# danini/multi-h

Hardware: AMD Instinct MI355X
Metric: scored homography hypotheses/sec (50k pts x 100k models) (higher is better)
Workload: dtype f64

## Files before the change

### multi-h_amd/csrc/capi.hip

```cpp

#include "capi_engine.hpp"

thread_local std::string g_err;

namespace mhe {

void resolve_timers(mh_engine* e)
{
    for (int k = 0; k < MH_K_COUNT_; ++k) {
        KernelTimer& t = e->timers[k];
        for (auto& pr : t.pending) {
            float ms = 0.f;
            if (hipEventSynchronize(pr.second) == hipSuccess &&
                hipEventElapsedTime(&ms, pr.first, pr.second) == hipSuccess) {
                t.total_ms += ms;
                t.launches += 1;
            }
        }
        t.pending.clear();
    }
}

int enter(mh_engine* e)
{
    if (!e) return fail(MH_ERR_INVALID, "null engine");
    HIPCHK(hipSetDevice(e->device));
    return MH_OK;
}

int require_points(mh_engine* e)
{
    int rc = enter(e);
    if (rc) return rc;
    if (e->n <= 0) return fail(MH_ERR_NOT_SET, "correspondences are not set");
    return MH_OK;
}

int require_models(mh_engine* e)
{
    int rc = require_points(e);
    if (rc) return rc;
    if (e->m <= 0) return fail(MH_ERR_NOT_SET, "model set is empty");
    return MH_OK;
}

int require_models_or_empty_shard(mh_engine* e, bool* empty)
{
    *empty = false;
    int rc = require_points(e);
    if (rc) return rc;
    if (e->m <= 0 && (e->t_stream_fn || e->t_host_fn)) { *empty = true; e->counts_fresh = true; return MH_OK; }
    if (e->m <= 0) return fail(MH_ERR_NOT_SET, "model set is empty");
    return MH_OK;
}

hipError_t reserve_counts(mh_engine* e, size_t n)
{
    if (n <= e->counts.cap) return hipSuccess;
    e->counts_zeroed = false;
    return e->counts.reserve(n);
}

int quiesce(mh_engine* e)
{
    HIPCHK(hipStreamSynchronize(e->stream));
    if (e->side_stream) HIPCHK(hipStreamSynchronize(e->side_stream));
    if (e->xchg_stream) HIPCHK(hipStreamSynchronize(e->xchg_stream));
    e->xchg_pending = false;
    return MH_OK;
}

int join_xchg(mh_engine* e)
{
    if (e->xchg_pending && e->xchg_calls > 0)
        HIPCHK(hipStreamWaitEvent(e->stream, e->ev_x[(e->xchg_calls - 1) % 3], 0));
    return MH_OK;
}

}

namespace {

template <typename Fn>
static void host_parallel_for(int n, Fn fn)
{
    unsigned t = std::thread::hardware_concurrency();
    if (t == 0) t = 1;
    if (t > 16) t = 16;
    if (n < 20000) t = 1;
    if (t == 1) { fn(0, n); return; }
    std::vector<std::thread> pool;
    const int chunk = (n + (int)t - 1) / (int)t;
    for (unsigned k = 0; k < t; ++k) {
        const int b = (int)k * chunk, en = std::min(n, b + chunk);
        if (b < en) pool.emplace_back(fn, b, en);
    }
    for (auto& th : pool) th.join();
}

int build_sym_graph(mh_engine* e, const int* rowptr, const int* col, int n)
{
    for (int i = 0; i < n; ++i)
        if (rowptr[i + 1] < rowptr[i]) return fail(MH_ERR_INVALID, "rowptr must be non-decreasing");
    std::unique_ptr<std::atomic<int>[]> cnt(new std::atomic<int>[(size_t)n + 1]);
    for (int i = 0; i <= n; ++i) cnt[i].store(0, std::memory_order_relaxed);
    std::atomic<int> bad(0);
    host_parallel_for(n, [&](int b, int en) {
        for (int i = b; i < en; ++i)
            for (int k = rowptr[i]; k < rowptr[i + 1]; ++k) {
                const int j = col[k];
                if (j < 0 || j >= n) { bad.store(1, std::memory_order_relaxed); continue; }
                if (j == i) continue;
                cnt[i].fetch_add(1, std::memory_order_relaxed);
                cnt[j].fetch_add(1, std::memory_order_relaxed);
            }
    });
    if (bad.load()) return fail(MH_ERR_INVALID, "neighbour index out of range");
    std::vector<long long> start(n + 1, 0);
    for (int i = 0; i < n; ++i) start[i + 1] = start[i] + cnt[i].load(std::memory_order_relaxed);
    if (start[n] > 0x7fffffffll) return fail(MH_ERR_OVERFLOW, "too many neighbour entries");
    std::vector<int> raw((size_t)start[n]);
    for (int i = 0; i < n; ++i) cnt[i].store(0, std::memory_order_relaxed);
    host_parallel_for(n, [&](int b, int en) {
        for (int i = b; i < en; ++i)
            for (int k = rowptr[i]; k < rowptr[i + 1]; ++k) {
                const int j = col[k];
                if (j == i) continue;
                raw[(size_t)(start[i] + cnt[i].fetch_add(1, std::memory_order_relaxed))] = j;
                raw[(size_t)(start[j] + cnt[j].fetch_add(1, std::memory_order_relaxed))] = i;
            }
    });
    std::vector<int> mult((size_t)start[n]);
    e->g_rowptr.assign(n + 1, 0);
    host_parallel_for(n, [&](int b, int en) {
        for (int i = b; i < en; ++i) {
            int* rb = raw.data() + start[i];
            int* re = raw.data() + start[i + 1];
            int* mb = mult.data() + start[i];
            std::sort(rb, re);
            int u = 0;
            for (int* p = rb; p < re;) {
                int* q = p;
                while (q < re && *q == *p) ++q;
                rb[u] = *p;
                mb[u] = (int)(q - p);
                ++u;
                p = q;
            }
            e->g_rowptr[i + 1] = u;
        }
    });
    for (int i = 0; i < n; ++i) e->g_rowptr[i + 1] += e->g_rowptr[i];
    const int nnz = e->g_rowptr[n];
    e->g_col.resize(nnz);
    e->g_w.resize(nnz);
    e->g_rev.assign(nnz, -1);
    host_parallel_for(n, [&](int b, int en) {
        for (int i = b; i < en; ++i) {
            const int len = e->g_rowptr[i + 1] - e->g_rowptr[i];
            std::copy(raw.data() + start[i], raw.data() + start[i] + len, e->g_col.data() + e->g_rowptr[i]);
            std::copy(mult.data() + start[i], mult.data() + start[i] + len, e->g_w.data() + e->g_rowptr[i]);
        }
    });
    host_parallel_for(n, [&](int b, int en) {
        for (int i = b; i < en; ++i)
            for (int k = e->g_rowptr[i]; k < e->g_rowptr[i + 1]; ++k) {
                const int j = e->g_col[k];
                const int* rb = e->g_col.data() + e->g_rowptr[j];
                const int* re = e->g_col.data() + e->g_rowptr[j + 1];
                e->g_rev[k] = (int)(std::lower_bound(rb, re, i) - e->g_col.data());
            }
    });
    return MH_OK;
}

static int upload_order(mh_engine* e)
{
    const int n = e->n;
    if (e->order_n == n) return MH_OK;
    std::vector<int> order(n);
    for (int i = 0; i < n; ++i) order[i] = i;
    unsigned long long z = 0x6d682d6f72646572ull;
    for (int i = n - 1; i > 0; --i) {
        z += 0x9E3779B97F4A7C15ull;
        unsigned long long x = z;
        x = (x ^ (x >> 30)) * 0xBF58476D1CE4E5B9ull;
        x = (x ^ (x >> 27)) * 0x94D049BB133111EBull;
        x ^= x >> 31;
        const int j = (int)(((x >> 32) * (unsigned long long)(i + 1)) >> 32);
        std::swap(order[i], order[j]);
    }
    HIPCHK(e->d_order.reserve(n));
    HIPCHK(hipMemcpyAsync(e->d_order.p, order.data(), sizeof(int) * n, hipMemcpyHostToDevice, e->stream));
    HIPCHK(hipStreamSynchronize(e->stream));
    e->order_n = n;
    return MH_OK;
}

static int upload_wsum(mh_engine* e)
{
    HIPCHK(e->d_wsum.reserve(e->n));
    HIPCHK(launch_row_weight_sums(e->n, e->d_rowptr.p, e->d_w.p, e->d_wsum.p, e->stream));
    return MH_OK;
}

int upload_graph(mh_engine* e)
{
    const int n = e->n, nnz = (int)e->g_col.size();
    HIPCHK(e->d_rowptr.reserve(n + 1));
    HIPCHK(e->d_col.reserve(nnz));
    HIPCHK(e->d_w.reserve(nnz));
    HIPCHK(e->d_rev.reserve(nnz));
    HIPCHK(hipMemcpyAsync(e->d_rowptr.p, e->g_rowptr.data(), sizeof(int) * (n + 1), hipMemcpyHostToDevice, e->stream));
    if (nnz) {
        HIPCHK(hipMemcpyAsync(e->d_col.p, e->g_col.data(), sizeof(int) * nnz, hipMemcpyHostToDevice, e->stream));
        HIPCHK(hipMemcpyAsync(e->d_w.p, e->g_w.data(), sizeof(int) * nnz, hipMemcpyHostToDevice, e->stream));
        HIPCHK(hipMemcpyAsync(e->d_rev.p, e->g_rev.data(), sizeof(int) * nnz, hipMemcpyHostToDevice, e->stream));
    }
    HIPCHK(hipStreamSynchronize(e->stream));
    int rc = upload_order(e);
    if (rc) return rc;
    rc = upload_wsum(e);
    if (rc) return rc;
    HIPCHK(hipStreamSynchronize(e->stream));
    e->g_nnz = nnz;
    e->g_host_valid = true;
    e->have_graph = true;
    return MH_OK;
}

static hipError_t fetch_ints(mh_engine* e, int* dst, const int* src_dev, size_t count)
{
    hipError_t he = hipMemcpyAsync(dst, src_dev, sizeof(int) * count, hipMemcpyDeviceToHost, e->stream);
    return he != hipSuccess ? he : hipStreamSynchronize(e->stream);
}

static int device_sym_graph(mh_engine* e, const int* rowptr_dev, int stride, const int* col_dev)
{
    const int n = e->n;
    HIPCHK(e->gb_deg.reserve(n));
    HIPCHK(e->gb_start.reserve((size_t)n + 1));
    HIPCHK(launch_sym_count(n, rowptr_dev, stride, col_dev, e->gb_deg.p, e->gb_start.p, e->gb_info.p, e->stream));
    int info[8] = {}, total = 0;
    HIPCHK(hipMemcpyAsync(info, e->gb_info.p, sizeof(int) * 4, hipMemcpyDeviceToHost, e->stream));
    HIPCHK(hipMemcpyAsync(&total, e->gb_start.p + n, sizeof(int), hipMemcpyDeviceToHost, e->stream));
    HIPCHK(hipStreamSynchronize(e->stream));
    if (info[2] == 2) return fail(MH_ERR_INVALID, "rowptr must be non-decreasing");
    if (info[2]) return fail(MH_ERR_INVALID, "neighbour index out of range (non-finite coordinates, or fewer than k neighbours at finite float32 distance?)");
    if (info[0]) return fail(MH_ERR_OVERFLOW, "too many neighbour entries");
    if (info[1] > SYM_MAX_ROW) {
        std::vector<int> rp(n + 1), col;
        if (rowptr_dev) {
            HIPCHK(fetch_ints(e, rp.data(), rowptr_dev, (size_t)n + 1));
            col.resize((size_t)rp[n]);
            if (rp[n] > 0) HIPCHK(fetch_ints(e, col.data(), col_dev, col.size()));
        } else {
            std::vector<int> dense((size_t)n * stride);
            HIPCHK(fetch_ints(e, dense.data(), col_dev, dense.size()));
            for (int i = 0; i < n; ++i) {
                rp[i] = (int)col.size();
                for (int j = 0; j < stride; ++j) if (dense[(size_t)i * stride + j] >= 0) col.push_back(dense[(size_t)i * stride + j]);
            }
            rp[n] = (int)col.size();
        }
        int rc = build_sym_graph(e, rp.data(), col.data(), n);
        if (rc) return rc;
        return upload_graph(e);
    }
    HIPCHK(e->gb_cursor.reserve(n));
    HIPCHK(e->gb_uniq.reserve(n));
    HIPCHK(e->gb_raw.reserve((size_t)std::max(total, 1)));
    HIPCHK(e->gb_mult.reserve((size_t)std::max(total, 1)));
    HIPCHK(e->d_rowptr.reserve((size_t)n + 1));
    HIPCHK(launch_sym_build(n, rowptr_dev, stride, col_dev, e->gb_start.p, e->gb_cursor.p, e->gb_raw.p, e->gb_mult.p,
                            e->gb_uniq.p, e->d_rowptr.p, e->gb_info.p, e->stream));
    int nnz = 0;
    HIPCHK(hipMemcpyAsync(&nnz, e->d_rowptr.p + n, sizeof(int), hipMemcpyDeviceToHost, e->stream));
    HIPCHK(hipStreamSynchronize(e->stream));
    HIPCHK(e->d_col.reserve((size_t)std::max(nnz, 1)));
    HIPCHK(e->d_w.reserve((size_t)std::max(nnz, 1)));
    HIPCHK(e->d_rev.reserve((size_t)std::max(nnz, 1)));
    HIPCHK(launch_sym_finish(n, e->gb_start.p, e->gb_raw.p, e->gb_mult.p, e->d_rowptr.p, e->d_col.p, e->d_w.p, e->d_rev.p, e->stream));
    int rc = upload_order(e);
    if (rc) return rc;
    rc = upload_wsum(e);
    if (rc) return rc;
    HIPCHK(hipStreamSynchronize(e->stream));
    e->g_nnz = nnz;
    e->g_host_valid = false;
    e->have_graph = true;
    return MH_OK;
}

__global__ void k_split_soa(int n, const double* src, const double* dst, const double* aff,
                            double* x1, double* y1, double* x2, double* y2, double* a11,
                            double* a12, double* a21, double* a22)
{
    const int i = blockIdx.x * 256 + threadIdx.x;
    if (i >= n) return;
    x1[i] = src[2 * i]; y1[i] = src[2 * i + 1];
    x2[i] = dst[2 * i]; y2[i] = dst[2 * i + 1];
    if (aff) { a11[i] = aff[4 * i]; a12[i] = aff[4 * i + 1]; a21[i] = aff[4 * i + 2]; a22[i] = aff[4 * i + 3]; }
}

}

extern "C" {

int mh_abi_version(void) { return MH_ABI_VERSION; }

const char* mh_last_error(void) { return g_err.c_str(); }

int mh_device_count(void)
{
    int c = 0;
    if (hipGetDeviceCount(&c) != hipSuccess) return 0;
    return c;
}

int mh_create(mh_engine** out, int device)
{
    return guarded([&]() -> int {
    if (!out) return fail(MH_ERR_INVALID, "out is null");
    *out = nullptr;
    int c = 0;
    if (hipGetDeviceCount(&c) != hipSuccess || c <= 0)
        return fail(MH_ERR_NO_DEVICE, "no HIP device visible; the Multi-H engine has no CPU fallback");
    if (device < 0 || device >= c) return fail(MH_ERR_INVALID, "device index out of range");
    HIPCHK(hipSetDevice(device));
    hipDeviceProp_t prop;
    HIPCHK(hipGetDeviceProperties(&prop, device));
    if (std::strncmp(prop.gcnArchName, "gfx950", 6) != 0)
        return fail(MH_ERR_NO_DEVICE, std::string("device arch is ") + prop.gcnArchName +
                                           "; this library carries gfx950 code objects only");
    mh_engine* e = new (std::nothrow) mh_engine();
    if (!e) return fail(MH_ERR_INVALID, "out of host memory");
    e->device = device;
    e->cu_count = prop.multiProcessorCount > 0 ? prop.multiProcessorCount : 256;
    hipError_t he = e->own_stream.ensure();
    if (he != hipSuccess) { delete e; return fail(MH_ERR_HIP, hipGetErrorString(he)); }
    e->stream = e->own_stream;
    *out = e;
    return MH_OK;
    });
}

void mh_destroy(mh_engine* e)
{
    if (!e) return;
    (void)hipSetDevice(e->device);
    (void)quiesce(e);
    resolve_timers(e);
    delete e;
}

int mh_set_params(mh_engine* e, double thr_F, double thr_H, double locality, double lambda, int min_inliers)
{
    return guarded([&]() -> int {
    if (!e) return fail(MH_ERR_INVALID, "null engine");
    if (!(thr_H > 0.0) || !(lambda > 0.0)) return fail(MH_ERR_INVALID, "thr_hom and lambda must be positive");
    e->thr_F = thr_F; e->thr_H = thr_H; e->locality = locality; e->lambda = lambda;
    e->min_inliers = min_inliers;
    e->cost_L = 0;
    return MH_OK;
    });
}

int mh_set_stream(mh_engine* e, void* hip_stream, int external)
{
    return guarded([&]() -> int {
    int rc0 = enter(e);
    if (rc0) return rc0;
    int rcq = quiesce(e);
    if (rcq) return rcq;
    resolve_timers(e);
    e->stream = external ? (hipStream_t)hip_stream : e->own_stream.s;
    return MH_OK;
    });
}

int mh_synchronize(mh_engine* e)
{
    return guarded([&]() -> int {
    int rc0 = enter(e);
    if (rc0) return rc0;
    rc0 = quiesce(e);
    if (rc0) return rc0;
    resolve_timers(e);
    return MH_OK;
    });
}

int mh_set_correspondences(mh_engine* e, const double* src_xy, const double* dst_xy,
                           const double* affines, int n)
{
    return guarded([&]() -> int {
    int rc0 = enter(e);
    if (rc0) return rc0;
    if (!src_xy || !dst_xy || n <= 0) return fail(MH_ERR_INVALID, "src/dst must be non-null and n > 0");
    rc0 = quiesce(e);
    if (rc0) return rc0;
    e->pf_count = 0;
    e->pf_head = 0;
    e->smp_k = 0;
    e->weights_models_seq = -1;
    const size_t cap = (size_t)n + 2;
    HIPCHK(e->x1.reserve(cap)); HIPCHK(e->y1.reserve(cap));
    HIPCHK(e->x2.reserve(cap)); HIPCHK(e->y2.reserve(cap));
    HIPCHK(e->a11.reserve(cap)); HIPCHK(e->a12.reserve(cap));
    HIPCHK(e->a21.reserve(cap)); HIPCHK(e->a22.reserve(cap));
    DevBuf<double> s, d, a;
    HIPCHK(s.reserve((size_t)n * 2));
    HIPCHK(d.reserve((size_t)n * 2));
    HIPCHK(hipMemcpyAsync(s.p, src_xy, sizeof(double) * 2 * n, hipMemcpyHostToDevice, e->stream));
    HIPCHK(hipMemcpyAsync(d.p, dst_xy, sizeof(double) * 2 * n, hipMemcpyHostToDevice, e->stream));
    if (affines) {
        HIPCHK(a.reserve((size_t)n * 4));
        HIPCHK(hipMemcpyAsync(a.p, affines, sizeof(double) * 4 * n, hipMemcpyHostToDevice, e->stream));
    }
    hipLaunchKernelGGL(k_split_soa, dim3((n + 255) / 256), dim3(256), 0, e->stream, n, s.p, d.p,
                       affines ? a.p : nullptr, e->x1.p, e->y1.p, e->x2.p, e->y2.p, e->a11.p,
                       e->a12.p, e->a21.p, e->a22.p);
    HIPCHK(hipGetLastError());
    HIPCHK(hipStreamSynchronize(e->stream));
    if (n != e->n) {
        drop_models(e);
        e->ldr = 0; e->fm = 0; e->f7_m = 0;
    }
    {
        double xmin = src_xy[0], xmax = src_xy[0], ymin = src_xy[1], ymax = src_xy[1], dmax = 0.0;
        bool finite = true, dfinite = true;
        for (int i = 0; i < n; ++i) {
            const double x = src_xy[2 * i], y = src_xy[2 * i + 1];
            finite = finite && std::isfinite(x) && std::isfinite(y);
            xmin = x < xmin ? x : xmin; xmax = x > xmax ? x : xmax;
            ymin = y < ymin ? y : ymin; ymax = y > ymax ? y : ymax;
            const double a = std::fabs(dst_xy[2 * i]), b = std::fabs(dst_xy[2 * i + 1]);
            dfinite = dfinite && std::isfinite(a) && std::isfinite(b);
            dmax = a > dmax ? a : dmax; dmax = b > dmax ? b : dmax;
        }
        if (!finite) xmin = xmax = ymin = ymax = NAN;
        e->bbox[0] = xmin; e->bbox[1] = xmax; e->bbox[2] = ymin; e->bbox[3] = ymax;
        e->absmax_x = std::max(std::fabs(xmin), std::fabs(xmax));
        e->absmax_y = std::max(std::fabs(ymin), std::fabs(ymax));
        e->absmax_dst = dmax;
        e->coords32_ok = finite && dfinite && e->absmax_x < 0x1p20 && e->absmax_y < 0x1p20 && dmax < 0x1p20;
    }
    e->n = n;
    e->have_aff = affines != nullptr;
    e->have_graph = false;
    e->g_rowptr.clear(); e->g_col.clear(); e->g_w.clear(); e->g_rev.clear();
    e->g_host_valid = false; e->g_nnz = 0;
    e->cost_L = 0;
    return MH_OK;
    });
}

int mh_set_epipolar(mh_engine* e, const double F[9], const double e2[2])
{
    return guarded([&]() -> int {
    if (!e || !F || !e2) return fail(MH_ERR_INVALID, "null argument");
    for (int i = 0; i < 9; ++i) e->epi.F[i] = F[i];
    e->epi.ex = e2[0];
    e->epi.ey = e2[1];
    e->have_epi = true;
    return MH_OK;
    });
}

int mh_set_neighbors_csr(mh_engine* e, const int* rowptr, const int* col, int n)
{
    return guarded([&]() -> int {
    int rc = require_points(e);
    if (rc) return rc;
    if (!rowptr || n != e->n) return fail(MH_ERR_INVALID, "rowptr null or n != number of correspondences");
    if (rowptr[n] > 0 && !col) return fail(MH_ERR_INVALID, "col is null");
    if (rowptr[0] < 0) return fail(MH_ERR_INVALID, "rowptr must be non-decreasing");
    for (int i = 0; i < n; ++i)
        if (rowptr[i + 1] < rowptr[i]) return fail(MH_ERR_INVALID, "rowptr must be non-decreasing");
    HIPCHK(e->gb_info.reserve(8));
    HIPCHK(hipMemsetAsync(e->gb_info.p, 0, sizeof(int) * 8, e->stream));
    HIPCHK(e->gb_hits_rp.reserve((size_t)n + 1));
    HIPCHK(e->gb_hits_col.reserve((size_t)std::max(rowptr[n], 1)));
    HIPCHK(hipMemcpyAsync(e->gb_hits_rp.p, rowptr, sizeof(int) * ((size_t)n + 1), hipMemcpyHostToDevice, e->stream));
    if (rowptr[n] > 0)
        HIPCHK(hipMemcpyAsync(e->gb_hits_col.p, col, sizeof(int) * (size_t)rowptr[n], hipMemcpyHostToDevice, e->stream));
    HIPCHK(hipStreamSynchronize(e->stream));
    return device_sym_graph(e, e->gb_hits_rp.p, 0, e->gb_hits_col.p);
    });
}

static int knn_table(mh_engine* e, int k, double radius, int* tbl)
{
    const int n = e->n;
    HIPCHK(e->gb_info.reserve(8));
    HIPCHK(hipMemsetAsync(e->gb_info.p, 0, sizeof(int) * 8, e->stream));
    const Points pp = e->pts();
    if (e->tune_knn_grid && std::isfinite(pp.xmin) && std::isfinite(pp.xmax) && std::isfinite(pp.ymin) && std::isfinite(pp.ymax)) {
        const int G = knn_grid_cells(n);
        HIPCHK(e->knn_cell.reserve((size_t)n));
        HIPCHK(e->knn_count.reserve((size_t)G * G));
        HIPCHK(e->knn_start.reserve((size_t)G * G + 1));
        HIPCHK(e->knn_P.reserve((size_t)4 * n));
        HIPCHK(e->knn_orig.reserve((size_t)n));
        const hipError_t hg = launch_knn_grid(pp, k, tbl, e->knn_cell.p, e->knn_count.p, e->knn_start.p, e->knn_P.p, e->knn_orig.p, e->stream);
        if (hg == hipSuccess) {
            const float r2g = radius > 0.0 ? (float)radius * (float)radius : INFINITY;
            HIPCHK(launch_hits_filter(pp, k, r2g, tbl, e->gb_info.p + 2, e->stream));
            return MH_OK;
        }
        if (hg != hipErrorInvalidValue) HIPCHK(hg);
    }
    const int blocks = (n + 255) / 256;
    int splits = (4 * e->cu_count + blocks - 1) / blocks;
    splits = std::max(1, std::min(splits, std::min(KNN_MAX_SPLITS, (n + 1023) / 1024)));
    const int kk = k <= 8 ? 8 : k <= 16 ? 16 : 32;
    if (splits > 1) {
        HIPCHK(e->knn_part_d.reserve((size_t)splits * n * kk));
        HIPCHK(e->knn_part_i.reserve((size_t)splits * n * kk));
    }
    HIPCHK(launch_knn(e->pts(), k, tbl, splits, e->knn_part_d.p, e->knn_part_i.p, e->stream));
    const float r2 = radius > 0.0 ? (float)radius * (float)radius : INFINITY;
    HIPCHK(launch_hits_filter(e->pts(), k, r2, tbl, e->gb_info.p + 2, e->stream));
    return MH_OK;
}

static int build_knn_graph(mh_engine* e, int k, double radius)
{
    int rc = require_points(e);
    if (rc) return rc;
    if (k < 1 || k > 32 || k >= e->n) return fail(MH_ERR_INVALID, "k must be in [1, 32] and < n");
    HIPCHK(e->knn_tmp.reserve((size_t)e->n * k));
    rc = knn_table(e, k, radius, e->knn_tmp.p);
    if (rc) return rc;
    return device_sym_graph(e, nullptr, k, e->knn_tmp.p);
}

int mh_build_neighbors_knn(mh_engine* e, int k)
{
    return guarded([&]() -> int { return build_knn_graph(e, k, 0.0); });
}

int mh_build_neighbors_knn_radius(mh_engine* e, int k, double radius)
{
    return guarded([&]() -> int { return build_knn_graph(e, k, radius); });
}

int mh_build_sample_neighbours(mh_engine* e, int k)
{
    return guarded([&]() -> int {
    int rc = require_points(e);
    if (rc) return rc;
    if (k < 3 || k > 32 || k >= e->n) return fail(MH_ERR_INVALID, "k must be in [3, 32] and < n");
    rc = quiesce(e);
    if (rc) return rc;
    e->smp_k = 0;
    HIPCHK(e->smp_nbr.reserve((size_t)e->n * k));
    rc = knn_table(e, k, 0.0, e->smp_nbr.p);
    if (rc) return rc;
    int err = 0;
    HIPCHK(fetch_ints(e, &err, e->gb_info.p + 2, 1));
    if (err) return fail(MH_ERR_INVALID, "neighbour index out of range (non-finite coordinates, or fewer than k neighbours at finite float32 distance?)");
    e->smp_k = k;
    return MH_OK;
    });
}

int mh_get_sample_neighbours(mh_engine* e, int* nbr, int* k_out)
{
    return guarded([&]() -> int {
    if (!e) return fail(MH_ERR_INVALID, "null engine");
    if (e->smp_k <= 0) return fail(MH_ERR_NOT_SET, "no sampling table; call mh_build_sample_neighbours");
    HIPCHK(hipSetDevice(e->device));
    if (nbr) HIPCHK(fetch_ints(e, nbr, e->smp_nbr.p, (size_t)e->n * e->smp_k));
    if (k_out) *k_out = e->smp_k;
    return MH_OK;
    });
}

int mh_build_neighbors_radius(mh_engine* e, double radius, long long max_hits, long long* hits_out)
{
    return guarded([&]() -> int {
    int rc = require_points(e);
    if (rc) return rc;
    if (!(radius > 0.0)) return fail(MH_ERR_INVALID, "radius must be positive");
    const int n = e->n;
    const float r2 = (float)radius * (float)radius;
    HIPCHK(e->knn_tmp.reserve((size_t)n + 1));
    HIPCHK(launch_radius_count(e->pts(), r2, e->knn_tmp.p, e->stream));
    std::vector<int> cnt(n), rowptr(n + 1, 0);
    HIPCHK(hipMemcpyAsync(cnt.data(), e->knn_tmp.p, sizeof(int) * n, hipMemcpyDeviceToHost, e->stream));
    HIPCHK(hipStreamSynchronize(e->stream));
    long long total = 0;
    for (int i = 0; i < n; ++i) total += cnt[i];
    if (hits_out) *hits_out = total;
    const long long limit = max_hits > 0 ? max_hits : 0x7fffffffll;
    if (total > limit || total > 0x7fffffffll) {
        char msg[160];
        snprintf(msg, sizeof msg, "radius search yields %lld hits (limit %lld): use a smaller radius or k-NN", total, limit);
        return fail(MH_ERR_OVERFLOW, msg);
    }
    for (int i = 0; i < n; ++i) rowptr[i + 1] = rowptr[i] + cnt[i];
    DevBuf<int> d_rp, d_col;
    HIPCHK(d_rp.reserve((size_t)n + 1));
    HIPCHK(d_col.reserve((size_t)std::max<long long>(total, 1)));
    HIPCHK(hipMemcpyAsync(d_rp.p, rowptr.data(), sizeof(int) * (n + 1), hipMemcpyHostToDevice, e->stream));
    HIPCHK(launch_radius_fill(e->pts(), r2, d_rp.p, d_col.p, e->stream));
    HIPCHK(e->gb_info.reserve(8));
    HIPCHK(hipMemsetAsync(e->gb_info.p, 0, sizeof(int) * 8, e->stream));
    return device_sym_graph(e, d_rp.p, 0, d_col.p);
    });
}

int mh_get_sym_graph(mh_engine* e, int* rowptr, int* col, int* w, int* nnz)
{
    return guarded([&]() -> int {
    if (!e) return fail(MH_ERR_INVALID, "null engine");
    if (!e->have_graph) return fail(MH_ERR_NOT_SET, "neighbour graph is not set");
    if (!e->g_host_valid) {
        HIPCHK(hipSetDevice(e->device));
        e->g_rowptr.resize((size_t)e->n + 1); e->g_col.resize(e->g_nnz); e->g_w.resize(e->g_nnz); e->g_rev.resize(e->g_nnz);
        HIPCHK(fetch_ints(e, e->g_rowptr.data(), e->d_rowptr.p, (size_t)e->n + 1));
        if (e->g_nnz) {
            HIPCHK(fetch_ints(e, e->g_col.data(), e->d_col.p, (size_t)e->g_nnz));
            HIPCHK(fetch_ints(e, e->g_w.data(), e->d_w.p, (size_t)e->g_nnz));
            HIPCHK(fetch_ints(e, e->g_rev.data(), e->d_rev.p, (size_t)e->g_nnz));
        }
        e->g_host_valid = true;
    }
    if (nnz) *nnz = e->g_nnz;
    if (rowptr) std::copy(e->g_rowptr.begin(), e->g_rowptr.end(), rowptr);
    if (col) std::copy(e->g_col.begin(), e->g_col.end(), col);
    if (w) std::copy(e->g_w.begin(), e->g_w.end(), w);
    return MH_OK;
    });
}

int mh_device_buffer(mh_engine* e, int which, void** ptr_dev, unsigned long long* bytes)
{
    return guarded([&]() -> int {
    if (!e || !ptr_dev || !bytes) return fail(MH_ERR_INVALID, "null argument");
    switch (which) {
    case MH_BUF_COUNTS: *ptr_dev = e->counts.p; *bytes = sizeof(int) * (size_t)e->m; break;
    case MH_BUF_MODELS: *ptr_dev = e->H.p; *bytes = sizeof(double) * 9 * (size_t)e->m; break;
    case MH_BUF_RESIDUALS: *ptr_dev = (e->ldr > 0 && e->m > 0) ? e->R.p : nullptr; *bytes = sizeof(double) * (size_t)e->m * (size_t)e->ldr; break;
    case MH_BUF_LABELS: *ptr_dev = e->ew_label.p; *bytes = sizeof(int) * (size_t)e->n; break;
    case MH_BUF_COST: *ptr_dev = e->cost.p; *bytes = sizeof(int) * (size_t)e->n * e->cost_L; break;
    case MH_BUF_GATHERED_SCORES: *ptr_dev = e->sel_gathered.p; *bytes = sizeof(int) * e->sel_gathered.cap; break;
    case MH_BUF_LABEL_COUNTS: *ptr_dev = e->label_counts.p; *bytes = sizeof(int) * std::min<size_t>(e->label_counts.cap, (size_t)e->m); break;
    case MH_BUF_WEIGHTS: *ptr_dev = e->weights_models_seq == e->models_seq ? e->weights.p : nullptr; *bytes = sizeof(int) * (size_t)e->m; break;
    default: return fail(MH_ERR_INVALID, "unknown buffer id");
    }
    if (!*ptr_dev) return fail(MH_ERR_NOT_SET, "buffer has not been produced yet");
    return MH_OK;
    });
}

int mh_profile_enable(mh_engine* e, int on)
{
    return guarded([&]() -> int {
    if (!e) return fail(MH_ERR_INVALID, "null engine");
    e->profiling = on != 0;
    return MH_OK;
    });
}

int mh_profile_reset(mh_engine* e)
{
    return guarded([&]() -> int {
    int rc0 = enter(e);
    if (rc0) return rc0;
    HIPCHK(hipStreamSynchronize(e->stream));
    resolve_timers(e);
    for (int k = 0; k < MH_K_COUNT_; ++k) { e->timers[k].launches = 0; e->timers[k].total_ms = 0.0; }
    return MH_OK;
    });
}

int mh_profile_get(mh_engine* e, int kernel, int* launches, double* total_ms)
{
    return guarded([&]() -> int {
    if (!e || kernel < 0 || kernel >= MH_K_COUNT_) return fail(MH_ERR_INVALID, "bad kernel id");
    HIPCHK(hipSetDevice(e->device));
    HIPCHK(hipStreamSynchronize(e->stream));
    if (e->xchg_stream) HIPCHK(hipStreamSynchronize(e->xchg_stream));
    resolve_timers(e);
    if (launches) *launches = e->timers[kernel].launches;
    if (total_ms) *total_ms = e->timers[kernel].total_ms;
    return MH_OK;
    });
}

int mh_set_tuning(mh_engine* e, int key, int value)
{
    return guarded([&]() -> int {
    if (!e) return fail(MH_ERR_INVALID, "null engine");
#ifdef MH_TUNING
    if (key == 0) { e->tune_residual_variant = value; return MH_OK; }
    if (key == 1) { e->tune_score_variant = value; return MH_OK; }
    if (key == 13 && value >= 0) { e->tune_ld = value; return MH_OK; }
#else
    if (key == 0 || key == 1) {
        if (value == 0) return MH_OK;
        return fail(MH_ERR_INVALID, "residual / score kernel variants exist only in a library built with -DMH_TUNING");
    }
#endif
    if (key >= 2 && key <= 5 && value >= 1) { e->tune_expand[key - 2] = value; return MH_OK; }
    if (key == 6 && value >= 0) { e->tune_reduce = value; return MH_OK; }
    if (key == 7 && value >= 1 && value <= 64) { e->tune_ms_batch = value; return MH_OK; }
    if (key == 29 && value >= 0 && value <= 64) { e->tune_ms_persist = value; return MH_OK; }
    if (key == 32 && (value == 0 || value == 1)) { e->tune_ms_indexed = value; return MH_OK; }
    if (key == 37 && value >= 1 && value <= EXPAND_MAX_CTX) { e->tune_expand_ctx = value; return MH_OK; }
    if (key == 38 && value >= 0 && value <= (1 << 20)) { e->tune_batch_min_labels = value; return MH_OK; }
    if (key == 39 && (value == 0 || value == 16 || value == 32 || value == 64)) { e->tune_batch_spw = value; return MH_OK; }
    if (key == 36 && (value == 0 || value == 1)) { e->tune_select_decrement = value; return MH_OK; }
    if (key == 33 && value >= 0 && value <= (1 << 20)) { e->tune_ms_dense = value; return MH_OK; }
    if (key == 30 && (value == 0 || value == 1)) { e->tune_select_refine = value; return MH_OK; }
    if (key == 31 && (value == 0 || value == 1)) { e->tune_knn_grid = value; return MH_OK; }
    if (key == 8 && value >= 0 && value <= (1 << 20)) { e->trace_moves = value; return MH_OK; }
    if (key == 9 && value >= -1) { e->detail_move = value; return MH_OK; }
    if (key == 10 && value >= 1 && value <= 64) { e->tune_push_mult = value; return MH_OK; }
    if (key == 11 && (value == 0 || value == 1)) { e->tune_recycle = value; return MH_OK; }
    if (key == 12 && (value == 1 || value == 2)) { e->tune_reduce_launches = value; return MH_OK; }
    if (key == 14 && value >= 0 && value <= 8) { e->inject_barrier_timeouts = value; return MH_OK; }
    if (key == 40 && (value == 0 || (value >> 4) >= 1)) { e->inject_solve_failure = value; return MH_OK; }
    if (key == 15 && (value == 0 || value == 1)) { e->tune_score32 = value; return MH_OK; }
#ifdef MH_TUNING
    if (key == 16 && value >= 0 && value <= 16) { e->tune_score32_tiling = value; return MH_OK; }
#else
    if (key == 16 && value == 0) return MH_OK;
#endif
    if (key == 17 && value >= 0 && value <= 1000) { e->tune_cascade_iters = value; return MH_OK; }
    if (key == 18 && value >= 0 && value <= 1000) { e->inject_select_failure = value; return MH_OK; }
    if (key == 19 && value >= -1 && value <= 1024) { e->tune_sweep_headroom = value; return MH_OK; }
    if (key == 20 && (value == 0 || value == 1)) { e->tune_dlt_first = value; return MH_OK; }
    if (key == 21 && value >= 0 && value <= (1 << 16)) { e->comp_moves = value; return MH_OK; }
    if (key == 22 && value >= 0 && value <= 16 && !e->side_stream) { e->tune_stream_shift = value; return MH_OK; }
    if (key == 23 && value >= -1 && value <= 64) { e->tune_cost32_resident = value; return MH_OK; }
    if (key == 24 && value >= -1 && value <= 64) { e->tune_score32_resident = value; return MH_OK; }
    if (key == 25 && value >= 0 && value <= 2) { e->tune_dlt_variant = value; return MH_OK; }
#ifdef MH_TUNING
    if (key == 26 && value >= 0 && value <= 4096) { e->tune_sweep_slices = value; return MH_OK; }
    if (key == 27 && (value == 0 || value == 1)) { e->tune_cost32_slice_major = value; return MH_OK; }
    if (key == 28 && (value == 0 || value == 1)) { e->tune_cost32_batched = value; return MH_OK; }
    if (key == 34 && value >= 0 && value <= 2) { e->tune_3pt_form = value; return MH_OK; }
#else
    if ((key == 26 || key == 27 || key == 28 || key == 34) && value == 0) return MH_OK;
    if (key == 16 || key == 26 || key == 27 || key == 28 || key == 34)
        return fail(MH_ERR_INVALID, "this schedule variant exists only in a library built with -DMH_TUNING");
#endif
    return fail(MH_ERR_INVALID, "unknown tuning key");
    });
}

}
```

### multi-h_amd/csrc/capi_engine.hpp

```cpp
#pragma once
#include "../../include/multih_hip.h"
#include "mh_kernels.hpp"

#include <algorithm>
#include <chrono>
#include <cstdlib>
#include <cmath>
#include <cstdio>
#include <cstring>
#include <string>
#include <utility>
#include <atomic>
#include <memory>
#include <thread>
#include <vector>

using namespace mh;

extern thread_local std::string g_err;

inline int fail(int code, const std::string& msg)
{
    g_err = msg;
    return code;
}

#define HIPCHK(expr)                                                                      \
    do {                                                                                  \
        hipError_t e_ = (expr);                                                           \
        if (e_ != hipSuccess)                                                             \
            return fail(MH_ERR_HIP, std::string(#expr) + ": " + hipGetErrorString(e_));   \
    } while (0)

struct NoCopy {
    NoCopy() = default;
    NoCopy(const NoCopy&) = delete;
    NoCopy& operator=(const NoCopy&) = delete;
};

template <class T>
struct DevBuf : NoCopy {
    T* p = nullptr;
    size_t cap = 0;
    DevBuf() = default;
    DevBuf(DevBuf&& o) noexcept { *this = std::move(o); }
    DevBuf& operator=(DevBuf&& o) noexcept { std::swap(p, o.p); std::swap(cap, o.cap); return *this; }
    ~DevBuf() { if (p) (void)hipFree(p); }
    hipError_t reserve(size_t n)
    {
        if (n <= cap) return hipSuccess;
        if (p) { hipError_t e = hipFree(p); p = nullptr; cap = 0; if (e != hipSuccess) return e; }
        hipError_t e = hipMalloc((void**)&p, std::max<size_t>(n, 1) * sizeof(T));
        if (e == hipSuccess) cap = n;
        return e;
    }
};

template <class T>
struct PinnedBuf : NoCopy {
    T* h = nullptr;
    T* d = nullptr;
    size_t cap = 0;
    ~PinnedBuf() { if (h) (void)hipHostFree(h); }
    hipError_t ensure(size_t n, bool mapped = true)
    {
        if (n <= cap) return hipSuccess;
        if (h) { (void)hipHostFree(h); h = d = nullptr; cap = 0; }
        hipError_t e = hipHostMalloc((void**)&h, n * sizeof(T), mapped ? hipHostMallocMapped : hipHostMallocDefault);
        if (e == hipSuccess && mapped) e = hipHostGetDevicePointer((void**)&d, h, 0);
        if (e != hipSuccess) { if (h) (void)hipHostFree(h); h = d = nullptr; return e; }
        std::memset(h, 0, n * sizeof(T));
        cap = n;
        return hipSuccess;
    }
};

struct Event : NoCopy {
    hipEvent_t ev = nullptr;
    Event() = default;
    Event(Event&& o) noexcept : ev(o.ev) { o.ev = nullptr; }
    Event& operator=(Event&& o) noexcept { std::swap(ev, o.ev); return *this; }
    ~Event() { if (ev) (void)hipEventDestroy(ev); }
    hipError_t ensure(unsigned flags = hipEventDisableTiming) { return ev ? hipSuccess : hipEventCreateWithFlags(&ev, flags); }
    operator hipEvent_t() const { return ev; }
};

struct Stream : NoCopy {
    hipStream_t s = nullptr;
    ~Stream() { if (s) { (void)hipStreamSynchronize(s); (void)hipStreamDestroy(s); } }
    hipError_t ensure(bool highest_priority = false)
    {
        if (s) return hipSuccess;
        if (!highest_priority) return hipStreamCreateWithFlags(&s, hipStreamNonBlocking);
        int lo = 0, hi = 0;
        hipError_t e = hipDeviceGetStreamPriorityRange(&lo, &hi);
        return e != hipSuccess ? e : hipStreamCreateWithPriority(&s, hipStreamNonBlocking, hi);
    }
    operator hipStream_t() const { return s; }
};

struct ExpandCtxBufs {
    DevBuf<int> arcs, sites, core, flags;
    DevBuf<long long> acc;
    DevBuf<unsigned char> took;
    static size_t pitch(int count) { return ((size_t)count + 2 + 63) & ~(size_t)63; }
    hipError_t reserve(int n, int nnz, bool with_took_list, hipStream_t stream)
    {
        auto grow = [&](auto& buf, size_t count) -> hipError_t {
            const size_t had = buf.cap;
            hipError_t e = buf.reserve(count);
            if (e == hipSuccess && buf.cap != had) e = hipMemsetAsync(buf.p, 0, sizeof(*buf.p) * buf.cap, stream);
            return e;
        };
        hipError_t e = grow(arcs, 2 * pitch(nnz));
        if (e == hipSuccess) e = grow(sites, (with_took_list ? 5 : 4) * pitch(n));
        if (e == hipSuccess) e = grow(core, (size_t)EXPAND_CORE_SHARDS * n);
        if (e == hipSuccess) e = grow(flags, EXPAND_FLAG_WORDS);
        if (e == hipSuccess) e = grow(acc, EXPAND_ACC_WORDS);
        if (e == hipSuccess) e = grow(took, (size_t)n + 2);
        return e;
    }
    ExpandWork::Ctx view(int n, int nnz) const
    {
        const size_t pa = pitch(nnz), ps = pitch(n);
        ExpandWork::Ctx x{};
        x.cap = arcs.p; x.sent = arcs.p + pa;
        x.excess = sites.p; x.sink_cap = sites.p + ps; x.height = sites.p + 2 * ps; x.decided = sites.p + 3 * ps;
        x.took_list = sites.cap >= 5 * ps ? sites.p + 4 * ps : nullptr;
        x.took = took.p; x.core = core.p; x.flags = flags.p; x.acc = acc.p;
        return x;
    }
};

struct KernelTimer {
    std::vector<std::pair<Event, Event>> pending;
    int launches = 0;
    double total_ms = 0.0;
};

enum class BatchOrigin { GIVEN, DLT4, HAF, P3 };
struct ResidentBatch {
    int m = 0;
    BatchOrigin origin = BatchOrigin::GIVEN;
    int haf_members = 0;
    bool have_samples = false;
};

struct CountsSlot {
    DevBuf<int> buf;
    bool zeroed = false;
    int wait = -1;
};

struct mh_engine : ResidentBatch {
    int device = 0;
    Stream own_stream;
    hipStream_t stream = nullptr;
    double thr_F = 3.0, thr_H = 2.5, locality = 0.002, lambda = 0.5;
    int min_inliers = 0;

    int n = 0;
    bool have_aff = false, have_epi = false, have_graph = false;
    DevBuf<double> x1, y1, x2, y2, a11, a12, a21, a22;
    Epipolar epi{};

    std::vector<int> g_rowptr, g_col, g_w, g_rev;
    bool g_host_valid = false;
    int g_nnz = 0;
    DevBuf<int> gb_deg, gb_start, gb_cursor, gb_raw, gb_mult, gb_uniq, gb_info, gb_hits_rp, gb_hits_col;
    int order_n = -1;
    DevBuf<int> d_rowptr, d_col, d_w, d_rev;

    DevBuf<double> H, H_one;
    DevBuf<int> samples, counts;
    DevBuf<unsigned> haf_used;
    DevBuf<double> R;
    long long ldr = 0;
    DevBuf<int> C;
    long long ldc = 0;
    DevBuf<unsigned char> mask;
    DevBuf<double> moments, min_eig;
    DevBuf<double> cp_pts, cp_H, cp_out;
    DevBuf<int> cp_begin, cp_tri;
    DevBuf<unsigned char> cp_ok;
    DevBuf<int> sel_orig[2], sel_counts, sel_carried[2], sel_left, sel_rec, sel_scores, sel_gathered;
    DevBuf<int> sel_weights, sel_carried_w[2], sel_left_w;
    DevBuf<double> sel_cand_H[2], sel_out_H;
    DevBuf<SelRecord> sel_records;
    DevBuf<long long> sel_counter;
    DevBuf<unsigned long long> sel_keys;
    int t_rank = 0, t_world = 1;
    mh_allgather_stream_fn t_stream_fn = nullptr;
    mh_allgather_dev_fn t_host_fn = nullptr;
    void* t_ctx = nullptr;
    Stream side_stream;
    Event ev_main, ev_side_pre;
    int tune_score32_resident = 12;
    int occ_score32 = -1, occ_cost32 = -1;
    int tune_cost32_batched = 0;
    int tune_cost32_slice_major = 0;
    int tune_sweep_slices = 0;
    int tune_dlt_variant = 0;
    int tune_cost32_resident = 8;
    int tune_stream_shift = 0;
    Stream dummy_streams[16];
    int tune_dlt_first = 1;
    static constexpr int PF_DEPTH = 2;
    DevBuf<double> pf_H[PF_DEPTH];
    DevBuf<int> pf_samples[PF_DEPTH];
    int pf_m[PF_DEPTH] = { 0, 0 };
    Event pf_ev[PF_DEPTH];
    int pf_head = 0, pf_count = 0;
    Stream xchg_stream;
    Event ev_sweep, ev_x[3];
    CountsSlot counts_waiting[2];
    long long xchg_calls = 0;
    long long models_seq = 0, best_models_seq = -1;
    bool counts_zeroed = false;
    bool counts_fresh = false;
    bool xchg_pending = false;
    PinnedBuf<int> h_best;
    int best_seq = 0;
    PinnedBuf<int> h_sel;
    long long copies_h2d = 0, copies_d2h = 0;

    int fm = 0;
    int fund_metric = 0;
    DevBuf<double> fund, fund_one;
    DevBuf<int> fund_samples, fund_counts, fund_inl;
    int fund_tuple = 8;
    int f7_m = 0;
    DevBuf<int> fund_nvalid, fund_stop;
    DevBuf<unsigned char> fund_mask, ref_keep, ref_in, ref_reason;
    int ref_reason_n = 0;
    DevBuf<double> ref_out;

    DevBuf<double> loc_H, loc_feat, ms_data, ms_mean;
    DevBuf<int> ms_votes, ms_out, ms_list, ms_pcnt, ms_heads, ms_tickets;
    DevBuf<double> ms_partial, ms_partial2;
    DevBuf<unsigned long long> ms_ticks;
    DevBuf<int> ms_ctl, ms_pcnt2;
    int ms_persist_per_cu = -1, ms_persist_per_cu6 = -1;
    int tune_select_refine = 0;
    int estimator = MH_ESTIMATOR_HAF;
    int data_term = MH_DATA_TERM_REFERENCE;
    DevBuf<int> r3_scratch;
    int tune_3pt_form = 0;
    DevBuf<double> sel_refit;
    DevBuf<int> sel_refit_ctr;
    DevBuf<double> ms_rs;
    DevBuf<int> ms_order, ms_cells, ms_cursor, ms_cellcount;
    int tune_ms_indexed = 1;
    int tune_ms_dense = 8;
    long long ms_indexed_launches = 0;
    int tune_ms_persist = 12;
    long long ms_persist_launches = 0, ms_persist_fallbacks = 0, ms_rounds = 0;

    int cost_L = 0;
    DevBuf<int> cost, labels_in, labels_pts, label_counts;
    DevBuf<int> ew_label, ew_cur, ew_trace, ew_saved, d_order, d_wsum;
    int comp_moves = 0;
    DevBuf<int> ew_comp, ew_comp_out;
    int trace_moves = 0;
    int detail_move = -1;
    ExpandCtxBufs ew_ctx[EXPAND_MAX_CTX];
    DevBuf<int> ew_bctl;
    PinnedBuf<int> h_batch;
    int tune_expand_ctx = 16;
    int tune_batch_min_labels = 16;
    int tune_batch_spw = 0;
    int cu_count = 256;
    DevBuf<int> sweep_ctl;
    int sweep_wg_per_cu = -1;
    int tune_sweep_headroom = 0;
    int solve_grid_max = 0;
    double longest_barrier_wait_ms = 0.0;
    int last_expand_retries = 0;
    long long expand_retries_total = 0;
    int last_solve_grid = 0;
    int inject_select_failure = 0;
    int inject_barrier_timeouts = 0;
    int inject_solve_failure = 0;
    PinnedBuf<int> h_flags;
    PinnedBuf<long long> h_acc;
    PinnedBuf<MeanShiftResultBlock> h_ms;
    PinnedBuf<int> h_ms_list;
    DevBuf<double> sel_pts[4];
    DevBuf<int> sel_pack_count;
    DevBuf<double> sel_gone[4];
    int tune_select_decrement = 1;
    int tune_knn_grid = 1;
    DevBuf<int> knn_cell, knn_count, knn_start, knn_orig;
    DevBuf<float> knn_P;
    DevBuf<int> knn_tmp, knn_part_i;
    DevBuf<float> knn_part_d;
    int sampler = MH_SAMPLER_UNIFORM, sampler_uniform_per_16 = 0;
    DevBuf<int> smp_nbr;
    int smp_k = 0;
    Dlt4Local dlt_local() const { return sampler == MH_SAMPLER_LOCAL ? Dlt4Local{ smp_nbr.p, smp_k, sampler_uniform_per_16 } : Dlt4Local{}; }

    bool profiling = false;
    KernelTimer timers[MH_K_COUNT_];
    int tune_residual_variant = 0;
    int tune_ld = 0;
    int tune_score_variant = 0;
    int residual_mode = MH_RESIDUAL_FORWARD;
    int tune_ms_batch = 6;
    int tune_reduce = 2;
    int tune_reduce_launches = 1;
    int tune_recycle = 1;
    int tune_expand[4] = { 128, 512, 1, 256 };
    int tune_cascade_iters = 2;
    int tune_push_mult = 6;
    ExpandStats last_expand{};

    double bbox[4] = { NAN, NAN, NAN, NAN };
    bool coords32_ok = false;
    double absmax_x = NAN, absmax_y = NAN, absmax_dst = NAN;
    int tune_score32_tiling = 0;
    int tune_score32 = 1;
    DevBuf<float> H32;
    DevBuf<unsigned long long> fb_pairs;
    long long score_pairs = 0;
    long long score_pairs_plain_fp64 = 0;
    DevBuf<int> weights, weights_counts;
    long long weights_models_seq = -1;
    PinnedBuf<int> h_best_w;
    Points pts() const { return Points{ x1.p, y1.p, x2.p, y2.p, n, bbox[0], bbox[1], bbox[2], bbox[3] }; }
};

namespace mhe {

template <typename Fn>
int guarded(Fn&& fn)
{
    try {
        return fn();
    } catch (const std::bad_alloc&) {
        return fail(MH_ERR_INVALID, "out of host memory");
    } catch (const std::exception& ex) {
        return fail(MH_ERR_INVALID, std::string("internal error: ") + ex.what());
    } catch (...) {
        return fail(MH_ERR_INVALID, "internal error");
    }
}

struct ScopedTimer {
    mh_engine* e;
    int k;
    hipStream_t st;
    Event a, b;
    bool on = false;
    ScopedTimer(mh_engine* e_, int k_, hipStream_t on_stream = nullptr) : e(e_), k(k_), st(on_stream ? on_stream : e_->stream)
    {
        if (!e->profiling || a.ensure(hipEventDefault) != hipSuccess || b.ensure(hipEventDefault) != hipSuccess) return;
        (void)hipEventRecord(a, st);
        on = true;
    }
    ~ScopedTimer()
    {
        if (!on) return;
        (void)hipEventRecord(b, st);
        e->timers[k].pending.emplace_back(std::move(a), std::move(b));
    }
};

inline void drop_models(mh_engine* e)
{
    static_cast<ResidentBatch&>(*e) = ResidentBatch{};
    e->cost_L = 0;
    e->counts_fresh = false;
    ++e->models_seq;
}

inline void install_models(mh_engine* e, int m, BatchOrigin origin, bool have_samples, int haf_members = 0)
{
    static_cast<ResidentBatch&>(*e) = ResidentBatch{ m, origin, haf_members, have_samples };
}

inline void counts_scored(mh_engine* e) { e->counts_fresh = true; e->counts_zeroed = false; }

inline int hand_counts_to_exchange(mh_engine* e, int par)
{
    CountsSlot* w = e->counts_waiting;
    const int wait = w[0].wait;
    std::swap(e->counts, w[0].buf);
    e->counts_zeroed = w[0].zeroed;
    w[0].zeroed = true;
    w[0].wait = par;
    std::swap(w[0], w[1]);
    return wait;
}

void resolve_timers(mh_engine* e);
int enter(mh_engine* e);
int require_points(mh_engine* e);
int require_models(mh_engine* e);
int require_models_or_empty_shard(mh_engine* e, bool* empty);
hipError_t reserve_counts(mh_engine* e, size_t n);
int quiesce(mh_engine* e);
int join_xchg(mh_engine* e);
int score_models(mh_engine* e, const Points& p, const double* Hs, int m, double thr2, const unsigned char* dmask, int* counts_dev);
int msac_models(mh_engine* e, const Points& p, const double* Hs, int m, double thr2, const unsigned char* dmask, int* counts_dev,
                int* weights_dev, bool plain_variant_only);
int launch_estimator(mh_engine* e, const int* labels_dev, int Nh, double* H_dev, int* counts_dev);
int ensure_xchg_stream(mh_engine* e);
int ensure_side_stream(mh_engine* e);

}

using namespace mhe;
```

### multi-h_amd/csrc/capi_score.hip

```cpp
#include "capi_engine.hpp"

namespace mhe {

static bool pretest_usable(const mh_engine* e, double thr2, bool plain_variant_only)
{
    if (plain_variant_only && e->tune_score_variant != 0) return false;
    return e->tune_score32 && e->coords32_ok && thr2 >= 0x1p-40 && thr2 <= 0x1p40;
}

static int ensure_sweep_ctl(mh_engine* e)
{
    if (!e->sweep_ctl.p) {
        HIPCHK(e->sweep_ctl.reserve(2));
        HIPCHK(hipMemsetAsync(e->sweep_ctl.p, 0, sizeof(int) * 2, e->stream));
    }
    return MH_OK;
}

int score_models(mh_engine* e, const Points& p, const double* Hs, int m, double thr2, const unsigned char* dmask, int* counts_dev)
{
    const bool fwd = e->residual_mode != MH_RESIDUAL_SYMMETRIC;
    if (fwd && m > 0 && pretest_usable(e, thr2, true)) {
        HIPCHK(e->H32.reserve((size_t)m * 16));
        HIPCHK(e->fb_pairs.reserve(1));
        if (e->score_pairs == 0) HIPCHK(hipMemsetAsync(e->fb_pairs.p, 0, sizeof(unsigned long long), e->stream));
        HIPCHK(launch_model32(Hs, m, e->absmax_x, e->absmax_y, e->absmax_dst, e->H32.p, e->stream));
        int* ctl = nullptr;
        if (e->tune_score32_resident != 0) {
            int rc = ensure_sweep_ctl(e);
            if (rc) return rc;
            ctl = e->sweep_ctl.p;
        }
        HIPCHK(launch_score32(p, Hs, e->H32.p, m, thr2, e->absmax_dst, dmask, counts_dev, e->fb_pairs.p, e->tune_score32_tiling, e->stream,
                              ctl, e->cu_count, e->tune_score32_resident, &e->occ_score32));
        e->score_pairs += (long long)m * p.n;
        return MH_OK;
    }
    HIPCHK(launch_score(p, Hs, m, thr2, dmask, counts_dev, fwd ? e->tune_score_variant : -1, e->stream));
    return MH_OK;
}

int msac_models(mh_engine* e, const Points& p, const double* Hs, int m, double thr2, const unsigned char* dmask, int* counts_dev,
                int* weights_dev, bool plain_variant_only)
{
    if (m <= 0 || p.n <= 0) return MH_OK;
    HIPCHK(e->fb_pairs.reserve(1));
    if (e->score_pairs == 0) HIPCHK(hipMemsetAsync(e->fb_pairs.p, 0, sizeof(unsigned long long), e->stream));
    if (pretest_usable(e, thr2, plain_variant_only)) {
        HIPCHK(e->H32.reserve((size_t)m * 16));
        HIPCHK(launch_model32(Hs, m, e->absmax_x, e->absmax_y, e->absmax_dst, e->H32.p, e->stream));
        HIPCHK(launch_msac32(p, Hs, e->H32.p, m, thr2, e->absmax_dst, dmask, counts_dev, weights_dev, e->fb_pairs.p, e->stream));
    } else {
        HIPCHK(launch_msac64(p, Hs, m, thr2, dmask, counts_dev, weights_dev, e->stream));
        e->score_pairs_plain_fp64 += (long long)m * p.n;
    }
    e->score_pairs += (long long)m * p.n;
    return MH_OK;
}

int ensure_side_stream(mh_engine* e)
{
    if (!e->side_stream)
        for (int k = 0; k < e->tune_stream_shift; ++k) HIPCHK(e->dummy_streams[k].ensure());
    HIPCHK(e->side_stream.ensure(true));
    for (int q = 0; q < mh_engine::PF_DEPTH; ++q) HIPCHK(e->pf_ev[q].ensure());
    HIPCHK(e->ev_main.ensure());
    HIPCHK(e->ev_side_pre.ensure());
    return MH_OK;
}

}

extern "C" {

int mh_propose_dlt4(mh_engine* e, unsigned long long seed, long long first, int m)
{
    return guarded([&]() -> int {
    int rc = require_points(e);
    if (rc) return rc;
    if (m <= 0) return fail(MH_ERR_INVALID, "m must be positive");
    if (e->n < 4) return fail(MH_ERR_INVALID, "need at least 4 correspondences");
    if (e->sampler == MH_SAMPLER_LOCAL && e->smp_k <= 0) return fail(MH_ERR_NOT_SET, "the local sampler has no table; call mh_build_sample_neighbours");
    drop_models(e);
    HIPCHK(e->H.reserve((size_t)m * 9));
    HIPCHK(e->samples.reserve((size_t)m * 4));
    HIPCHK(reserve_counts(e, (size_t)m + 1));
    {
        ScopedTimer t(e, MH_K_DLT4);
        HIPCHK(launch_dlt4(e->pts(), seed, first, m, e->samples.p, e->H.p, e->stream, e->tune_dlt_variant == 1 ? 1 : 0, e->dlt_local()));
    }
    install_models(e, m, BatchOrigin::DLT4, true);
    return MH_OK;
    });
}

int mh_set_sampler(mh_engine* e, int sampler, int uniform_per_16)
{
    return guarded([&]() -> int {
    if (!e) return fail(MH_ERR_INVALID, "null engine");
    if (sampler != MH_SAMPLER_UNIFORM && sampler != MH_SAMPLER_LOCAL) return fail(MH_ERR_INVALID, "unknown sampler");
    if (uniform_per_16 < 0 || uniform_per_16 > 16) return fail(MH_ERR_INVALID, "uniform_per_16 must be in [0, 16]");
    e->sampler = sampler;
    e->sampler_uniform_per_16 = uniform_per_16;
    return MH_OK;
    });
}

int mh_set_models(mh_engine* e, const double* H, int m)
{
    return guarded([&]() -> int {
    if (!e || m < 0 || (m > 0 && !H)) return fail(MH_ERR_INVALID, "null argument or m < 0");
    HIPCHK(hipSetDevice(e->device));
    drop_models(e);
    if (m == 0) return MH_OK;
    HIPCHK(e->H.reserve((size_t)m * 9));
    HIPCHK(reserve_counts(e, (size_t)m + 1));
    HIPCHK(hipMemcpyAsync(e->H.p, H, sizeof(double) * 9 * m, hipMemcpyHostToDevice, e->stream));
    HIPCHK(hipStreamSynchronize(e->stream));
    install_models(e, m, BatchOrigin::GIVEN, false);
    return MH_OK;
    });
}

int mh_get_models(mh_engine* e, double* H)
{
    return guarded([&]() -> int {
    if (!e || !H) return fail(MH_ERR_INVALID, "null argument");
    HIPCHK(hipSetDevice(e->device));
    if (e->m <= 0) return fail(MH_ERR_NOT_SET, "model set is empty");
    HIPCHK(hipMemcpyAsync(H, e->H.p, sizeof(double) * 9 * e->m, hipMemcpyDeviceToHost, e->stream));
    HIPCHK(hipStreamSynchronize(e->stream));
    return MH_OK;
    });
}

int mh_get_model(mh_engine* e, int idx, double H[9])
{
    return guarded([&]() -> int {
    if (!e || !H) return fail(MH_ERR_INVALID, "null argument");
    HIPCHK(hipSetDevice(e->device));
    if (e->m <= 0) return fail(MH_ERR_NOT_SET, "model set is empty");
    if (idx < 0 || idx >= e->m) return fail(MH_ERR_INVALID, "model index out of range");
    HIPCHK(hipMemcpyAsync(H, e->H.p + 9 * (size_t)idx, sizeof(double) * 9, hipMemcpyDeviceToHost, e->stream));
    HIPCHK(hipStreamSynchronize(e->stream));
    return MH_OK;
    });
}

int mh_get_model_count(mh_engine* e, int* m)
{
    return guarded([&]() -> int {
    if (!e || !m) return fail(MH_ERR_INVALID, "null argument");
    *m = e->m;
    return MH_OK;
    });
}

int mh_get_samples(mh_engine* e, int* idx)
{
    return guarded([&]() -> int {
    if (!e || !idx) return fail(MH_ERR_INVALID, "null argument");
    HIPCHK(hipSetDevice(e->device));
    if (!e->have_samples) return fail(MH_ERR_NOT_SET, "no sampled batch; call mh_propose_dlt4");
    HIPCHK(hipMemcpyAsync(idx, e->samples.p, sizeof(int) * 4 * e->m, hipMemcpyDeviceToHost, e->stream));
    HIPCHK(hipStreamSynchronize(e->stream));
    return MH_OK;
    });
}

int mh_set_residual_mode(mh_engine* e, int mode)
{
    return guarded([&]() -> int {
    if (!e) return fail(MH_ERR_INVALID, "null engine");
    if (mode != MH_RESIDUAL_FORWARD && mode != MH_RESIDUAL_SYMMETRIC) return fail(MH_ERR_INVALID, "unknown residual mode");
    e->residual_mode = mode;
    return MH_OK;
    });
}

int mh_score(mh_engine* e, double thr2, const unsigned char* point_mask, int* counts)
{
    return guarded([&]() -> int {
    bool empty_shard = false;
    int rc = require_models_or_empty_shard(e, &empty_shard);
    if (rc || empty_shard) return rc;
    HIPCHK(reserve_counts(e, (size_t)e->m + 1));
    const unsigned char* dmask = nullptr;
    if (point_mask) {
        HIPCHK(e->mask.reserve((size_t)e->n + 2));
        HIPCHK(hipMemcpyAsync(e->mask.p, point_mask, e->n, hipMemcpyHostToDevice, e->stream));
        dmask = e->mask.p;
    }
    {
        ScopedTimer t(e, MH_K_SCORE);
        rc = score_models(e, e->pts(), e->H.p, e->m, thr2, dmask, e->counts.p);
        if (rc) return rc;
    }
    counts_scored(e);
    if (counts) {
        HIPCHK(hipMemcpyAsync(counts, e->counts.p, sizeof(int) * e->m, hipMemcpyDeviceToHost, e->stream));
        HIPCHK(hipStreamSynchronize(e->stream));
    }
    return MH_OK;
    });
}

int mh_score_msac(mh_engine* e, double thr2, const unsigned char* point_mask, int* counts, int* weights)
{
    return guarded([&]() -> int {
    bool empty_shard = false;
    int rc = require_models_or_empty_shard(e, &empty_shard);
    if (rc || empty_shard) return rc;
    if (e->residual_mode == MH_RESIDUAL_SYMMETRIC) return fail(MH_ERR_INVALID, "mh_score_msac: forward residual only");
    if ((long long)e->n * MH_MSAC_SCALE > 2147483647ll) return fail(MH_ERR_OVERFLOW, "mh_score_msac: n * MH_MSAC_SCALE exceeds int32");
    HIPCHK(reserve_counts(e, (size_t)e->m + 1));
    HIPCHK(e->weights.reserve((size_t)e->m + 1));
    HIPCHK(e->weights_counts.reserve((size_t)e->m + 1));
    const unsigned char* dmask = nullptr;
    if (point_mask) {
        HIPCHK(e->mask.reserve((size_t)e->n + 2));
        HIPCHK(hipMemcpyAsync(e->mask.p, point_mask, e->n, hipMemcpyHostToDevice, e->stream));
        dmask = e->mask.p;
    }
    e->weights_models_seq = -1;
    {
        ScopedTimer t(e, MH_K_SCORE);
        rc = msac_models(e, e->pts(), e->H.p, e->m, thr2, dmask, e->counts.p, e->weights.p, false);
        if (rc) return rc;
    }
    HIPCHK(hipMemcpyAsync(e->weights_counts.p, e->counts.p, sizeof(int) * (size_t)e->m, hipMemcpyDeviceToDevice, e->stream));
    counts_scored(e);
    e->weights_models_seq = e->models_seq;
    if (counts) HIPCHK(hipMemcpyAsync(counts, e->counts.p, sizeof(int) * e->m, hipMemcpyDeviceToHost, e->stream));
    if (weights) HIPCHK(hipMemcpyAsync(weights, e->weights.p, sizeof(int) * e->m, hipMemcpyDeviceToHost, e->stream));
    if (counts || weights) HIPCHK(hipStreamSynchronize(e->stream));
    return MH_OK;
    });
}

int mh_residual_matrix(mh_engine* e, double thr2, double* R_host, int* counts)
{
    return guarded([&]() -> int {
    bool empty_shard = false;
    int rc = require_models_or_empty_shard(e, &empty_shard);
    if (rc || empty_shard) return rc;
    e->ldr = residual_ld(e->n);
    size_t r_elems = (size_t)e->m * (size_t)e->ldr;
#ifdef MH_TUNING
    if (e->tune_ld > 0) { e->ldr = std::max<long long>(e->tune_ld, e->ldr); r_elems = (size_t)e->m * (size_t)e->ldr; }
    r_elems = std::max(r_elems, (size_t)((e->m + 15) / 16 * 16) * (size_t)((e->n + 1023) / 1024 * 1024));
#endif
    HIPCHK(e->R.reserve(r_elems));
    HIPCHK(reserve_counts(e, (size_t)e->m + 1));
    int resident = 0;
    if (e->tune_sweep_headroom >= 0 && e->residual_mode != MH_RESIDUAL_SYMMETRIC && (e->tune_residual_variant == 0 || (e->tune_residual_variant >= 50 && e->tune_residual_variant <= 52))) {
        if (e->sweep_wg_per_cu < 0) e->sweep_wg_per_cu = residual_workgroups_per_cu();
        const int headroom = e->tune_sweep_headroom > 0 ? e->tune_sweep_headroom : (e->t_stream_fn && e->t_world > 1 ? 32 : 0);
        resident = e->sweep_wg_per_cu * e->cu_count - headroom;
        if (resident < e->cu_count) resident = 0;
        if (resident > 0) {
            rc = ensure_sweep_ctl(e);
            if (rc) return rc;
        }
    }
    if (e->pf_count == 1 && e->tune_dlt_first && e->ev_side_pre) HIPCHK(hipStreamWaitEvent(e->stream, e->ev_side_pre, 0));
    {
        ScopedTimer t(e, MH_K_RESIDUAL);
        SweepLaunch how;
        how.slices = e->tune_sweep_slices;
        how.slice_major = e->tune_sweep_slices > 0 ? 1 : 0;
        how.counts_zeroed = e->counts_zeroed;
        how.resident_grid = resident;
        how.resident_ctl = e->sweep_ctl.p;
        HIPCHK(launch_residual(e->pts(), e->H.p, e->m, thr2, e->R.p, e->ldr, e->counts.p,
                               e->residual_mode == MH_RESIDUAL_SYMMETRIC ? -1 : e->tune_residual_variant, e->stream, how));
    }
    counts_scored(e);
    if (R_host)
        HIPCHK(hipMemcpy2DAsync(R_host, sizeof(double) * e->n, e->R.p, sizeof(double) * e->ldr,
                                sizeof(double) * e->n, e->m, hipMemcpyDeviceToHost, e->stream));
    if (counts)
        HIPCHK(hipMemcpyAsync(counts, e->counts.p, sizeof(int) * e->m, hipMemcpyDeviceToHost, e->stream));
    if (R_host || counts) HIPCHK(hipStreamSynchronize(e->stream));
    return MH_OK;
    });
}

int mh_cost_matrix(mh_engine* e, int* C_host, int* counts)
{
    return guarded([&]() -> int {
    bool empty_shard = false;
    int rc = require_models_or_empty_shard(e, &empty_shard);
    if (rc || empty_shard) return rc;
    e->ldc = cost_ld(e->n);
    HIPCHK(e->C.reserve((size_t)e->m * (size_t)e->ldc));
    HIPCHK(reserve_counts(e, (size_t)e->m + 1));
    {
        ScopedTimer t(e, MH_K_COSTMATRIX);
        const double thr2 = e->thr_H * e->thr_H;
        if (pretest_usable(e, thr2, false)) {
            HIPCHK(e->H32.reserve((size_t)e->m * 16));
            HIPCHK(launch_model32(e->H.p, e->m, e->absmax_x, e->absmax_y, e->absmax_dst, e->H32.p, e->stream));
            int* ctl = nullptr;
            if (e->tune_cost32_resident != 0) {
                rc = ensure_sweep_ctl(e);
                if (rc) return rc;
                ctl = e->sweep_ctl.p;
            }
            HIPCHK(launch_cost32(e->pts(), e->H.p, e->H32.p, e->m, e->lambda, thr2, e->absmax_dst, e->C.p, e->ldc, e->counts.p, e->stream,
                                 ctl, e->cu_count, e->tune_cost32_resident > 0 ? e->tune_cost32_resident : 0, e->tune_cost32_slice_major, e->tune_cost32_batched, &e->occ_cost32,
                                 e->data_term == MH_DATA_TERM_RISING));
        } else
            HIPCHK(launch_cost_matrix(e->pts(), e->H.p, e->m, e->lambda, thr2, e->C.p, e->ldc, e->counts.p, e->stream,
                                      e->data_term == MH_DATA_TERM_RISING));
    }
    counts_scored(e);
    if (C_host)
        HIPCHK(hipMemcpy2DAsync(C_host, sizeof(int) * e->n, e->C.p, sizeof(int) * e->ldc, sizeof(int) * e->n, e->m,
                                hipMemcpyDeviceToHost, e->stream));
    if (counts) HIPCHK(hipMemcpyAsync(counts, e->counts.p, sizeof(int) * e->m, hipMemcpyDeviceToHost, e->stream));
    if (C_host || counts) HIPCHK(hipStreamSynchronize(e->stream));
    return MH_OK;
    });
}

int mh_get_residual_rows(mh_engine* e, int first, int count, double* rows_host)
{
    return guarded([&]() -> int {
    int rc = require_models(e);
    if (rc) return rc;
    if (!e->R.p || e->ldr <= 0) return fail(MH_ERR_NOT_SET, "residual matrix has not been computed");
    if (first < 0 || count <= 0 || first + count > e->m || !rows_host)
        return fail(MH_ERR_INVALID, "row range out of bounds or null output");
    HIPCHK(hipMemcpy2DAsync(rows_host, sizeof(double) * e->n, e->R.p + (size_t)first * e->ldr,
                            sizeof(double) * e->ldr, sizeof(double) * e->n, count,
                            hipMemcpyDeviceToHost, e->stream));
    HIPCHK(hipStreamSynchronize(e->stream));
    return MH_OK;
    });
}

int mh_prefetch_dlt4(mh_engine* e, unsigned long long seed, long long first, int m)
{
    return guarded([&]() -> int {
    int rc = require_points(e);
    if (rc) return rc;
    if (m <= 0) return fail(MH_ERR_INVALID, "m must be positive");
    if (e->n < 4) return fail(MH_ERR_INVALID, "need at least 4 correspondences");
    if (e->sampler == MH_SAMPLER_LOCAL && e->smp_k <= 0) return fail(MH_ERR_NOT_SET, "the local sampler has no table; call mh_build_sample_neighbours");
    rc = ensure_side_stream(e);
    if (rc) return rc;
    if (e->pf_count >= mh_engine::PF_DEPTH) return fail(MH_ERR_INVALID, "two batches are already prefetched: adopt one first (mh_adopt_prefetched)");
    const int slot = (e->pf_head + e->pf_count) % mh_engine::PF_DEPTH;
    if (e->pf_H[slot].cap < (size_t)m * 9 || e->pf_samples[slot].cap < (size_t)m * 4) {
        HIPCHK(hipStreamSynchronize(e->side_stream));
        HIPCHK(hipStreamSynchronize(e->stream));
        HIPCHK(e->pf_H[slot].reserve((size_t)m * 9));
        HIPCHK(e->pf_samples[slot].reserve((size_t)m * 4));
    }
    HIPCHK(hipEventRecord(e->ev_main, e->stream));
    HIPCHK(hipStreamWaitEvent(e->side_stream, e->ev_main, 0));
    HIPCHK(hipEventRecord(e->ev_side_pre, e->side_stream));
    {
        ScopedTimer t(e, MH_K_DLT4, e->side_stream);
        HIPCHK(launch_dlt4(e->pts(), seed, first, m, e->pf_samples[slot].p, e->pf_H[slot].p, e->side_stream, e->tune_dlt_variant == 2 ? 0 : 1, e->dlt_local()));
    }
    HIPCHK(hipEventRecord(e->pf_ev[slot], e->side_stream));
    e->pf_m[slot] = m;
    ++e->pf_count;
    return MH_OK;
    });
}

int mh_adopt_prefetched(mh_engine* e)
{
    return guarded([&]() -> int {
    int rc = require_points(e);
    if (rc) return rc;
    if (e->pf_count <= 0) return fail(MH_ERR_NOT_SET, "no prefetched batch (mh_prefetch_dlt4)");
    const int slot = e->pf_head;
    drop_models(e);
    HIPCHK(hipStreamWaitEvent(e->stream, e->pf_ev[slot], 0));
    HIPCHK(reserve_counts(e, (size_t)e->pf_m[slot] + 1));
    std::swap(e->H, e->pf_H[slot]);
    std::swap(e->samples, e->pf_samples[slot]);
    e->pf_head = (e->pf_head + 1) % mh_engine::PF_DEPTH;
    --e->pf_count;
    install_models(e, e->pf_m[slot], BatchOrigin::DLT4, true);
    return MH_OK;
    });
}

int mh_inliers_of_model(mh_engine* e, int idx, double thr2, int label_value, int* labels)
{
    return guarded([&]() -> int {
    int rc = require_models(e);
    if (rc) return rc;
    if (idx < 0 || idx >= e->m || !labels) return fail(MH_ERR_INVALID, "bad model index or null labels");
    HIPCHK(e->labels_pts.reserve(e->n));
    HIPCHK(hipMemcpyAsync(e->labels_pts.p, labels, sizeof(int) * e->n, hipMemcpyHostToDevice, e->stream));
    HIPCHK(launch_inliers_of_model(e->pts(), e->H.p, idx, thr2, label_value, e->labels_pts.p, e->stream));
    HIPCHK(hipMemcpyAsync(labels, e->labels_pts.p, sizeof(int) * e->n, hipMemcpyDeviceToHost, e->stream));
    HIPCHK(hipStreamSynchronize(e->stream));
    return MH_OK;
    });
}

int mh_inliers_of_homography(mh_engine* e, const double* H, double thr2, int label_value, int* labels)
{
    return guarded([&]() -> int {
    int rc = require_points(e);
    if (rc) return rc;
    if (!H || !labels) return fail(MH_ERR_INVALID, "null homography or labels");
    HIPCHK(e->H_one.reserve(9));
    HIPCHK(e->labels_pts.reserve(e->n));
    HIPCHK(hipMemcpyAsync(e->H_one.p, H, sizeof(double) * 9, hipMemcpyHostToDevice, e->stream));
    HIPCHK(hipMemcpyAsync(e->labels_pts.p, labels, sizeof(int) * e->n, hipMemcpyHostToDevice, e->stream));
    HIPCHK(launch_inliers_of_model(e->pts(), e->H_one.p, 0, thr2, label_value, e->labels_pts.p, e->stream));
    HIPCHK(hipMemcpyAsync(labels, e->labels_pts.p, sizeof(int) * e->n, hipMemcpyDeviceToHost, e->stream));
    HIPCHK(hipStreamSynchronize(e->stream));
    return MH_OK;
    });
}

int mh_inlier_moments(mh_engine* e, double thr2, double* moments, double* min_eig)
{
    return guarded([&]() -> int {
    int rc = require_models(e);
    if (rc) return rc;
    HIPCHK(e->moments.reserve((size_t)e->m * 6));
    HIPCHK(e->min_eig.reserve(e->m));
    HIPCHK(launch_moments(e->pts(), e->H.p, e->m, thr2, e->moments.p, e->min_eig.p, e->stream));
    if (moments)
        HIPCHK(hipMemcpyAsync(moments, e->moments.p, sizeof(double) * 6 * e->m, hipMemcpyDeviceToHost, e->stream));
    if (min_eig)
        HIPCHK(hipMemcpyAsync(min_eig, e->min_eig.p, sizeof(double) * e->m, hipMemcpyDeviceToHost, e->stream));
    HIPCHK(hipStreamSynchronize(e->stream));
    return MH_OK;
    });
}

}
```

### multi-h_amd/csrc/capi_select.hip

```cpp
#include "capi_engine.hpp"

namespace mhe {

int ensure_xchg_stream(mh_engine* e)
{
    HIPCHK(e->xchg_stream.ensure(true));
    HIPCHK(e->ev_sweep.ensure());
    for (int b = 0; b < 3; ++b) HIPCHK(e->ev_x[b].ensure());
    return MH_OK;
}

}

namespace {

int exchange(mh_engine* e, const void* send_dev, void* recv_dev, size_t bytes_per_rank, hipStream_t on)
{
    if (e->t_stream_fn) {
        if (e->t_stream_fn(e->t_ctx, send_dev, recv_dev, (unsigned long long)bytes_per_rank, (void*)on) != 0)
            return fail(MH_ERR_INVALID, "all-gather failed (stream-ordered transport)");
        return MH_OK;
    }
    if (!e->t_host_fn) return fail(MH_ERR_NOT_SET, "no transport set (mh_set_transport)");
    HIPCHK(hipStreamSynchronize(on));
    if (e->t_host_fn(e->t_ctx, send_dev, recv_dev, (unsigned long long)bytes_per_rank) != 0)
        return fail(MH_ERR_INVALID, "all-gather failed (host-synchronised transport)");
    return MH_OK;
}

int selection_mode_word(const mh_engine* e, bool by_weight)
{
    int w = 0;
    if (e->residual_mode == MH_RESIDUAL_SYMMETRIC) w |= SEL_MODE_SYMMETRIC;
    if (e->tune_select_refine != 0) w |= SEL_MODE_REFIT | (e->estimator == MH_ESTIMATOR_3PT ? SEL_MODE_REFIT_3PT : 0);
    if (e->sampler == MH_SAMPLER_LOCAL)
        w |= SEL_MODE_SAMPLER_LOCAL | (e->smp_k << SEL_MODE_SAMPLER_K_SHIFT) | (e->sampler_uniform_per_16 << SEL_MODE_SAMPLER_UNIFORM_SHIFT);
    if (by_weight) w |= SEL_MODE_BY_WEIGHT;
    if (e->origin == BatchOrigin::HAF) w |= SEL_MODE_HAF | (e->haf_members << SEL_MODE_HAF_MEMBERS_SHIFT);
    if (e->origin == BatchOrigin::P3) w |= SEL_MODE_P3;
    return w;
}

int select_greedy(mh_engine* e, double thr2, int need, int max_models, unsigned char* point_mask, double* H_out,
                  long long* counters_out, int* counts_out, int* weights_out, int* selected_out, long long total_m, const bool by_weight)
{
    int rc = require_points(e);
    if (rc) return rc;
    if (!H_out || !selected_out || max_models <= 0 || need < 1) return fail(MH_ERR_INVALID, "bad argument");
    const int n = e->n;
    if (by_weight) {
        if (e->residual_mode == MH_RESIDUAL_SYMMETRIC) return fail(MH_ERR_INVALID, "mh_select_greedy_msac: forward residual only");
        if ((long long)n * MH_MSAC_SCALE > 2147483647ll) return fail(MH_ERR_OVERFLOW, "mh_select_greedy_msac: n * MH_MSAC_SCALE exceeds int32");
    }
    int M = e->m;
    const bool sharded = e->t_stream_fn || e->t_host_fn;
    const int world = sharded ? e->t_world : 1, rank = sharded ? e->t_rank : 0;
    if (total_m <= 0) total_m = M;
    if (total_m > 0xfffffffell) return fail(MH_ERR_INVALID, "more than 2^32 - 2 hypotheses in a batch");
    const int base = (int)(total_m / world), rem = (int)(total_m % world);
    const int longest = base + (rem ? 1 : 0);
    const int mine = base + (rank < rem ? 1 : 0);
    const unsigned int my_off = (unsigned int)((long long)rank * base + std::min(rank, rem));
    int local_rc = MH_OK;
    std::string local_msg;
    auto local_failure = [&](int code, const std::string& msg) { if (local_rc == MH_OK) { local_rc = code; local_msg = msg; } };
    const int symmetric = e->residual_mode == MH_RESIDUAL_SYMMETRIC ? 1 : 0;
    const bool refine = e->tune_select_refine != 0;
    const bool refit3 = e->estimator == MH_ESTIMATOR_3PT;
    const bool refine_usable = refine && e->have_epi && (refit3 || e->have_aff);
    const int mode_word = selection_mode_word(e, by_weight);
    if (refine && !refine_usable)
        local_failure(MH_ERR_NOT_SET, std::string(by_weight ? "mh_select_greedy_msac" : "mh_select_greedy") +
                                      (refit3 ? " with refitted winners (mh_set_tuning key 30) needs the epipolar geometry"
                                              : " with refitted winners (mh_set_tuning key 30) needs affinities and the epipolar geometry"));
    if (refine) {
        HIPCHK(e->labels_pts.reserve((size_t)n));
        HIPCHK(e->sel_refit.reserve(10));
        HIPCHK(e->sel_refit_ctr.reserve(2));
        if (refit3) HIPCHK(e->r3_scratch.reserve(reestimate_3pt_scratch_ints(n, 1)));
    }
    if (!sharded && M <= 0) local_failure(MH_ERR_NOT_SET, "model set is empty");
    else if (M != mine) local_failure(MH_ERR_INVALID, "the resident model set is not this rank's shard of total_m hypotheses");
    if (local_rc != MH_OK && !sharded) return fail(local_rc, local_msg);
    if (local_rc != MH_OK) M = 0;
    rc = join_xchg(e);
    if (rc) return rc;
    const size_t cap = (size_t)std::max(M, 1);
    for (int b = 0; b < 2; ++b) { HIPCHK(e->sel_orig[b].reserve(cap)); HIPCHK(e->sel_cand_H[b].reserve(cap * 9)); }
    HIPCHK(e->sel_counts.reserve(cap));
    if (by_weight) HIPCHK(e->sel_weights.reserve(cap));
    HIPCHK(e->sel_rec.reserve(8));
    HIPCHK(e->sel_keys.reserve(2));
    HIPCHK(e->sel_out_H.reserve((size_t)max_models * 9));
    HIPCHK(e->sel_counter.reserve(max_models));
    HIPCHK(e->sel_records.reserve((size_t)world + 1));
    HIPCHK(e->mask.reserve((size_t)n + 2));
    if (sharded) {
        HIPCHK(e->sel_scores.reserve((size_t)std::max(longest, 1)));
        HIPCHK(e->sel_gathered.reserve((size_t)world * std::max(longest, 1)));
    }
    HIPCHK(e->h_sel.ensure(8));
    const int* const h_sel = e->h_sel.h;
    hipStream_t s = e->stream;
    if (point_mask) { HIPCHK(hipMemcpyAsync(e->mask.p, point_mask, n, hipMemcpyHostToDevice, s)); ++e->copies_h2d; }
    else HIPCHK(hipMemsetAsync(e->mask.p, 1, n, s));
    HIPCHK(hipMemsetAsync(e->sel_rec.p, 0, sizeof(int) * 8, s));
    HIPCHK(hipMemsetAsync(e->sel_keys.p, 0, sizeof(unsigned long long) * 2, s));
    HIPCHK(hipMemsetAsync(e->sel_records.p, 0, sizeof(SelRecord) * ((size_t)world + 1), s));
    if (sharded && longest > 0) HIPCHK(hipMemsetAsync(e->sel_scores.p, 0xff, sizeof(int) * (size_t)longest, s));
    unsigned long long* key_local = e->sel_keys.p;
    unsigned long long* key_check = e->sel_keys.p + 1;
    SelRecord* my_record = e->sel_records.p;
    SelRecord* records = sharded ? e->sel_records.p + 1 : e->sel_records.p;

    int active = n;
    if (point_mask) { active = 0; for (int i = 0; i < n; ++i) active += point_mask[i] != 0 ? 1 : 0; }
    for (int c = 0; c < 4; ++c) HIPCHK(e->sel_pts[c].reserve((size_t)n + 2));
    HIPCHK(e->sel_pack_count.reserve(1));
    const bool decrement = e->tune_select_decrement != 0;
    if (decrement) {
        for (int c = 0; c < 4; ++c) HIPCHK(e->sel_gone[c].reserve((size_t)n + 2));
        for (int b = 0; b < 2; ++b) HIPCHK(e->sel_carried[b].reserve(cap));
        HIPCHK(e->sel_left.reserve(cap));
        if (by_weight) {
            for (int b = 0; b < 2; ++b) HIPCHK(e->sel_carried_w[b].reserve(cap));
            HIPCHK(e->sel_left_w.reserve(cap));
        }
    }
    int gone = 0;
    int* const weights = by_weight ? e->sel_weights.p : nullptr;

    int Mc = M, cur = 0, selected = 0, packed_as = -1;
    bool first = true;
    for (int round = 0; round < max_models; ++round) {
        const double* Hs = first ? e->H.p : e->sel_cand_H[cur].p;
        const int* orig = first ? nullptr : e->sel_orig[cur].p;
        auto score = [&](const Points& p, int* counts, int* wgts) -> int {
            return by_weight ? msac_models(e, p, Hs, Mc, thr2, nullptr, counts, wgts, true) : score_models(e, p, Hs, Mc, thr2, nullptr, counts);
        };
        auto score_round = [&]() -> int {
            if (e->inject_select_failure > 0 && --e->inject_select_failure == 0)
                return fail(MH_ERR_HIP, "greedy selection: injected rank-local failure (test hook, mh_set_tuning key 18)");
            if (Mc <= 0) return MH_OK;
            ScopedTimer t(e, MH_K_SCORE);
            if (decrement && !first && gone <= active) {
                if (gone == 0) {
                    HIPCHK(hipMemcpyAsync(e->sel_counts.p, e->sel_carried[cur].p, sizeof(int) * (size_t)Mc, hipMemcpyDeviceToDevice, s));
                    if (weights) HIPCHK(hipMemcpyAsync(weights, e->sel_carried_w[cur].p, sizeof(int) * (size_t)Mc, hipMemcpyDeviceToDevice, s));
                    return MH_OK;
                }
                Points left = e->pts();
                left.x1 = e->sel_gone[0].p; left.y1 = e->sel_gone[1].p; left.x2 = e->sel_gone[2].p; left.y2 = e->sel_gone[3].p;
                left.n = gone;
                const int rcs = score(left, e->sel_left.p, e->sel_left_w.p);
                if (rcs) return rcs;
                HIPCHK(launch_sel_subtract(e->sel_carried[cur].p, e->sel_left.p, e->sel_carried_w[cur].p, e->sel_left_w.p, Mc, e->sel_counts.p, weights, s));
                return MH_OK;
            }
            if (active == n) return score(e->pts(), e->sel_counts.p, weights);
            if (active > 0) {
                HIPCHK(launch_sel_pack_points(e->pts(), e->mask.p, e->sel_pts[0].p, e->sel_pts[1].p, e->sel_pts[2].p, e->sel_pts[3].p,
                                              e->sel_pack_count.p, s));
                packed_as = active;
                Points packed = e->pts();
                packed.x1 = e->sel_pts[0].p; packed.y1 = e->sel_pts[1].p; packed.x2 = e->sel_pts[2].p; packed.y2 = e->sel_pts[3].p;
                packed.n = active;
                return score(packed, e->sel_counts.p, weights);
            }
            HIPCHK(hipMemsetAsync(e->sel_counts.p, 0, sizeof(int) * (size_t)Mc, s));
            if (weights) HIPCHK(hipMemsetAsync(weights, 0, sizeof(int) * (size_t)Mc, s));
            return MH_OK;
        };
        if (local_rc == MH_OK) {
            const int src = score_round();
            if (src != MH_OK) {
                if (!sharded) return src;
                local_failure(src, g_err);
                Mc = 0;
            }
        }
        const int local_err = local_rc != MH_OK ? 1 : 0;
        const bool gather_scores = sharded && first && longest > 0;
        HIPCHK(launch_sel_argmax(e->sel_counts.p, weights, orig, Mc, need, my_off, key_local, gather_scores ? e->sel_scores.p : nullptr, s));
        HIPCHK(launch_sel_record(e->sel_counts.p, weights, orig, Hs, Mc, my_off, key_local, local_err, mode_word, my_record, s));
        if (sharded) {
            if (gather_scores) {
                rc = exchange(e, e->sel_scores.p, e->sel_gathered.p, sizeof(int) * (size_t)longest, s);
                if (rc) return rc;
                HIPCHK(launch_sel_argmax_gathered(e->sel_gathered.p, world, longest, base, rem, key_check, s));
            }
            rc = exchange(e, my_record, records, sizeof(SelRecord), s);
            if (rc) return rc;
        }
        HIPCHK(launch_sel_compact(e->sel_counts.p, weights, orig, Hs, Mc, need, records, world, my_off, e->sel_orig[cur ^ 1].p,
                                  e->sel_cand_H[cur ^ 1].p, e->sel_rec.p, decrement ? e->sel_carried[cur ^ 1].p : nullptr,
                                  e->sel_carried_w[cur ^ 1].p, s));
        const double* refit = nullptr;
        if (refine_usable) {
            Affines aff{ e->a11.p, e->a12.p, e->a21.p, e->a22.p };
            HIPCHK(launch_sel_refit(e->pts(), aff, e->epi, records, world, thr2, e->mask.p, e->labels_pts.p, e->sel_refit.p,
                                    e->sel_refit_ctr.p, e->sel_refit_ctr.p + 1, s, by_weight, symmetric, refit3 ? e->r3_scratch.p : nullptr));
            refit = e->sel_refit.p;
        }
        const unsigned long long* check = gather_scores && !local_err ? key_check : nullptr;
        double* gp[4] = { decrement ? e->sel_gone[0].p : nullptr, decrement ? e->sel_gone[1].p : nullptr,
                          decrement ? e->sel_gone[2].p : nullptr, decrement ? e->sel_gone[3].p : nullptr };
        HIPCHK(launch_sel_claim(e->pts(), records, world, check, thr2, e->mask.p, e->sel_rec.p, e->sel_out_H.p, e->sel_counter.p,
                                max_models, s, by_weight, symmetric, refit, gp[0], gp[1], gp[2], gp[3]));
        HIPCHK(launch_sel_publish(e->sel_rec.p, e->sel_keys.p, my_record, e->h_sel.d, s));
        HIPCHK(hipStreamSynchronize(s));
        if (local_rc != MH_OK) return fail(local_rc, local_msg);
        if (h_sel[4] != 0)
            return fail(h_sel[4] == 3 ? MH_ERR_INVALID : MH_ERR_HIP,
                        h_sel[4] == 2 ? "greedy selection: the gathered score vector and the ranks' records disagree about the winner"
                        : h_sel[4] == 3 ? "greedy selection: the ranks are not in the same residual mode (mh_set_residual_mode) or do not agree on refitted winners (mh_set_tuning key 30), the estimator (mh_set_estimator), the proposer's sampler (mh_set_sampler) or the selection's score (mh_select_greedy / mh_select_greedy_msac), or proposed their shards differently (mh_propose_haf and its members, mh_propose_3pt)"
                                           : "greedy selection: a rank reported an error");
        if (h_sel[0] < 0) break;
        if (counts_out) counts_out[selected] = h_sel[6];
        if (weights_out) weights_out[selected] = h_sel[0];
        ++selected;
        gone = h_sel[5];
        active -= gone;
        Mc = h_sel[2];
        cur ^= 1;
        first = false;
    }
    *selected_out = selected;
    if (selected > 0) {
        HIPCHK(hipMemcpyAsync(H_out, e->sel_out_H.p, sizeof(double) * 9 * (size_t)selected, hipMemcpyDeviceToHost, s));
        ++e->copies_d2h;
        if (counters_out) {
            HIPCHK(hipMemcpyAsync(counters_out, e->sel_counter.p, sizeof(long long) * (size_t)selected, hipMemcpyDeviceToHost, s));
            ++e->copies_d2h;
        }
    }
    if (point_mask) { HIPCHK(hipMemcpyAsync(point_mask, e->mask.p, n, hipMemcpyDeviceToHost, s)); ++e->copies_d2h; }
    int packed_n = packed_as;
    if (packed_as >= 0) { HIPCHK(hipMemcpyAsync(&packed_n, e->sel_pack_count.p, sizeof(int), hipMemcpyDeviceToHost, s)); ++e->copies_d2h; }
    HIPCHK(hipStreamSynchronize(s));
    if (packed_n != packed_as)
        return fail(MH_ERR_HIP, "greedy selection: the packed support set does not have the expected size");
    return MH_OK;
}

}

extern "C" {

int mh_set_transport(mh_engine* e, int rank, int world, mh_allgather_stream_fn stream_fn, mh_allgather_dev_fn host_fn, void* ctx)
{
    return guarded([&]() -> int {
    if (!e) return fail(MH_ERR_INVALID, "null engine");
    if (world < 1 || rank < 0 || rank >= world) return fail(MH_ERR_INVALID, "bad rank / world");
    if (stream_fn && host_fn) return fail(MH_ERR_INVALID, "give ONE transport: stream-ordered or host-synchronised");
    if (world > 1 && !stream_fn && !host_fn) return fail(MH_ERR_INVALID, "world > 1 needs a transport");
    if (e->xchg_pending) {
        HIPCHK(hipSetDevice(e->device));
        int rcq = quiesce(e);
        if (rcq) return rcq;
    }
    e->t_rank = rank; e->t_world = world; e->t_stream_fn = stream_fn; e->t_host_fn = host_fn; e->t_ctx = ctx;
    return MH_OK;
    });
}

int mh_select_greedy(mh_engine* e, double thr2, int need, int max_models, unsigned char* point_mask,
                     double* H_out, long long* counters_out, int* counts_out, int* selected_out, long long total_m)
{
    return guarded([&]() -> int {
    return select_greedy(e, thr2, need, max_models, point_mask, H_out, counters_out, counts_out, nullptr, selected_out, total_m, false);
    });
}

int mh_select_greedy_msac(mh_engine* e, double thr2, int need, int max_models, unsigned char* point_mask,
                          double* H_out, long long* counters_out, int* counts_out, int* weights_out, int* selected_out, long long total_m)
{
    return guarded([&]() -> int {
    return select_greedy(e, thr2, need, max_models, point_mask, H_out, counters_out, counts_out, weights_out, selected_out, total_m, true);
    });
}

int mh_select_best(mh_engine* e, long long total_m, long long* best_index, int* best_count)
{
    return guarded([&]() -> int {
    int rc = require_points(e);
    if (rc) return rc;
    const bool sharded = e->t_stream_fn || e->t_host_fn;
    const int world = sharded ? e->t_world : 1, rank = sharded ? e->t_rank : 0;
    if (e->m <= 0 && (!sharded || total_m <= 0)) return fail(MH_ERR_NOT_SET, "model set is empty");
    HIPCHK(reserve_counts(e, (size_t)e->m + 1));
    if (total_m <= 0) total_m = e->m;
    const int base = (int)(total_m / world), rem = (int)(total_m % world);
    const int longest = base + (rem ? 1 : 0);
    HIPCHK(e->h_best.ensure(4));
    const int* const h_best = e->h_best.h;
    hipStream_t s = e->stream;
    const bool fetch = best_index || best_count;
    auto result = [&]() -> int {
        if (h_best[2] != e->best_seq) return fail(MH_ERR_HIP, "best-model result is stale");
        if (h_best[3] != 0) return fail(MH_ERR_HIP, "mh_select_best: a rank reported an error");
        if (best_index) *best_index = h_best[1];
        if (best_count) *best_count = h_best[0];
        return MH_OK;
    };
    const bool same_generation = e->best_seq != 0 && e->best_models_seq == e->models_seq;
    if (same_generation && !e->counts_fresh) {
        if (!fetch) return MH_OK;
        rc = quiesce(e);
        if (rc) return rc;
        return result();
    }
    int local_rc = MH_OK;
    const char* local_msg = "";
    if (e->m != base + (rank < rem ? 1 : 0)) { local_rc = MH_ERR_INVALID; local_msg = "the resident model set is not this rank's shard of total_m hypotheses"; }
    else if (e->m > 0 && !e->counts_fresh) { local_rc = MH_ERR_NOT_SET; local_msg = "the batch has not been scored (mh_residual_matrix / mh_score / mh_cost_matrix)"; }
    if (local_rc != MH_OK && !sharded) return fail(local_rc, local_msg);
    if (local_rc != MH_OK) {
        HIPCHK(reserve_counts(e, (size_t)std::max(longest, e->m) + 1));
        if (longest > 0) HIPCHK(hipMemsetAsync(e->counts.p, 0xfe, sizeof(int) * (size_t)longest, s));
        e->counts_zeroed = false;
    }
    const int mine = local_rc != MH_OK ? longest : e->m;
    if (e->t_host_fn) {
        rc = join_xchg(e);
        if (rc) return rc;
        HIPCHK(e->sel_scores.reserve((size_t)std::max(longest, 1)));
        HIPCHK(e->sel_gathered.reserve((size_t)world * std::max(longest, 1)));
        HIPCHK(launch_pad_scores(e->counts.p, mine, longest, e->sel_scores.p, s));
        rc = exchange(e, e->sel_scores.p, e->sel_gathered.p, sizeof(int) * (size_t)longest, s);
        if (rc) return rc;
        HIPCHK(launch_best_fused(e->sel_gathered.p, world, longest, base, rem, e->h_best.d, nullptr, 0, s));
        ++e->best_seq;
        e->best_models_seq = e->models_seq;
        e->counts_fresh = false;
        if (fetch || local_rc != MH_OK) HIPCHK(hipStreamSynchronize(s));
    } else {
        rc = ensure_xchg_stream(e);
        if (rc) return rc;
        hipStream_t x = e->xchg_stream;
        if (sharded) {
            if (e->sel_gathered.cap < (size_t)world * longest) {
                rc = quiesce(e);
                if (rc) return rc;
                HIPCHK(e->sel_gathered.reserve((size_t)world * longest));
            }
            if (longest > mine)
                HIPCHK(hipMemsetAsync(e->counts.p + mine, 0xff, sizeof(int) * (size_t)(longest - mine), s));
        }
        HIPCHK(hipEventRecord(e->ev_sweep, s));
        HIPCHK(hipStreamWaitEvent(x, e->ev_sweep, 0));
        const bool rotate = !fetch && local_rc == MH_OK;
        int* clear = rotate ? e->counts.p : nullptr;
        const int clear_count = rotate ? (int)e->counts.cap : 0;
        {
            ScopedTimer t(e, MH_K_EXCHANGE, x);
            if (sharded) {
                rc = exchange(e, e->counts.p, e->sel_gathered.p, sizeof(int) * (size_t)longest, x);
                if (rc) return rc;
                HIPCHK(launch_best_fused(e->sel_gathered.p, world, longest, base, rem, e->h_best.d, clear, clear_count, x));
            } else {
                HIPCHK(launch_best_fused(e->counts.p, 1, e->m, 0, 0, e->h_best.d, clear, clear_count, x));
            }
        }
        const int par = (int)(e->xchg_calls % 3);
        HIPCHK(hipEventRecord(e->ev_x[par], x));
        ++e->xchg_calls;
        e->xchg_pending = true;
        ++e->best_seq;
        e->best_models_seq = e->models_seq;
        if (!rotate) {
            HIPCHK(hipStreamSynchronize(x));
            e->xchg_pending = false;
            e->counts_fresh = false;
        } else {
            const int wait = hand_counts_to_exchange(e, par);
            e->counts_fresh = false;
            HIPCHK(reserve_counts(e, (size_t)e->m + 1));
            if (wait >= 0) HIPCHK(hipStreamWaitEvent(s, e->ev_x[wait], 0));
        }
    }
    if (local_rc != MH_OK) return fail(local_rc, local_msg);
    if (fetch) return result();
    return MH_OK;
    });
}

int mh_select_best_msac(mh_engine* e, long long* best_index, int* best_weight, int* best_count)
{
    return guarded([&]() -> int {
    int rc = require_points(e);
    if (rc) return rc;
    if ((e->t_stream_fn || e->t_host_fn) && e->t_world > 1) return fail(MH_ERR_INVALID, "mh_select_best_msac: one rank only (the weights are not exchanged)");
    if (e->m <= 0) return fail(MH_ERR_NOT_SET, "model set is empty");
    if (e->weights_models_seq != e->models_seq || !e->weights.p) return fail(MH_ERR_NOT_SET, "the batch has no weights (mh_score_msac)");
    HIPCHK(e->h_best_w.ensure(4));
    const int* const h_best_w = e->h_best_w.h;
    const int seq = h_best_w[2];
    HIPCHK(launch_best_fused(e->weights.p, 1, e->m, 0, 0, e->h_best_w.d, nullptr, 0, e->stream));
    HIPCHK(hipStreamSynchronize(e->stream));
    if (h_best_w[2] != seq + 1 || h_best_w[3] != 0 || h_best_w[1] < 0 || h_best_w[1] >= e->m)
        return fail(MH_ERR_HIP, "mh_select_best_msac: no result from the arg-max");
    if (best_index) *best_index = h_best_w[1];
    if (best_weight) *best_weight = h_best_w[0];
    if (best_count) {
        HIPCHK(hipMemcpyAsync(best_count, e->weights_counts.p + h_best_w[1], sizeof(int), hipMemcpyDeviceToHost, e->stream));
        HIPCHK(hipStreamSynchronize(e->stream));
    }
    return MH_OK;
    });
}

int mh_get_score_stats(mh_engine* e, long long* pairs, long long* pairs_fp64, int reset)
{
    return guarded([&]() -> int {
    int rc = enter(e);
    if (rc) return rc;
    unsigned long long fb = 0;
    if (e->fb_pairs.p && e->score_pairs > 0) {
        HIPCHK(hipMemcpyAsync(&fb, e->fb_pairs.p, sizeof(fb), hipMemcpyDeviceToHost, e->stream));
        HIPCHK(hipStreamSynchronize(e->stream));
    }
    if (pairs) *pairs = e->score_pairs;
    if (pairs_fp64) *pairs_fp64 = (long long)fb + e->score_pairs_plain_fp64;
    if (reset) { e->score_pairs = 0; e->score_pairs_plain_fp64 = 0; }
    return MH_OK;
    });
}

int mh_get_copy_stats(mh_engine* e, long long* h2d, long long* d2h, int reset)
{
    return guarded([&]() -> int {
    if (!e) return fail(MH_ERR_INVALID, "null engine");
    if (h2d) *h2d = e->copies_h2d;
    if (d2h) *d2h = e->copies_d2h;
    if (reset) { e->copies_h2d = 0; e->copies_d2h = 0; }
    return MH_OK;
    });
}

}
```

### multi-h_amd/csrc/mh_kernels.hpp

```cpp
#pragma once
#include <hip/hip_runtime.h>
#include <cstdint>

namespace mh {

struct Points {
    const double* x1;
    const double* y1;
    const double* x2;
    const double* y2;
    int n;
    double xmin, xmax, ymin, ymax;
};

struct Affines {
    const double* a11;
    const double* a12;
    const double* a21;
    const double* a22;
};

struct Epipolar {
    double F[9];
    double ex, ey;
};

inline long long residual_ld(int n) { return ((long long)n + 15) & ~15ll; }

struct SweepLaunch {
    int slices = 0;
    bool contiguous = false;
    int swapxy = 0;
    bool counts_zeroed = false;
    int resident_grid = 0;
    int* resident_ctl = nullptr;
    int slice_major = 0;
};
hipError_t launch_residual(const Points& p, const double* H, int M, double thr2, double* R,
                           long long ldr, int* counts, int variant, hipStream_t s, const SweepLaunch& how);
int residual_workgroups_per_cu();
hipError_t launch_score(const Points& p, const double* H, int M, double thr2,
                        const unsigned char* mask, int* counts, int variant, hipStream_t s);
hipError_t launch_model32(const double* H, int M, double X, double Y, double Cmax, float* H32 , hipStream_t s);
hipError_t launch_score32(const Points& p, const double* H, const float* H32, int M, double thr2, double Cmax, const unsigned char* mask,
                          int* counts, unsigned long long* fallback_pairs, int tiling, hipStream_t s, int* resident_ctl = nullptr,
                          int cu_count = 256, int resident_slices = 0, int* occ_cache = nullptr);
hipError_t launch_cost32(const Points& p, const double* H, const float* H32, int M, double lambda, double thr2, double Cmax,
                         int* C, long long ldc, int* counts, hipStream_t s, int* resident_ctl = nullptr, int cu_count = 256,
                         int psplit_override = 0, int slice_major = 0, int batched = 0, int* occ_cache = nullptr, int rising = 0);
hipError_t launch_msac32(const Points& p, const double* H, const float* H32, int M, double thr2, double Cmax, const unsigned char* mask,
                         int* counts, int* weights, unsigned long long* fp64_pairs, hipStream_t s);
hipError_t launch_msac64(const Points& p, const double* H, int M, double thr2, const unsigned char* mask, int* counts, int* weights,
                         hipStream_t s);
hipError_t launch_inliers_of_model(const Points& p, const double* H, int idx, double thr2,
                                   int label_value, int* labels, hipStream_t s);
hipError_t launch_moments(const Points& p, const double* H, int M, double thr2, double* moments,
                          double* min_eig, hipStream_t s);

hipError_t launch_compat_select(const double* pts , const int* begin , int clusters,
                                const int* tri , const double* H ,
                                const unsigned char* ok, int trials, double* out , hipStream_t s);
hipError_t launch_compat_fit(const double* pts, const int* begin, int clusters, const int* tri, const double F[9], int trials,
                             double* H, unsigned char* ok, hipStream_t s);

struct Dlt4Local { const int* nbr = nullptr; int k = 0; int uniform_per_16 = 0; };
hipError_t launch_dlt4(const Points& p, unsigned long long seed, long long first, int M,
                       int* idx_out, double* H_out, hipStream_t s, int variant = 0 ,
                       Dlt4Local local = Dlt4Local{});

hipError_t launch_fund8(const Points& p, unsigned long long seed, long long first, int M,
                        int* idx_out , double* F_out, hipStream_t s);

hipError_t launch_fund7(const Points& p, unsigned long long seed, long long first, int M,
                        int* idx_out , double* F_out , int* nvalid_out , hipStream_t s);

hipError_t launch_ransac_stop(const int* counts , const int* nvalid , int S, int n, double confidence,
                              const double* F , double* F_win, int* out, hipStream_t s);
hipError_t launch_fund_mask(const Points& p, const double* F_in, double thr2, unsigned char* mask_out, int* count,
                            hipStream_t s, int metric);
hipError_t launch_sampson_score(const Points& p, const double* F, int M, double thr2, int* counts,
                                hipStream_t s, int metric);
hipError_t launch_fund_refit(const Points& p, const double* F_in, double thr2, double* F_out,
                             unsigned char* mask_out, int* count_out, hipStream_t s, int metric);

inline long long cost_ld(int n) { return ((long long)n + 31) & ~31ll; }
hipError_t launch_cost_matrix(const Points& p, const double* H, int M, double lambda, double thr2, int* C, long long ldc,
                              int* counts, hipStream_t s, int rising = 0);
hipError_t launch_data_cost(const Points& p, const double* H, int Nh, double lambda, double thr2,
                            int* cost, hipStream_t s, int rising = 0);

hipError_t launch_reestimate(const Points& p, const Affines& a, const int* labels, int Nh,
                             const Epipolar& ep, double* H, int* counts, hipStream_t s);

size_t reestimate_3pt_scratch_ints(int n, int Nh);
hipError_t launch_reestimate_3pt(const Points& p, const int* labels, int Nh, const Epipolar& ep, double* H, int* counts,
                                 int* scratch, hipStream_t s, int form = 0);

hipError_t launch_haf_point(const Points& p, const Affines& a, const Epipolar& ep, double locality,
                            double* H_out , double* feat_out ,
                            hipStream_t s);

hipError_t launch_haf_propose(const Points& p, const Affines& a, const Epipolar& ep, const int* nbr, int k, int members,
                              double thr2, long long first, int m, int stride, double* H_out, unsigned* used_out, hipStream_t s);

hipError_t launch_propose_3pt(const Points& p, const double F[9], unsigned long long seed, long long first, int M,
                              int* idx_out, double* H_out, hipStream_t s, Dlt4Local local = Dlt4Local{});

hipError_t launch_refine_points(const Points& p, const Affines& a, const double F[9], const double e1[2],
                                const double e2[2], const unsigned char* in_mask, unsigned char* keep,
                                double* out , unsigned char* reason , hipStream_t s,
                                int points_only = 0);

constexpr int MS_BATCH = 256;
struct MeanShiftWork {
    const double* data;
    int n, d;
    double* mean;
    int* votes;
    int* out;
    int* list;
    double* partial;
    int* partial_cnt;
};
struct MeanShiftResultBlock { int out[4]; double mean[16]; };
struct MeanShiftActive { unsigned char climb[MS_BATCH]; };
hipError_t launch_ms_climb(const MeanShiftWork& w, const MeanShiftActive& active, int n_active, const int* starts_dev, double band_sq,
                           double stop_thresh, int iterations, MeanShiftResultBlock* result_dev,
                           int* tickets , hipStream_t s);
hipError_t launch_ms_persist(const MeanShiftWork& w, const MeanShiftActive& active, int n_active, double band_sq, double stop_thresh,
                             int max_iters, int* ctl, double* partial2, int* partial_cnt2, MeanShiftResultBlock* result_dev,
                             hipStream_t s, unsigned long long* ticks = nullptr);
bool ms_persist_supported(int n, int d);
int ms_persist_occupancy(int d);
struct MeanShiftIndex {
    const double* rs;
    const int* order;
    const int* cell_start;
    int cells, coord;
    double lo, inv_w;
};
bool ms_indexed_supported(int n, int d);
int ms_index_max_cells();
hipError_t launch_ms_index_build(const double* data, int n, int d, const MeanShiftIndex& ix, int* count, int* cursor, int* cell_start,
                                 int* order, double* rs, hipStream_t s);
hipError_t launch_ms_indexed(const MeanShiftWork& w, const MeanShiftActive& active, int n_active, const int* starts_dev,
                             const MeanShiftIndex& ix, double band_sq, double stop_thresh, int max_iters, int dense_limit,
                             int keep, int* running, MeanShiftResultBlock* result_dev, hipStream_t s,
                             unsigned long long* ticks = nullptr);
hipError_t launch_ms_pack(const MeanShiftWork& w, int climbs, int longest, const int* offsets_dev, const int* lengths_dev, int* packed,
                          hipStream_t s);
hipError_t launch_ms_collect(const MeanShiftWork& w, int climbs, hipStream_t s);

struct Graph {
    const int* rowptr;
    const int* col;
    const int* w;
    const int* rev;
    int n, nnz;
    const int* order;
    const int* wsum;
};

constexpr int EXPAND_MAX_CTX = 16;
constexpr int EXPAND_FLAG_WORDS = 896;
constexpr int EXPAND_HOST_WORDS = 32;
constexpr int EXPAND_ACC_WORDS = 64 + 3 * 64 * 16;
constexpr int EXPAND_CORE_SHARDS = 8;

struct ExpandTuning {
    int relax_rounds = 0, push_cycles = 0, push_phases = 0, solve_grid = 0, push_mult = 0;
    int reduce_rounds = 0;
    int reduce_launches = 1;
    int cascade_iters = 0;
    long long barrier_timeout_ticks = 0;
    long long barrier_first_timeout_ticks = 0;
    int batch_min_labels = 0;
    int batch_spw = 0;
};

struct ExpandHooks { int inject_group = 0, inject_ctx = 0; };

struct ExpandWork {
    int* label = nullptr;
    int* cur_cost = nullptr;
    struct Ctx {
        int* cap;
        int* sent;
        int* excess;
        int* sink_cap;
        int* height;
        int* decided;
        unsigned char* took;
        int* core;
        int* flags;
        long long* acc;
        int* took_list;
    };
    int n_ctx = 1;
    Ctx ctx[EXPAND_MAX_CTX] = {};
    int* h_flags = nullptr;
    long long* h_acc = nullptr;
    int* h_flags_dev = nullptr;
    long long* h_acc_dev = nullptr;
    int* bctl = nullptr;
    int* h_batch = nullptr;
    int* h_batch_dev = nullptr;
    int* saved_flow = nullptr;
    int* saved_sink = nullptr;
    int* trace = nullptr;
    int trace_moves = 0;
    int detail_move = -1;
    int* comp_out = nullptr;
    int* comp_scratch = nullptr;
    int comp_moves = 0;
    ExpandTuning tune;
    ExpandHooks hooks;
};

struct ExpandStats {
    int cycles;
    long long energy;
    int moves, accepted;
    long long push_phases, relax_intervals;
    long long host_syncs;
    long long reduce_launches, flow_moves;
    long long launches;
    long long moves_run;
    long long moves_solved;
    long long core_sites, core_max;
    long long barriers, outer_iterations;
    double solve_ms;
    double barrier_ms, relax_ms, push_ms;
    double tail_ms;
    long long tail_rounds;
    double max_barrier_wait_ms;
    long long batches, batch_committed, batch_invalid, host_skipped, solo_moves;
    long long injected_discarded;
};

enum class ExpandStatus { ok, hip_error, overflow, barrier_timeout, no_convergence, too_many_sites };
struct ExpandResult { ExpandStatus status = ExpandStatus::ok; hipError_t hip = hipSuccess; };

hipError_t solver_blocks_per_cu(int* blocks);
ExpandResult run_expansion(const Graph& g, const int* cost , int L, int potts,
                           ExpandWork& w, int max_cycles, ExpandStats* st, hipStream_t s);
hipError_t launch_init_labeling(const int* cost, int L, int n, const int* init_or_null_dev,
                                int* label, int* cur_cost, hipStream_t s);
hipError_t launch_argmin_labels(const int* cost, int L, int n, int* label, long long* acc,
                                hipStream_t s);

hipError_t launch_sel_pack_points(const Points& p, const unsigned char* mask, double* cx1, double* cy1, double* cx2, double* cy2,
                                  int* count, hipStream_t s);
struct SelRecord { unsigned long long key; double H[9]; int err; int mode; };
constexpr int SEL_MODE_SYMMETRIC = 1 << 0;
constexpr int SEL_MODE_REFIT = 1 << 1;
constexpr int SEL_MODE_REFIT_3PT = 1 << 2;
constexpr int SEL_MODE_SAMPLER_LOCAL = 1 << 3;
constexpr int SEL_MODE_SAMPLER_K_SHIFT = 4;
constexpr int SEL_MODE_SAMPLER_UNIFORM_SHIFT = 10;
constexpr int SEL_MODE_BY_WEIGHT = 1 << 15;
constexpr int SEL_MODE_HAF = 1 << 16;
constexpr int SEL_MODE_HAF_MEMBERS_SHIFT = 17;
constexpr int SEL_MODE_P3 = 1 << 23;
static_assert(sizeof(SelRecord) == 88, "the exchanged record is 88 bytes");
hipError_t launch_sel_argmax(const int* counts, const int* weights, const int* orig, int Mc, int need, unsigned int my_off,
                             unsigned long long* key, int* scores_full, hipStream_t s);
hipError_t launch_sel_argmax_gathered(const int* gathered, int world, int longest, int base, int rem, unsigned long long* key,
                                      hipStream_t s);
hipError_t launch_sel_record(const int* counts, const int* weights, const int* orig, const double* Hs, int Mc, unsigned int my_off,
                             const unsigned long long* key_local, int err, int mode, SelRecord* record, hipStream_t s);
hipError_t launch_sel_compact(const int* counts, const int* weights, const int* orig, const double* Hs, int Mc, int need,
                              const SelRecord* records, int world, unsigned int my_off, int* next_orig, double* next_H, int* rec,
                              int* next_counts, int* next_weights, hipStream_t s);
hipError_t launch_sel_subtract(const int* carried_c, const int* left_c, const int* carried_w, const int* left_w, int Mc, int* counts,
                               int* weights, hipStream_t s);
hipError_t launch_sel_claim(const Points& p, const SelRecord* records, int world, const unsigned long long* key_check, double thr2,
                            unsigned char* mask, int* rec, double* sel_H, long long* sel_counter, int max_models, hipStream_t s,
                            bool by_weight, int symmetric, const double* refit, double* cx1, double* cy1, double* cx2, double* cy2);
hipError_t launch_sel_refit(const Points& p, const Affines& a, const Epipolar& ep, const SelRecord* records, int world, double thr2,
                            const unsigned char* mask, int* labels, double* refit, int* sum, int* label_count, hipStream_t s,
                            bool by_weight, int symmetric, int* scratch3);
hipError_t launch_sel_publish(int* rec, unsigned long long* keys, SelRecord* my_record, int* h_rec_dev, hipStream_t s);
hipError_t launch_best_fused(int* scores, int world, int longest, int base, int rem, int* h_best_dev, int* clear,
                             int clear_count, hipStream_t s);
hipError_t launch_pad_scores(const int* counts, int m, int longest, int* scores, hipStream_t s);

constexpr int KNN_MAX_SPLITS = 16;
hipError_t launch_knn(const Points& p, int k, int* nbr_out , int splits, float* part_d, int* part_i, hipStream_t s);
int knn_grid_cells(int n);
hipError_t launch_knn_grid(const Points& p, int k, int* nbr_out, int* cell_of, int* count, int* start, float* P4, int* orig, hipStream_t s);
hipError_t launch_radius_count(const Points& p, float r2, int* counts , hipStream_t s);
hipError_t launch_radius_fill(const Points& p, float r2, const int* rowptr , int* col , hipStream_t s);

constexpr int SYM_MAX_ROW = 1024;
hipError_t launch_hits_filter(const Points& p, int stride, float r2, int* col, int* err, hipStream_t s);
hipError_t launch_sym_count(int n, const int* rowptr, int stride, const int* col, int* deg, int* start , int* info, hipStream_t s);
hipError_t launch_sym_build(int n, const int* rowptr, int stride, const int* col, const int* start, int* cursor, int* raw,
                            int* mult, int* uniq, int* out_rowptr , int* info, hipStream_t s);
hipError_t launch_row_weight_sums(int n, const int* rowptr, const int* w, int* wsum, hipStream_t s);
hipError_t launch_sym_finish(int n, const int* start, const int* raw, const int* mult, const int* rowptr, int* col, int* w,
                             int* rev, hipStream_t s);

}
```

### multi-h_amd/csrc/msac32.hip

```cpp
#include "../../include/multih_hip.h"
#include "pretest32.hpp"

namespace mh {

template <int PPL, int MC, bool MASK>
__global__ void __launch_bounds__(256, 6)
k_msac32(const double* __restrict__ x1, const double* __restrict__ y1, const double* __restrict__ x2,
         const double* __restrict__ y2, int N, const double* __restrict__ H, const float* __restrict__ H32, int M,
         double thr2, float thr2_f, float c_thr, float k1, int* __restrict__ counts, int* __restrict__ weights,
         const unsigned char* __restrict__ mask, int psplit, unsigned long long* __restrict__ fp64_pairs)
{
    constexpr int WAVE_PTS = 64 * PPL, TILE = 4 * WAVE_PTS;
    const int lane = threadIdx.x & 63;
    const int wave = __builtin_amdgcn_readfirstlane(threadIdx.x >> 6);
    const int m0 = blockIdx.x * MC;
    __shared__ float4 s_m[MC * 4];
    stage_model32<MC, 256>(s_m, H32, m0, M);
    __syncthreads();
    const float vthr2 = vgpr_copy(thr2_f), vc_thr = vgpr_copy(c_thr), vk1 = vgpr_copy(k1);
    int cnt = 0, wgt = 0;
    unsigned long long fb = 0;
    for (int base = blockIdx.y * TILE; base < N; base += psplit * TILE) {
        const int n0 = base + wave * WAVE_PTS + lane * PPL;
        float fx[PPL], fy[PPL], gx[PPL], gy[PPL], cx[PPL];
        unsigned long long okm[PPL];
        load_tile32<PPL, MASK>(x1, y1, x2, y2, N, n0, mask, fx, fy, gx, gy, cx, okm);
#pragma unroll 1
        for (int mi = 0; mi < MC; ++mi) {
            const int m = m0 + mi;
            if (m >= M) break;
            const Model32 mod = model32_from_lds(s_m, mi);
            unsigned long long farq[PPL], all_far = ~0ull;
#pragma unroll
            for (int q = 0; q < PPL; ++q) {
                farq[q] = cheap_far(mod, fx[q], fy[q], gx[q], gy[q], vk1);
                all_far &= farq[q];
            }
            if (all_far == ~0ull) continue;
            int c_m = 0, w_lane = 0;
#pragma unroll
            for (int q = 0; q < PPL; ++q) {
                if (farq[q] == ~0ull) continue;
                asm volatile("; msac32: full bound");
                const Bound32 b = full_bound(mod, fx[q], fy[q], gx[q], gy[q], cx[q], vthr2, vc_thr);
                const unsigned long long above = __builtin_amdgcn_ballot_w64(b.t >= 0.0f);
                const unsigned long long out = (b.trust & b.clear & above) | farq[q];
                const unsigned long long cand = ~out & okm[q];
                if (cand == 0ull) continue;
                bool in64 = false;
                if ((cand >> lane) & 1ull) {
                    const double* h = H + 9 * (size_t)m;
                    const int n = n0 + q;
                    const double e2 = fwd_d2(h[0], h[1], h[2], h[3], h[4], h[5], h[6], h[7], h[8], x1[n], y1[n], x2[n], y2[n]);
                    in64 = e2 < thr2;
                    w_lane += data_term<false>(e2, thr2, (double)MH_MSAC_SCALE, 0);
                    ++fb;
                }
                c_m += __builtin_popcountll(__builtin_amdgcn_ballot_w64(in64));
            }
            if (c_m > 0) {
                cnt = lane_acc_add(cnt, mi, c_m);
                wgt = lane_acc_add(wgt, mi, __builtin_amdgcn_readfirstlane(wave_sum(w_lane)));
            }
        }
    }
    finish32<MC, 4, 2>({ cnt, wgt }, threadIdx.x >> 6, m0, M, psplit, { counts, weights });
    add_fp64_pairs(fp64_pairs, fb);
}

template <bool MASK>
__global__ void __launch_bounds__(256)
k_msac64(const double* __restrict__ x1, const double* __restrict__ y1, const double* __restrict__ x2,
         const double* __restrict__ y2, int N, const double* __restrict__ H, int M, double thr2, int* __restrict__ counts,
         int* __restrict__ weights, const unsigned char* __restrict__ mask, int psplit)
{
    constexpr int MC = 64, TILE = 256;
    const int lane = threadIdx.x & 63;
    const int wave = __builtin_amdgcn_readfirstlane(threadIdx.x >> 6);
    const int m0 = blockIdx.x * MC;
    __shared__ double s_h[MC * 9];
    stage_model64<MC, 256>(s_h, H, m0, M);
    __syncthreads();
    int cnt = 0, wgt = 0;
    for (int base = blockIdx.y * TILE; base < N; base += psplit * TILE) {
        const int n = base + wave * 64 + lane;
        bool ok = n < N;
        const double px = ok ? x1[n] : 1.0, py = ok ? y1[n] : 1.0, qx = ok ? x2[n] : 1.0, qy = ok ? y2[n] : 1.0;
        if (MASK && ok) ok = mask[n] != 0;
        if (__builtin_amdgcn_ballot_w64(ok) == 0ull) continue;
#pragma unroll 1
        for (int mi = 0; mi < MC; ++mi) {
            if (m0 + mi >= M) break;
            const double* h = s_h + 9 * mi;
            const double d2 = fwd_d2(h[0], h[1], h[2], h[3], h[4], h[5], h[6], h[7], h[8], px, py, qx, qy);
            const bool in = ok && d2 < thr2;
            const unsigned long long inl = __builtin_amdgcn_ballot_w64(in);
            if (inl == 0ull) continue;
            const int w = in ? data_term<false>(d2, thr2, (double)MH_MSAC_SCALE, 0) : 0;
            cnt = lane_acc_add(cnt, mi, __builtin_popcountll(inl));
            wgt = lane_acc_add(wgt, mi, __builtin_amdgcn_readfirstlane(wave_sum(w)));
        }
    }
    finish32<MC, 4, 2>({ cnt, wgt }, threadIdx.x >> 6, m0, M, psplit, { counts, weights });
}

hipError_t launch_msac32(const Points& p, const double* H, const float* H32, int M, double thr2, double Cmax, const unsigned char* mask,
                         int* counts, int* weights, unsigned long long* fp64_pairs, hipStream_t s)
{
    if (M <= 0 || p.n <= 0) return hipSuccess;
    constexpr int PPL = 4, MC = 64;
    const int gx = (M + MC - 1) / MC, ntiles = (p.n + 256 * PPL - 1) / (256 * PPL);
    int psplit = 0;
    hipError_t e = point_slices(gx, ntiles, 16, 4, 0, M, counts, weights, s, &psplit);
    if (e != hipSuccess) return e;
    const Pretest32Launch c(thr2, Cmax, 1.0);
    if (mask) hipLaunchKernelGGL((k_msac32<PPL, MC, true>), dim3(gx, psplit), dim3(256), 0, s, p.x1, p.y1, p.x2, p.y2, p.n, H, H32, M, thr2, c.thr2_f, c.c_thr, c.k1, counts, weights, mask, psplit, fp64_pairs);
    else hipLaunchKernelGGL((k_msac32<PPL, MC, false>), dim3(gx, psplit), dim3(256), 0, s, p.x1, p.y1, p.x2, p.y2, p.n, H, H32, M, thr2, c.thr2_f, c.c_thr, c.k1, counts, weights, mask, psplit, fp64_pairs);
    return hipGetLastError();
}

hipError_t launch_msac64(const Points& p, const double* H, int M, double thr2, const unsigned char* mask, int* counts, int* weights,
                         hipStream_t s)
{
    if (M <= 0 || p.n <= 0) return hipSuccess;
    const int gx = (M + 63) / 64, ntiles = (p.n + 255) / 256;
    int psplit = 0;
    hipError_t e = point_slices(gx, ntiles, 64, 4, 0, M, counts, weights, s, &psplit);
    if (e != hipSuccess) return e;
    if (mask) hipLaunchKernelGGL(k_msac64<true>, dim3(gx, psplit), dim3(256), 0, s, p.x1, p.y1, p.x2, p.y2, p.n, H, M, thr2, counts, weights, mask, psplit);
    else hipLaunchKernelGGL(k_msac64<false>, dim3(gx, psplit), dim3(256), 0, s, p.x1, p.y1, p.x2, p.y2, p.n, H, M, thr2, counts, weights, mask, psplit);
    return hipGetLastError();
}

}
```

### multi-h_amd/csrc/pretest32.hpp

```cpp
#pragma once
#include "mh_kernels.hpp"
#include "mh_device.hpp"

#include <cmath>

namespace mh {

constexpr float U32 = 5.9604644775390625e-08f;


__device__ __forceinline__ float vgpr_copy(float v)
{
    float r;
    asm volatile("v_mov_b32 %0, %1" : "=v"(r) : "s"(v));
    return r;
}

__device__ __forceinline__ int lane_acc_add(int acc, int mi, int add)
{
    const int v = __builtin_amdgcn_readlane(acc, mi) + add;
    asm("s_mov_b32 m0, %2\n\ts_nop 0\n\tv_writelane_b32 %0, %1, m0" : "+v"(acc) : "s"(v), "s"(mi) : "m0");
    return acc;
}

template <typename T>
__device__ __forceinline__ T wave_sum(T v)
{
#pragma unroll
    for (int o = 32; o >= 1; o >>= 1) v += __shfl_xor(v, o, 64);
    return v;
}

__device__ __forceinline__ void add_fp64_pairs(unsigned long long* __restrict__ counter, unsigned long long fb)
{
    if (counter) {
        fb = wave_sum(fb);
        if ((threadIdx.x & 63) == 0 && fb) atomicAdd(counter, fb);
    }
}

struct Model32 {
    float h0, h1, h2, h3, h4, h5, h6, h7, h8, es, en, tau, a25;
};

template <int MC, int THREADS>
__device__ __forceinline__ void stage_model32(float4* s_m, const float* __restrict__ H32, int m0, int M)
{
    for (int i = threadIdx.x; i < MC * 4; i += THREADS) {
        const size_t g = (size_t)m0 * 4 + i;
        s_m[i] = g < (size_t)M * 4 ? reinterpret_cast<const float4*>(H32)[g] : make_float4(0.f, 0.f, 0.f, NAN);
    }
}

template <int MC, int THREADS>
__device__ __forceinline__ void stage_model64(double* s_h, const double* __restrict__ H, int m0, int M)
{
    for (int i = threadIdx.x; i < MC * 9; i += THREADS) {
        const size_t g = (size_t)m0 * 9 + i;
        s_h[i] = g < (size_t)M * 9 ? H[g] : 0.0;
    }
}

__device__ __forceinline__ Model32 model32_from_lds(const float4* s_m, int mi)
{
    const float4 ma = s_m[4 * mi], mb = s_m[4 * mi + 1], mc = s_m[4 * mi + 2], md = s_m[4 * mi + 3];
    return { ma.x, ma.y, ma.z, ma.w, mb.x, mb.y, mb.z, mb.w, mc.x, mc.y, mc.z, mc.w, md.x };
}

template <int PPL, typename Each>
__device__ __forceinline__ void load_points32(const double* __restrict__ x1, const double* __restrict__ y1, const double* __restrict__ x2,
                                              const double* __restrict__ y2, int N, int n0, float (&fx)[PPL], float (&fy)[PPL],
                                              float (&gx)[PPL], float (&gy)[PPL], Each&& each)
{
#pragma unroll
    for (int q = 0; q < PPL; ++q) {
        const int n = n0 + q;
        const bool ok = n < N;
        const double px = ok ? x1[n] : 1.0, py = ok ? y1[n] : 1.0, qx = ok ? x2[n] : 1.0, qy = ok ? y2[n] : 1.0;
        each(q, ok, px, py, qx, qy);
        fx[q] = (float)px; fy[q] = (float)py; gx[q] = (float)qx; gy[q] = (float)qy;
    }
}

template <int PPL, bool MASK>
__device__ __forceinline__ void load_tile32(const double* __restrict__ x1, const double* __restrict__ y1, const double* __restrict__ x2,
                                            const double* __restrict__ y2, int N, int n0, const unsigned char* __restrict__ mask,
                                            float (&fx)[PPL], float (&fy)[PPL], float (&gx)[PPL], float (&gy)[PPL], float (&cx)[PPL],
                                            unsigned long long (&okm)[PPL])
{
    load_points32<PPL>(x1, y1, x2, y2, N, n0, fx, fy, gx, gy, [&](int q, bool ok, double, double, double, double) {
        if (MASK && ok) ok = mask[n0 + q] != 0;
        okm[q] = __builtin_amdgcn_ballot_w64(ok);
    });
#pragma unroll
    for (int q = 0; q < PPL; ++q) cx[q] = U32 * fmaxf(fabsf(gx[q]), fabsf(gy[q])) * 1.0000002f;
}

__device__ __forceinline__ unsigned long long cheap_far(const Model32& m, float fx, float fy, float gx, float gy, float vk1)
{
    const float s = __builtin_fmaf(m.h6, fx, __builtin_fmaf(m.h7, fy, m.h8));
    const float nx = __builtin_fmaf(m.h0, fx, __builtin_fmaf(m.h1, fy, m.h2));
    const float ny = __builtin_fmaf(m.h3, fx, __builtin_fmaf(m.h4, fy, m.h5));
    const float wx = __builtin_fmaf(gx, s, -nx), wy = __builtin_fmaf(gy, s, -ny);
    const float W = fmaxf(fabsf(wx), fabsf(wy));
    return __builtin_amdgcn_ballot_w64(fabsf(s) >= m.tau) & __builtin_amdgcn_ballot_w64(W >= fmaxf(vk1 * fabsf(s), m.a25));
}

struct Bound32 {
    unsigned long long trust, clear;
    float t;
};

__device__ __forceinline__ Bound32 full_bound(const Model32& m, float fx, float fy, float gx, float gy, float cx, float vthr2, float vc_thr)
{
    const float s = __builtin_fmaf(m.h6, fx, __builtin_fmaf(m.h7, fy, m.h8));
    const float nx = __builtin_fmaf(m.h0, fx, __builtin_fmaf(m.h1, fy, m.h2));
    const float ny = __builtin_fmaf(m.h3, fx, __builtin_fmaf(m.h4, fy, m.h5));
    const float r = __builtin_amdgcn_rcpf(s);
    const float uu = nx * r, vv = ny * r;
    const float dx = gx - uu, dy = gy - vv;
    const float w = fmaxf(fabsf(dx), fabsf(dy));
    const float d2 = __builtin_fmaf(dx, dx, dy * dy);
    const float mm = fmaxf(fabsf(uu), fabsf(vv));
    const float eq = __builtin_fmaf(__builtin_fmaf(mm, m.es, m.en), fabsf(r), (5.0f * U32) * mm);
    const float E = __builtin_fmaf(1.01f * U32, w, eq + cx);
    const float B0 = __builtin_fmaf(2.02f * E, __builtin_fmaf(2.0f, w, E), vc_thr);
    const float t = d2 - vthr2;
    return { __builtin_amdgcn_ballot_w64(fabsf(s) >= m.tau), __builtin_amdgcn_ballot_w64(fabsf(t) > B0), t };
}

template <int MC, int WAVES, int NS>
__device__ __forceinline__ void sums_to_global(int (&s_sum)[NS][WAVES][MC], int m0, int M, int psplit, int* const (&out)[NS])
{
    __syncthreads();
    if (threadIdx.x < MC && m0 + (int)threadIdx.x < M) {
        const int t = threadIdx.x;
#pragma unroll
        for (int k = 0; k < NS; ++k) {
            int c = 0;
#pragma unroll
            for (int w = 0; w < WAVES; ++w) c += s_sum[k][w][t];
            if (psplit == 1) out[k][m0 + t] = c;
            else atomicAdd(&out[k][m0 + t], c);
        }
    }
}

template <int MC, int WAVES, int NS>
__device__ __forceinline__ void finish32(const int (&acc)[NS], int wave, int m0, int M, int psplit, int* const (&out)[NS])
{
    static_assert(MC <= 64, "lane mi of a wave accumulates model m0 + mi");
    const int lane = threadIdx.x & 63;
    __shared__ int s_sum[NS][WAVES][MC];
    if (lane < MC) {
#pragma unroll
        for (int k = 0; k < NS; ++k) s_sum[k][wave][lane] = acc[k];
    }
    sums_to_global<MC, WAVES, NS>(s_sum, m0, M, psplit, out);
}

template <typename WG>
__device__ __forceinline__ void resident_items(int* __restrict__ ctl, int gx, int psplit, int nitems, int slice_major, WG&& wg)
{
    __shared__ int s_item;
#pragma unroll 1
    for (;;) {
        if (threadIdx.x == 0) s_item = atomicAdd(&ctl[0], 1);
        __syncthreads();
        const int item = s_item;
        if (item >= nitems) break;
        int bx, by;
        if (slice_major) { bx = item / psplit; by = item - bx * psplit; }
        else { by = item / gx; bx = item - by * gx; }
        wg(bx, by);
        __syncthreads();
    }
    if (threadIdx.x == 0 && atomicAdd(&ctl[1], 1) == (int)gridDim.x - 1) {
        ctl[1] = 0;
        __hip_atomic_store(&ctl[0], 0, __ATOMIC_RELEASE, __HIP_MEMORY_SCOPE_AGENT);
    }
}


struct Pretest32Launch {
    float thr2_f, c_thr, k1;
    Pretest32Launch(double thr2, double Cmax, double far_factor)
        : thr2_f((float)thr2),
          c_thr((float)(std::fabs((double)thr2_f - thr2) * 1.01 + 3.5 * (double)U32 * std::fabs(thr2) * 1.01) + 1e-45f),
          k1((float)(std::fmax(1.12 * far_factor * std::sqrt(std::fabs(thr2)), 25.4 * (double)U32 * Cmax) * (1.0 + 1e-6)) + 1e-30f)
    {
    }
};

inline int clamp_slices(int ps, int ntiles)
{
    if (ps > ntiles) ps = ntiles;
    return ps < 1 ? 1 : ps;
}

inline hipError_t point_slices(int gx, int ntiles, int many_tiles, int few, int chosen, int M, int* sums, int* sums2, hipStream_t s, int* psplit)
{
    *psplit = clamp_slices(chosen > 0 ? chosen : gx < 1024 ? (2048 + gx - 1) / gx : (ntiles >= many_tiles ? few : 1), ntiles);
    for (int* a : { sums, sums2 })
        if (a && *psplit > 1) {
            hipError_t e = hipMemsetAsync(a, 0, sizeof(int) * (size_t)M, s);
            if (e != hipSuccess) return e;
        }
    return hipSuccess;
}

inline int resident_grid(const void* kernel, int threads, int* occ_cache, int cu_count, int choice, int gx, int ntiles, int* slices)
{
    int per_cu = occ_cache ? *occ_cache : -1;
    if (per_cu < 0) {
        int q = 0;
        per_cu = hipOccupancyMaxActiveBlocksPerMultiprocessor(&q, kernel, threads, 0) == hipSuccess ? q : 0;
        if (per_cu > 0 && occ_cache) *occ_cache = per_cu;
    }
    *slices = clamp_slices(choice > 0 ? choice : (37500 + gx - 1) / gx, ntiles);
    const int grid = per_cu * cu_count;
    return grid > 0 && gx * *slices > grid ? grid : 0;
}

}
```

### multi-h_amd/csrc/score32.hip

```cpp
#include "pretest32.hpp"

namespace mh {

__global__ void __launch_bounds__(256)
k_model32(const double* __restrict__ H, int M, double X, double Y, double Cmax, float* __restrict__ out)
{
    const int m = blockIdx.x * 256 + threadIdx.x;
    if (m >= M) return;
    const double* h = H + 9 * (size_t)m;
    float* o = out + 16 * (size_t)m;
    bool ok = true;
    for (int q = 0; q < 9; ++q) {
        ok = ok && fabs(h[q]) < 0x1p100;
        o[q] = (float)h[q];
    }
    const double u = 0x1p-24;
    const double as = fabs(h[6]) * X + fabs(h[7]) * Y + fabs(h[8]);
    const double an = fmax(fabs(h[0]) * X + fabs(h[1]) * Y + fabs(h[2]), fabs(h[3]) * X + fabs(h[4]) * Y + fabs(h[5]));
    const double es = 5.0 * u * as, en = 5.0 * u * an;
    ok = ok && es >= 0x1p-80 && en >= 0x1p-80 && as < 0x1p100 && an < 0x1p100;
    const double up = 1.0 + 0x1p-22;
    o[9] = (float)(1.1 * es * up);
    o[10] = (float)(1.1 * en * up);
    o[11] = ok ? (float)(64.0 * es * up) : NAN;
    o[12] = (float)(25.2 * 1.01 * (Cmax * es + en) * up);
    o[13] = o[14] = o[15] = 0.f;
}

template <int PPL, int MC, bool MASK>
__device__ __forceinline__ void
score32_wg(const double* __restrict__ x1, const double* __restrict__ y1, const double* __restrict__ x2,
           const double* __restrict__ y2, int N, const double* __restrict__ H, const float* __restrict__ H32, int M,
           double thr2, float thr2_f, float c_thr, float k1, int* __restrict__ counts, const unsigned char* __restrict__ mask,
           int psplit, unsigned long long* __restrict__ fallback_pairs, const int bx, const int by)
{
    constexpr int WAVE_PTS = 64 * PPL, TILE = 4 * WAVE_PTS;
    const int lane = threadIdx.x & 63;
    const int wave = __builtin_amdgcn_readfirstlane(threadIdx.x >> 6);
    const int m0 = bx * MC;
    __shared__ float4 s_m[MC * 4];
    stage_model32<MC, 256>(s_m, H32, m0, M);
    __syncthreads();
    const float vthr2 = vgpr_copy(thr2_f), vc_thr = vgpr_copy(c_thr), vk1 = vgpr_copy(k1);
    int cnt = 0;
    unsigned long long fb = 0;
    for (int base = by * TILE; base < N; base += psplit * TILE) {
        const int n0 = base + wave * WAVE_PTS + lane * PPL;
        float fx[PPL], fy[PPL], gx[PPL], gy[PPL], cx[PPL];
        unsigned long long okm[PPL];
        load_tile32<PPL, MASK>(x1, y1, x2, y2, N, n0, mask, fx, fy, gx, gy, cx, okm);
#pragma unroll 1
        for (int mi = 0; mi < MC; ++mi) {
            const int m = m0 + mi;
            if (m >= M) break;
            const Model32 mod = model32_from_lds(s_m, mi);
            unsigned long long farq[PPL], all_far = ~0ull;
#pragma unroll
            for (int q = 0; q < PPL; ++q) {
                farq[q] = cheap_far(mod, fx[q], fy[q], gx[q], gy[q], vk1);
                all_far &= farq[q];
            }
            int c_m = 0;
            if (all_far != ~0ull) {
#pragma unroll
                for (int q = 0; q < PPL; ++q) {
                    if (farq[q] == ~0ull) continue;
                    asm volatile("; score32: full bound");
                    const Bound32 b = full_bound(mod, fx[q], fy[q], gx[q], gy[q], cx[q], vthr2, vc_thr);
                    const unsigned long long below = __builtin_amdgcn_ballot_w64(b.t < 0.0f);
                    const unsigned long long decided = (b.trust & b.clear) | farq[q];
                    unsigned long long inl = b.trust & b.clear & below;
                    if (decided != ~0ull) {
                        const bool need = ((decided >> lane) & 1ull) == 0ull;
                        bool in64 = false;
                        if (need) {
                            const double* h = H + 9 * (size_t)m;
                            const int n = n0 + q < N ? n0 + q : N - 1;
                            const double e2 = fwd_d2(h[0], h[1], h[2], h[3], h[4], h[5], h[6], h[7], h[8], x1[n], y1[n], x2[n], y2[n]);
                            in64 = e2 < thr2;
                            ++fb;
                        }
                        inl |= __builtin_amdgcn_ballot_w64(in64);
                    }
                    c_m += __builtin_popcountll(inl & okm[q]);
                }
            }
            cnt = lane_acc_add(cnt, mi, c_m);
        }
    }
    __shared__ int s_cnt[4][MC];
    if (lane < MC) s_cnt[wave][lane] = cnt;
    __syncthreads();
    if (threadIdx.x < MC && m0 + (int)threadIdx.x < M) {
        const int t = threadIdx.x;
        const int c = s_cnt[0][t] + s_cnt[1][t] + s_cnt[2][t] + s_cnt[3][t];
        if (psplit == 1) counts[m0 + t] = c;
        else atomicAdd(&counts[m0 + t], c);
    }
    add_fp64_pairs(fallback_pairs, fb);
}

template <int PPL, int MC, bool MASK, int MINW = 1>
__global__ void __launch_bounds__(256, MINW)
k_score32(const double* __restrict__ x1, const double* __restrict__ y1, const double* __restrict__ x2,
          const double* __restrict__ y2, int N, const double* __restrict__ H, const float* __restrict__ H32, int M,
          double thr2, float thr2_f, float c_thr, float k1, int* __restrict__ counts, const unsigned char* __restrict__ mask,
          int psplit, unsigned long long* __restrict__ fallback_pairs)
{
    score32_wg<PPL, MC, MASK>(x1, y1, x2, y2, N, H, H32, M, thr2, thr2_f, c_thr, k1, counts, mask, psplit, fallback_pairs, blockIdx.x, blockIdx.y);
}

template <int PPL, int MC, bool MASK, int MINW = 1>
__global__ void __launch_bounds__(256, MINW)
k_score32_resident(const double* __restrict__ x1, const double* __restrict__ y1, const double* __restrict__ x2,
                   const double* __restrict__ y2, int N, const double* __restrict__ H, const float* __restrict__ H32, int M,
                   double thr2, float thr2_f, float c_thr, float k1, int* __restrict__ counts, const unsigned char* __restrict__ mask,
                   int psplit, unsigned long long* __restrict__ fallback_pairs, int gx, int nitems, int* __restrict__ ctl)
{
    resident_items(ctl, gx, psplit, nitems, 0, [&](int bx, int by) {
        score32_wg<PPL, MC, MASK>(x1, y1, x2, y2, N, H, H32, M, thr2, thr2_f, c_thr, k1, counts, mask, psplit, fallback_pairs, bx, by);
    });
}

__device__ __forceinline__ void wave_lds_handover()
{
    asm volatile("" ::: "memory");
    __builtin_amdgcn_wave_barrier();
    asm volatile("" ::: "memory");
}

#define MH_COST32_ARGS                                                                                                          \
    const double* __restrict__ x1, const double* __restrict__ y1, const double* __restrict__ x2, const double* __restrict__ y2, \
    int N, const double* __restrict__ H, const float* __restrict__ H32, int M, double lam, double T, double thr2, float k1,     \
    int* __restrict__ C, long long ldc, int* __restrict__ counts, int psplit
#define MH_COST32_PASS x1, y1, x2, y2, N, H, H32, M, lam, T, thr2, k1, C, ldc, counts, psplit

template <int MC, int WAVES, bool RISING>
__device__ __forceinline__ void
cost32_wg(MH_COST32_ARGS, const int bx, const int by)
{
    constexpr int PPL = 4, WAVE_PTS = 64 * PPL, TILE = WAVES * WAVE_PTS, THREADS = 64 * WAVES;
    const int lane = threadIdx.x & 63;
    const int wave = __builtin_amdgcn_readfirstlane(threadIdx.x >> 6);
    const int m0 = bx * MC;
    __shared__ float4 s_m[MC * 4];
    __shared__ double s_h[MC * 9];
    __shared__ double s_p[WAVES * PPL * 4 * 64];
    stage_model32<MC, THREADS>(s_m, H32, m0, M);
    stage_model64<MC, THREADS>(s_h, H, m0, M);
    __syncthreads();
    double* wave_p = s_p + (size_t)wave * (PPL * 4 * 64);
    double* my_p = wave_p + lane;
    __shared__ unsigned char s_list[WAVES * 64 * PPL];
    __shared__ int s_c[WAVES * 64 * PPL];
    unsigned char* my_list = s_list + wave * (64 * PPL);
    int* my_c = s_c + wave * (64 * PPL);
    const float vk1 = vgpr_copy(k1);
    const int beyond = 2 * (int)round(lam * T);
    int cnt = 0;
    for (int base = by * TILE; base < N; base += psplit * TILE) {
        const int base_n = base + wave * WAVE_PTS;
        const int n0 = base_n + lane * PPL;
        float fx[PPL], fy[PPL], gx[PPL], gy[PPL];
        load_points32<PPL>(x1, y1, x2, y2, N, n0, fx, fy, gx, gy, [&](int q, bool, double px, double py, double qx, double qy) {
            my_p[(q * 4 + 0) * 64] = px; my_p[(q * 4 + 1) * 64] = py; my_p[(q * 4 + 2) * 64] = qx; my_p[(q * 4 + 3) * 64] = qy;
        });
        wave_lds_handover();
#pragma unroll 1
        for (int mi = 0; mi < MC; ++mi) {
            const int m = m0 + mi;
            if (m >= M) break;
            const Model32 mod = model32_from_lds(s_m, mi);
            int c[PPL];
            unsigned long long nearq[PPL], any_near = 0ull;
#pragma unroll
            for (int q = 0; q < PPL; ++q) {
                nearq[q] = ~cheap_far(mod, fx[q], fy[q], gx[q], gy[q], vk1);
                any_near |= nearq[q];
                c[q] = beyond;
            }
            int c_m = 0;
            if (any_near) {
                asm volatile("; cost32: FP64 pairs");
                int npairs = 0;
#pragma unroll
                for (int q = 0; q < PPL; ++q) {
                    if ((nearq[q] >> lane) & 1ull) {
                        const int pos = npairs + (int)__builtin_amdgcn_mbcnt_hi((unsigned)(nearq[q] >> 32), __builtin_amdgcn_mbcnt_lo((unsigned)nearq[q], 0u));
                        my_list[pos] = (unsigned char)(q * 64 + lane);
                    }
                    npairs += __builtin_popcountll(nearq[q]);
                }
                wave_lds_handover();
                const double* h = s_h + 9 * mi;
                const double h0d = h[0], h1d = h[1], h2d = h[2], h3d = h[3], h4d = h[4], h5d = h[5], h6d = h[6], h7d = h[7], h8d = h[8];
                for (int p0 = 0; p0 < npairs; p0 += 64) {
                    bool in64 = false;
                    if (p0 + lane < npairs) {
                        const int id = my_list[p0 + lane], q2 = id >> 6, l2 = id & 63;
                        const double* pp = wave_p + (q2 * 4) * 64 + l2;
                        const double d2 = fwd_d2(h0d, h1d, h2d, h3d, h4d, h5d, h6d, h7d, h8d, pp[0], pp[64], pp[128], pp[192]);
                        my_c[id] = data_term<RISING>(d2, T, lam, beyond);
                        in64 = (base_n + l2 * PPL + q2 < N) && d2 < thr2;
                    }
                    c_m += __builtin_popcountll(__builtin_amdgcn_ballot_w64(in64));
                }
                wave_lds_handover();
#pragma unroll
                for (int q = 0; q < PPL; ++q)
                    if ((nearq[q] >> lane) & 1ull) c[q] = my_c[q * 64 + lane];
                wave_lds_handover();
            }
            int* dst = C + (size_t)m * ldc + n0;
            if (n0 + 3 < N) {
                typedef int i4v __attribute__((ext_vector_type(4)));
                const i4v v = { c[0], c[1], c[2], c[3] };
                __builtin_nontemporal_store(v, reinterpret_cast<i4v*>(dst));
            }
            else
                for (int q = 0; q < PPL; ++q) if (n0 + q < N) dst[q] = c[q];
            if (any_near) cnt = lane_acc_add(cnt, mi, c_m);
        }
    }
    finish32<MC, WAVES, 1>({ cnt }, wave, m0, M, psplit, { counts });
}

template <int MC, int WAVES, bool RISING>
__device__ __forceinline__ void
cost32_wg_batched(MH_COST32_ARGS, const int bx, const int by)
{
    constexpr int PPL = 4, WAVE_PTS = 64 * PPL, TILE = WAVES * WAVE_PTS, THREADS = 64 * WAVES, LCAP = 64 + 64 * PPL;
    static_assert(MC <= 64, "a list entry carries the model in 6 bits");
    const int lane = threadIdx.x & 63;
    const int wave = __builtin_amdgcn_readfirstlane(threadIdx.x >> 6);
    const int m0 = bx * MC;
    __shared__ float4 s_m[MC * 4];
    __shared__ double s_h[MC * 9];
    __shared__ double s_p[WAVES * PPL * 4 * 64];
    __shared__ unsigned short s_list[WAVES * LCAP];
    __shared__ int s_cnt[1][WAVES][MC];
    stage_model32<MC, THREADS>(s_m, H32, m0, M);
    stage_model64<MC, THREADS>(s_h, H, m0, M);
    for (int i = threadIdx.x; i < WAVES * MC; i += THREADS) (&s_cnt[0][0][0])[i] = 0;
    __syncthreads();
    double* wave_p = s_p + (size_t)wave * (PPL * 4 * 64);
    double* my_p = wave_p + lane;
    unsigned short* my_list = s_list + wave * LCAP;
    const float vk1 = vgpr_copy(k1);
    const int beyond = 2 * (int)round(lam * T);
    typedef int i4v __attribute__((ext_vector_type(4)));
    const i4v vbeyond = { beyond, beyond, beyond, beyond };
    for (int base = by * TILE; base < N; base += psplit * TILE) {
        const int base_n = base + wave * WAVE_PTS;
        const int n0 = base_n + lane * PPL;
        float fx[PPL], fy[PPL], gx[PPL], gy[PPL];
        load_points32<PPL>(x1, y1, x2, y2, N, n0, fx, fy, gx, gy, [&](int q, bool, double px, double py, double qx, double qy) {
            my_p[(q * 4 + 0) * 64] = px; my_p[(q * 4 + 1) * 64] = py; my_p[(q * 4 + 2) * 64] = qx; my_p[(q * 4 + 3) * 64] = qy;
        });
        wave_lds_handover();
        auto evaluate = [&](int first, int count) {
            if (first + lane < count) {
                const int id = my_list[first + lane], mi2 = id >> 8, q2 = (id >> 6) & 3, l2 = id & 63;
                const double* h = s_h + 9 * mi2;
                const double* pp = wave_p + (q2 * 4) * 64 + l2;
                const double d2 = fwd_d2(h[0], h[1], h[2], h[3], h[4], h[5], h[6], h[7], h[8], pp[0], pp[64], pp[128], pp[192]);
                const int cost = data_term<RISING>(d2, T, lam, beyond);
                const int n = base_n + l2 * PPL + q2;
                if (n < N) {
                    C[(size_t)(m0 + mi2) * ldc + n] = cost;
                    if (d2 < thr2) atomicAdd(&s_cnt[0][wave][mi2], 1);
                }
            }
        };
        int nlist = 0;
#pragma unroll 1
        for (int mi = 0; mi < MC; ++mi) {
            const int m = m0 + mi;
            if (m >= M) break;
            const Model32 mod = model32_from_lds(s_m, mi);
            unsigned long long nearq[PPL], any_near = 0ull;
#pragma unroll
            for (int q = 0; q < PPL; ++q) {
                nearq[q] = ~cheap_far(mod, fx[q], fy[q], gx[q], gy[q], vk1);
                any_near |= nearq[q];
            }
            int* dst = C + (size_t)m * ldc + n0;
            if (n0 + 3 < N) *reinterpret_cast<i4v*>(dst) = vbeyond;
            else
                for (int q = 0; q < PPL; ++q) if (n0 + q < N) dst[q] = beyond;
            if (any_near) {
                asm volatile("; cost32: near pairs to the list");
#pragma unroll
                for (int q = 0; q < PPL; ++q) {
                    if ((nearq[q] >> lane) & 1ull) {
                        const int pos = nlist + (int)__builtin_amdgcn_mbcnt_hi((unsigned)(nearq[q] >> 32), __builtin_amdgcn_mbcnt_lo((unsigned)nearq[q], 0u));
                        my_list[pos] = (unsigned short)((mi << 8) | (q << 6) | lane);
                    }
                    nlist += __builtin_popcountll(nearq[q]);
                }
                if (nlist >= 64) {
                    wave_lds_handover();
                    asm volatile("s_waitcnt vmcnt(0)" ::: "memory");
                    do {
                        nlist -= 64;
                        evaluate(nlist, nlist + 64);
                    } while (nlist >= 64);
                    wave_lds_handover();
                }
            }
        }
        if (nlist > 0) {
            wave_lds_handover();
            asm volatile("s_waitcnt vmcnt(0)" ::: "memory");
            for (int p0 = 0; p0 < nlist; p0 += 64) evaluate(p0, nlist);
        }
        wave_lds_handover();
    }
    sums_to_global<MC, WAVES, 1>(s_cnt, m0, M, psplit, { counts });
}

template <int MC, int WAVES, bool BATCH, bool RISING>
__device__ __forceinline__ void
cost32_item(MH_COST32_ARGS, const int bx, const int by)
{
    if (BATCH) cost32_wg_batched<MC, WAVES, RISING>(MH_COST32_PASS, bx, by);
    else cost32_wg<MC, WAVES, RISING>(MH_COST32_PASS, bx, by);
}

template <int MC, int WAVES, bool BATCH>
__global__ void __launch_bounds__(64 * WAVES)
k_cost32(MH_COST32_ARGS)
{
    cost32_item<MC, WAVES, BATCH, false>(MH_COST32_PASS, blockIdx.x, blockIdx.y);
}

template <int MC, int WAVES, bool BATCH>
__global__ void __launch_bounds__(64 * WAVES)
k_cost32_resident(MH_COST32_ARGS, int gx, int nitems, int* __restrict__ ctl, int slice_major)
{
    resident_items(ctl, gx, psplit, nitems, slice_major, [&](int bx, int by) { cost32_item<MC, WAVES, BATCH, false>(MH_COST32_PASS, bx, by); });
}

template <int MC, int WAVES, bool BATCH>
__global__ void __launch_bounds__(64 * WAVES)
k_rising32(MH_COST32_ARGS)
{
    cost32_item<MC, WAVES, BATCH, true>(MH_COST32_PASS, blockIdx.x, blockIdx.y);
}

template <int MC, int WAVES, bool BATCH>
__global__ void __launch_bounds__(64 * WAVES)
k_rising32_resident(MH_COST32_ARGS, int gx, int nitems, int* __restrict__ ctl, int slice_major)
{
    resident_items(ctl, gx, psplit, nitems, slice_major, [&](int bx, int by) { cost32_item<MC, WAVES, BATCH, true>(MH_COST32_PASS, bx, by); });
}
#undef MH_COST32_ARGS
#undef MH_COST32_PASS

template <bool BATCH, bool RISING>
static hipError_t launch_cost32_t(const Points& p, const double* H, const float* H32, int M, double lambda, double thr2, double Cmax,
                                  int* C, long long ldc, int* counts, hipStream_t s, int* resident_ctl, int cu_count, int psplit_override, int slice_major,
                                  int* occ_cache)
{
    if (M <= 0 || p.n <= 0) return hipSuccess;
    constexpr int MC = 32;
    constexpr int WAVES = 8;
    const int gx = (M + MC - 1) / MC, ntiles = (p.n + 256 * WAVES - 1) / (256 * WAVES);
    const float k1 = Pretest32Launch(thr2, Cmax, 2.25).k1;
    const auto k_plain = RISING ? k_rising32<MC, WAVES, BATCH> : k_cost32<MC, WAVES, BATCH>;
    const auto k_resident = RISING ? k_rising32_resident<MC, WAVES, BATCH> : k_cost32_resident<MC, WAVES, BATCH>;
    int psplit = 0;
    const int grid = resident_ctl ? resident_grid((const void*)k_resident, 64 * WAVES, occ_cache, cu_count, psplit_override, gx, ntiles, &psplit) : 0;
    hipError_t e = point_slices(gx, ntiles, 8, 2, grid > 0 ? psplit : 0, M, counts, nullptr, s, &psplit);
    if (e != hipSuccess) return e;
    if (grid > 0)
        hipLaunchKernelGGL(k_resident, dim3(grid), dim3(64 * WAVES), 0, s, p.x1, p.y1, p.x2, p.y2, p.n, H, H32, M,
                           100.0 / lambda, thr2 * 81.0 / 16.0, thr2, k1, C, ldc, counts, psplit, gx, gx * psplit, resident_ctl, slice_major);
    else
        hipLaunchKernelGGL(k_plain, dim3(gx, psplit), dim3(64 * WAVES), 0, s, p.x1, p.y1, p.x2, p.y2, p.n, H, H32, M, 100.0 / lambda,
                           thr2 * 81.0 / 16.0, thr2, k1, C, ldc, counts, psplit);
    return hipGetLastError();
}

hipError_t launch_cost32(const Points& p, const double* H, const float* H32, int M, double lambda, double thr2, double Cmax,
                         int* C, long long ldc, int* counts, hipStream_t s, int* resident_ctl, int cu_count, int psplit_override, int slice_major,
                         int batched, int* occ_cache, int rising)
{
#ifdef MH_TUNING
    if (batched && rising) return launch_cost32_t<true, true>(p, H, H32, M, lambda, thr2, Cmax, C, ldc, counts, s, resident_ctl, cu_count, psplit_override, slice_major, nullptr);
    if (batched) return launch_cost32_t<true, false>(p, H, H32, M, lambda, thr2, Cmax, C, ldc, counts, s, resident_ctl, cu_count, psplit_override, slice_major, nullptr);
#else
    (void)batched;
    slice_major = 0;
#endif
    if (rising) return launch_cost32_t<false, true>(p, H, H32, M, lambda, thr2, Cmax, C, ldc, counts, s, resident_ctl, cu_count, psplit_override, slice_major, occ_cache);
    return launch_cost32_t<false, false>(p, H, H32, M, lambda, thr2, Cmax, C, ldc, counts, s, resident_ctl, cu_count, psplit_override, slice_major, occ_cache);
}

hipError_t launch_model32(const double* H, int M, double X, double Y, double Cmax, float* H32, hipStream_t s)
{
    if (M <= 0) return hipSuccess;
    hipLaunchKernelGGL(k_model32, dim3((M + 255) / 256), dim3(256), 0, s, H, M, X, Y, Cmax, H32);
    return hipGetLastError();
}

template <int PPL, int MC, int MINW = 1>
static hipError_t launch_score32_t(const Points& p, const double* H, const float* H32, int M, double thr2, double Cmax, const unsigned char* mask,
                                   int* counts, unsigned long long* fallback_pairs, hipStream_t s, int* resident_ctl = nullptr,
                                   int cu_count = 256, int resident_slices = 0, int* occ_cache = nullptr)
{
    const int gx = (M + MC - 1) / MC, ntiles = (p.n + 256 * PPL - 1) / (256 * PPL);
    int psplit = 0, resident = 0;
    if (resident_ctl && resident_slices != 0 && !mask)
        resident = resident_grid((const void*)k_score32_resident<PPL, MC, false, MINW>, 256, occ_cache, cu_count, resident_slices, gx, ntiles, &psplit);
    hipError_t e = point_slices(gx, ntiles, 16, 4, resident > 0 ? psplit : 0, M, counts, nullptr, s, &psplit);
    if (e != hipSuccess) return e;
    const Pretest32Launch c(thr2, Cmax, 1.0);
    if (resident > 0) {
        hipLaunchKernelGGL((k_score32_resident<PPL, MC, false, MINW>), dim3(resident), dim3(256), 0, s, p.x1, p.y1, p.x2, p.y2, p.n, H, H32, M, thr2, c.thr2_f,
                           c.c_thr, c.k1, counts, mask, psplit, fallback_pairs, gx, gx * psplit, resident_ctl);
        return hipGetLastError();
    }
    if (mask) hipLaunchKernelGGL((k_score32<PPL, MC, true, MINW>), dim3(gx, psplit), dim3(256), 0, s, p.x1, p.y1, p.x2, p.y2, p.n, H, H32, M, thr2, c.thr2_f, c.c_thr, c.k1, counts, mask, psplit, fallback_pairs);
    else hipLaunchKernelGGL((k_score32<PPL, MC, false, MINW>), dim3(gx, psplit), dim3(256), 0, s, p.x1, p.y1, p.x2, p.y2, p.n, H, H32, M, thr2, c.thr2_f, c.c_thr, c.k1, counts, mask, psplit, fallback_pairs);
    return hipGetLastError();
}

hipError_t launch_score32(const Points& p, const double* H, const float* H32, int M, double thr2, double Cmax, const unsigned char* mask,
                          int* counts, unsigned long long* fallback_pairs, int tiling, hipStream_t s, int* resident_ctl, int cu_count,
                          int resident_slices, int* occ_cache)
{
    if (M <= 0 || p.n <= 0) return hipSuccess;
    if (tiling == 0 && resident_ctl && resident_slices != 0)
        return launch_score32_t<4, 64, 6>(p, H, H32, M, thr2, Cmax, mask, counts, fallback_pairs, s, resident_ctl, cu_count, resident_slices, occ_cache);
#ifdef MH_TUNING
    switch (tiling) {
    case 1: return launch_score32_t<4, 16>(p, H, H32, M, thr2, Cmax, mask, counts, fallback_pairs, s);
    case 2: return launch_score32_t<8, 32>(p, H, H32, M, thr2, Cmax, mask, counts, fallback_pairs, s);
    case 3: return launch_score32_t<4, 32>(p, H, H32, M, thr2, Cmax, mask, counts, fallback_pairs, s);
    case 4: return launch_score32_t<8, 64>(p, H, H32, M, thr2, Cmax, mask, counts, fallback_pairs, s);
    case 5: return launch_score32_t<6, 32>(p, H, H32, M, thr2, Cmax, mask, counts, fallback_pairs, s);
    case 6: return launch_score32_t<8, 16>(p, H, H32, M, thr2, Cmax, mask, counts, fallback_pairs, s);
    case 7: return launch_score32_t<4, 64>(p, H, H32, M, thr2, Cmax, mask, counts, fallback_pairs, s);
    case 8: return launch_score32_t<4, 32, 5>(p, H, H32, M, thr2, Cmax, mask, counts, fallback_pairs, s);
    case 9: return launch_score32_t<4, 32, 6>(p, H, H32, M, thr2, Cmax, mask, counts, fallback_pairs, s);
    case 10: return launch_score32_t<4, 32, 8>(p, H, H32, M, thr2, Cmax, mask, counts, fallback_pairs, s);
    case 11: return launch_score32_t<2, 32, 8>(p, H, H32, M, thr2, Cmax, mask, counts, fallback_pairs, s);
    case 12: return launch_score32_t<4, 64, 6>(p, H, H32, M, thr2, Cmax, mask, counts, fallback_pairs, s);
    case 13: return launch_score32_t<4, 32>(p, H, H32, M, thr2, Cmax, mask, counts, fallback_pairs, s);
    case 14: return launch_score32_t<4, 64, 5>(p, H, H32, M, thr2, Cmax, mask, counts, fallback_pairs, s);
    case 15: return launch_score32_t<4, 64, 8>(p, H, H32, M, thr2, Cmax, mask, counts, fallback_pairs, s);
    case 16: return launch_score32_t<2, 64, 8>(p, H, H32, M, thr2, Cmax, mask, counts, fallback_pairs, s);
    default: break;
    }
#endif
    return launch_score32_t<4, 64, 6>(p, H, H32, M, thr2, Cmax, mask, counts, fallback_pairs, s);
}

}
```

### multi-h_amd/csrc/select.hip

```cpp
#include "../../include/multih_hip.h"
#include "mh_device.hpp"
#include "mh_kernels.hpp"

namespace mh {

__device__ __forceinline__ unsigned long long sel_key(int rank, unsigned int counter)
{
    return ((unsigned long long)(unsigned int)rank << 32) | (unsigned long long)(0xffffffffu - counter);
}

__device__ __forceinline__ unsigned long long wg_max_u64(unsigned long long k)
{
#pragma unroll
    for (int m = 32; m >= 1; m >>= 1) { const unsigned long long o = __shfl_xor(k, m, 64); k = o > k ? o : k; }
    __shared__ unsigned long long s[4];
    if ((threadIdx.x & 63) == 0) s[threadIdx.x >> 6] = k;
    __syncthreads();
    unsigned long long b = s[0];
    for (int w = 1; w < 4; ++w) b = s[w] > b ? s[w] : b;
    return b;
}

__device__ __forceinline__ int wave_append(bool on, int* __restrict__ count)
{
    const unsigned long long m = __ballot(on);
    const int lane = threadIdx.x & 63;
    int base = 0;
    if (lane == 0 && m) base = atomicAdd(count, (int)__popcll(m));
    base = __shfl(base, 0, 64);
    return base + (int)__popcll(m & ((1ull << lane) - 1ull));
}

__device__ __forceinline__ double sel_d2(const double* __restrict__ h, int symmetric, double x1, double y1, double x2, double y2)
{
    double d2 = fwd_d2(h[0], h[1], h[2], h[3], h[4], h[5], h[6], h[7], h[8], x1, y1, x2, y2);
    if (symmetric) {
        const double a0 = h[4] * h[8] - h[5] * h[7], a1 = h[2] * h[7] - h[1] * h[8], a2 = h[1] * h[5] - h[2] * h[4];
        const double a3 = h[5] * h[6] - h[3] * h[8], a4 = h[0] * h[8] - h[2] * h[6], a5 = h[2] * h[3] - h[0] * h[5];
        const double a6 = h[3] * h[7] - h[4] * h[6], a7 = h[1] * h[6] - h[0] * h[7], a8 = h[0] * h[4] - h[1] * h[3];
        d2 = d2 + fwd_d2(a0, a1, a2, a3, a4, a5, a6, a7, a8, x2, y2, x1, y1);
    }
    return d2;
}

template <bool BY_WEIGHT>
__global__ void __launch_bounds__(256)
k_sel_argmax(const int* __restrict__ counts, const int* __restrict__ weights, const int* __restrict__ orig, int Mc, int need,
             unsigned int my_off, unsigned long long* __restrict__ key, int* __restrict__ scores_full)
{
    const int c = blockIdx.x * 256 + threadIdx.x;
    unsigned long long k = 0;
    if (c < Mc) {
        const int o = orig ? orig[c] : c;
        const int cnt = counts[c];
        const int rank = BY_WEIGHT ? weights[c] : cnt;
        const bool eligible = cnt >= need;
        if (eligible) k = sel_key(rank, my_off + (unsigned int)o);
        if (scores_full) scores_full[o] = eligible ? rank : -1;
    }
    const unsigned long long b = wg_max_u64(k);
    if (threadIdx.x == 0 && b) atomicMax(key, b);
}

__global__ void __launch_bounds__(256)
k_sel_argmax_gathered(const int* __restrict__ gathered, int world, int longest, int base, int rem,
                      unsigned long long* __restrict__ key)
{
    const int c = blockIdx.x * 256 + threadIdx.x;
    unsigned long long k = 0;
    if (c < world * longest && gathered[c] >= 0) {
        const int r = c / longest, j = c - r * longest;
        k = sel_key(gathered[c], (unsigned int)(r * base + (r < rem ? r : rem) + j));
    }
    const unsigned long long b = wg_max_u64(k);
    if (threadIdx.x == 0 && b) atomicMax(key, b);
}

__global__ void __launch_bounds__(256)
k_sel_record(const int* __restrict__ rank, const int* __restrict__ orig, const double* __restrict__ Hs, int Mc,
             unsigned int my_off, const unsigned long long* __restrict__ key_local, int err, int mode, SelRecord* __restrict__ record)
{
    const int c = blockIdx.x * 256 + threadIdx.x;
    const unsigned long long kl = *key_local;
    if (c == 0) { record->err = err; record->mode = mode; }
    if (c >= Mc || !kl) return;
    const int o = orig ? orig[c] : c;
    if (sel_key(rank[c], my_off + (unsigned int)o) != kl) return;
    record->key = kl;
    const double* h = Hs + 9 * (size_t)c;
    for (int q = 0; q < 9; ++q) record->H[q] = h[q];
}

__device__ __forceinline__ unsigned long long sel_winner(const SelRecord* __restrict__ records, int world, int* rank_out)
{
    unsigned long long kg = 0;
    int wr = 0;
    for (int r = 0; r < world; ++r) { const unsigned long long k = records[r].key; if (k > kg) { kg = k; wr = r; } }
    if (rank_out) *rank_out = wr;
    return kg;
}

template <bool BY_WEIGHT>
__global__ void __launch_bounds__(256)
k_sel_compact(const int* __restrict__ counts, const int* __restrict__ weights, const int* __restrict__ orig,
              const double* __restrict__ Hs, int Mc, int need, const SelRecord* __restrict__ records, int world, unsigned int my_off,
              int* __restrict__ next_orig, double* __restrict__ next_H, int* __restrict__ rec, int* __restrict__ next_counts,
              int* __restrict__ next_weights)
{
    const int c = blockIdx.x * 256 + threadIdx.x;
    const unsigned long long kg = sel_winner(records, world, nullptr);
    bool keep = false;
    int o = 0, cnt_c = 0, rank_c = 0;
    if (c < Mc) {
        o = orig ? orig[c] : c;
        cnt_c = counts[c];
        rank_c = BY_WEIGHT ? weights[c] : cnt_c;
        const bool is_winner = kg && sel_key(rank_c, my_off + (unsigned int)o) == kg;
        keep = cnt_c >= need && !is_winner;
    }
    __shared__ int s_cnt, s_base;
    if (threadIdx.x == 0) s_cnt = 0;
    __syncthreads();
    int off = 0;
    if (keep) off = atomicAdd(&s_cnt, 1);
    __syncthreads();
    if (threadIdx.x == 0 && s_cnt > 0) s_base = atomicAdd(&rec[2], s_cnt);
    __syncthreads();
    if (keep) {
        const int pos = s_base + off;
        next_orig[pos] = o;
        if (next_counts) {
            next_counts[pos] = cnt_c;
            if (BY_WEIGHT) next_weights[pos] = rank_c;
        }
        const double* h = Hs + 9 * (size_t)c;
        for (int q = 0; q < 9; ++q) next_H[9 * (size_t)pos + q] = h[q];
    }
}

template <bool BY_WEIGHT>
__global__ void __launch_bounds__(256)
k_sel_claim(const double* __restrict__ x1, const double* __restrict__ y1, const double* __restrict__ x2,
            const double* __restrict__ y2, int N, const SelRecord* __restrict__ records, int world,
            const unsigned long long* __restrict__ key_check, double thr2, unsigned char* __restrict__ mask,
            int* __restrict__ rec, double* __restrict__ sel_H, long long* __restrict__ sel_counter, int max_models, int symmetric,
            const double* __restrict__ refit ,
            double* __restrict__ cx1, double* __restrict__ cy1, double* __restrict__ cx2, double* __restrict__ cy2 )
{
    int wr = 0;
    const unsigned long long kg = sel_winner(records, world, &wr);
    const int best = (int)(kg >> 32);
    const unsigned int pos = 0xffffffffu - (unsigned int)(kg & 0xffffffffull);
    const int n = blockIdx.x * 256 + threadIdx.x;
    if (n == 0) {
        rec[0] = kg ? best : -1;
        rec[1] = (int)pos;
        int err = 0;
        for (int r = 0; r < world; ++r) if (records[r].err) err = records[r].err;
        if (key_check && *key_check != kg) err = 2;
        for (int r = 1; r < world; ++r) if (records[r].mode != records[0].mode) err = 3;
        if (err) rec[4] = err;
    }
    if (!kg) return;
    const int sel = rec[3];
    if (sel >= max_models) return;
    const double* hyp = records[wr].H;
    const double* h = hyp;
    if (refit && refit[9] >= (double)best) {
        bool finite = true;
        for (int q = 0; q < 9; ++q) finite = finite && fabs(refit[q]) < 0x1p1000;
        if (finite) h = refit;
    }
    if (n == 0) {
        for (int q = 0; q < 9; ++q) sel_H[9 * (size_t)sel + q] = h[q];
        sel_counter[sel] = (long long)pos;
        if (!BY_WEIGHT) rec[6] = best;
    }
    bool leaves = false, own = false;
    if (n < N && mask[n]) {
        leaves = sel_d2(h, symmetric, x1[n], y1[n], x2[n], y2[n]) < thr2;
        if (BY_WEIGHT) own = h != hyp ? sel_d2(hyp, symmetric, x1[n], y1[n], x2[n], y2[n]) < thr2 : leaves;
        if (leaves) mask[n] = 0;
    }
    if (BY_WEIGHT) (void)wave_append(own, &rec[6]);
    const int at = wave_append(leaves, &rec[5]);
    if (leaves && cx1) { cx1[at] = x1[n]; cy1[at] = y1[n]; cx2[at] = x2[n]; cy2[at] = y2[n]; }
}

template <bool BY_WEIGHT>
__global__ void __launch_bounds__(256)
k_sel_subtract(const int* __restrict__ carried_c, const int* __restrict__ left_c, const int* __restrict__ carried_w,
               const int* __restrict__ left_w, int Mc, int* __restrict__ counts, int* __restrict__ weights)
{
    const int c = blockIdx.x * 256 + threadIdx.x;
    if (c >= Mc) return;
    counts[c] = carried_c[c] - left_c[c];
    if (BY_WEIGHT) weights[c] = carried_w[c] - left_w[c];
}

__global__ void __launch_bounds__(256)
k_sel_winner_labels(const double* __restrict__ x1, const double* __restrict__ y1, const double* __restrict__ x2,
                    const double* __restrict__ y2, int N, const SelRecord* __restrict__ records, int world, double thr2,
                    const unsigned char* __restrict__ mask, int* __restrict__ labels, double* __restrict__ refit, int symmetric)
{
    int wr = 0;
    const unsigned long long kg = sel_winner(records, world, &wr);
    const int n = blockIdx.x * 256 + threadIdx.x;
    const double* h = records[wr].H;
    if (n == 0) {
        for (int q = 0; q < 9; ++q) refit[q] = h[q];
        refit[9] = 0.0;
    }
    if (n >= N) return;
    int lab = -1;
    if (kg && mask[n] && sel_d2(h, symmetric, x1[n], y1[n], x2[n], y2[n]) < thr2) lab = 0;
    labels[n] = lab;
}

template <bool BY_WEIGHT>
__global__ void __launch_bounds__(256)
k_sel_measure(const double* __restrict__ x1, const double* __restrict__ y1, const double* __restrict__ x2,
              const double* __restrict__ y2, int N, double thr2, const unsigned char* __restrict__ mask,
              const double* __restrict__ refit, int* __restrict__ sum, int symmetric)
{
    const int n = blockIdx.x * 256 + threadIdx.x;
    bool in = false;
    int w = 0;
    if (n < N && mask[n]) {
        const double d2 = sel_d2(refit, symmetric, x1[n], y1[n], x2[n], y2[n]);
        in = d2 < thr2;
        if (BY_WEIGHT) w = data_term<false>(d2, thr2, (double)MH_MSAC_SCALE, 0);
    }
    const unsigned long long m = __ballot(in);
    if (!BY_WEIGHT) {
        if ((threadIdx.x & 63) == 0 && m) atomicAdd(sum, (int)__popcll(m));
        return;
    }
    if (m == 0ull) return;
#pragma unroll
    for (int o = 32; o >= 1; o >>= 1) w += __shfl_xor(w, o, 64);
    if ((threadIdx.x & 63) == 0) atomicAdd(sum, w);
}

__global__ void k_sel_measure_finish(const int* __restrict__ sum, double* __restrict__ refit)
{
    if (threadIdx.x == 0) refit[9] = (double)*sum;
}

__global__ void k_sel_publish(int* __restrict__ rec, unsigned long long* __restrict__ keys, SelRecord* __restrict__ my_record,
                              int* __restrict__ h_rec)
{
    if (threadIdx.x != 0) return;
    h_rec[0] = rec[0]; h_rec[1] = rec[1]; h_rec[2] = rec[2]; h_rec[4] = rec[4]; h_rec[5] = rec[5]; h_rec[6] = rec[6];
    if (rec[0] >= 0) rec[3] += 1;
    h_rec[3] = rec[3];
    rec[2] = 0;
    rec[5] = 0;
    rec[6] = 0;
    keys[0] = 0; keys[1] = 0;
    my_record->key = 0;
}

__global__ void __launch_bounds__(1024)
k_best_fused(int* scores, int world, int longest, int base, int rem, int* __restrict__ h_best, int* clear, int clear_count)
{
    const int total = world * longest;
    unsigned long long k = 0;
    int err = 0;
    for (int c = threadIdx.x; c < total; c += 1024) {
        const int v = scores[c];
        if (v < 0) { err |= v < -1 ? 1 : 0; continue; }
        const int r = world > 1 ? c / longest : 0, j = c - r * longest;
        const unsigned long long kk = sel_key(v, (unsigned int)(r * base + (r < rem ? r : rem) + j));
        k = kk > k ? kk : k;
    }
#pragma unroll
    for (int m = 32; m >= 1; m >>= 1) { const unsigned long long o = __shfl_xor(k, m, 64); k = o > k ? o : k; }
    err = __ballot(err != 0) != 0ull ? 1 : 0;
    __shared__ unsigned long long s_k[16];
    __shared__ int s_err[16];
    if ((threadIdx.x & 63) == 0) { s_k[threadIdx.x >> 6] = k; s_err[threadIdx.x >> 6] = err; }
    __syncthreads();
    if (threadIdx.x == 0) {
        unsigned long long b = 0;
        int any = 0;
        for (int w = 0; w < 16; ++w) { b = s_k[w] > b ? s_k[w] : b; any |= s_err[w]; }
        h_best[0] = b ? (int)(b >> 32) : -1;
        h_best[1] = (int)(0xffffffffu - (unsigned int)(b & 0xffffffffull));
        h_best[3] = any;
        h_best[2] += 1;
    }
    if (clear) for (int c = threadIdx.x; c < clear_count; c += 1024) clear[c] = 0;
}

__global__ void __launch_bounds__(256)
k_pad_scores(const int* __restrict__ counts, int m, int longest, int* __restrict__ scores)
{
    const int c = blockIdx.x * 256 + threadIdx.x;
    if (c < longest) scores[c] = c < m ? counts[c] : -1;
}

__global__ void __launch_bounds__(256)
k_sel_pack_points(Points p, const unsigned char* __restrict__ mask, double* __restrict__ cx1, double* __restrict__ cy1,
                  double* __restrict__ cx2, double* __restrict__ cy2, int* __restrict__ count)
{
    const int i = blockIdx.x * 256 + threadIdx.x;
    const bool on = i < p.n && mask[i] != 0;
    const int pos = wave_append(on, count);
    if (on) { cx1[pos] = p.x1[i]; cy1[pos] = p.y1[i]; cx2[pos] = p.x2[i]; cy2[pos] = p.y2[i]; }
}

hipError_t launch_sel_pack_points(const Points& p, const unsigned char* mask, double* cx1, double* cy1, double* cx2, double* cy2,
                                  int* count, hipStream_t s)
{
    hipError_t he = hipMemsetAsync(count, 0, sizeof(int), s);
    if (he != hipSuccess) return he;
    hipLaunchKernelGGL(k_sel_pack_points, dim3((p.n + 255) / 256), dim3(256), 0, s, p, mask, cx1, cy1, cx2, cy2, count);
    return hipGetLastError();
}

hipError_t launch_sel_argmax(const int* counts, const int* weights, const int* orig, int Mc, int need, unsigned int my_off,
                             unsigned long long* key, int* scores_full, hipStream_t s)
{
    if (Mc <= 0) return hipSuccess;
    const auto k = weights ? k_sel_argmax<true> : k_sel_argmax<false>;
    hipLaunchKernelGGL(k, dim3((Mc + 255) / 256), dim3(256), 0, s, counts, weights, orig, Mc, need, my_off, key, scores_full);
    return hipGetLastError();
}

hipError_t launch_sel_argmax_gathered(const int* gathered, int world, int longest, int base, int rem, unsigned long long* key,
                                      hipStream_t s)
{
    if (world * longest <= 0) return hipSuccess;
    hipLaunchKernelGGL(k_sel_argmax_gathered, dim3((world * longest + 255) / 256), dim3(256), 0, s, gathered, world, longest,
                       base, rem, key);
    return hipGetLastError();
}

hipError_t launch_sel_record(const int* counts, const int* weights, const int* orig, const double* Hs, int Mc, unsigned int my_off,
                             const unsigned long long* key_local, int err, int mode, SelRecord* record, hipStream_t s)
{
    hipLaunchKernelGGL(k_sel_record, dim3(Mc > 0 ? (Mc + 255) / 256 : 1), dim3(256), 0, s, weights ? weights : counts, orig, Hs, Mc,
                       my_off, key_local, err, mode, record);
    return hipGetLastError();
}

hipError_t launch_sel_compact(const int* counts, const int* weights, const int* orig, const double* Hs, int Mc, int need,
                              const SelRecord* records, int world, unsigned int my_off, int* next_orig, double* next_H, int* rec,
                              int* next_counts, int* next_weights, hipStream_t s)
{
    if (Mc <= 0) return hipSuccess;
    const auto k = weights ? k_sel_compact<true> : k_sel_compact<false>;
    hipLaunchKernelGGL(k, dim3((Mc + 255) / 256), dim3(256), 0, s, counts, weights, orig, Hs, Mc, need, records, world, my_off,
                       next_orig, next_H, rec, next_counts, next_weights);
    return hipGetLastError();
}

hipError_t launch_sel_subtract(const int* carried_c, const int* left_c, const int* carried_w, const int* left_w, int Mc, int* counts,
                               int* weights, hipStream_t s)
{
    if (Mc <= 0) return hipSuccess;
    const auto k = weights ? k_sel_subtract<true> : k_sel_subtract<false>;
    hipLaunchKernelGGL(k, dim3((Mc + 255) / 256), dim3(256), 0, s, carried_c, left_c, carried_w, left_w, Mc, counts, weights);
    return hipGetLastError();
}

hipError_t launch_sel_claim(const Points& p, const SelRecord* records, int world, const unsigned long long* key_check, double thr2,
                            unsigned char* mask, int* rec, double* sel_H, long long* sel_counter, int max_models, hipStream_t s,
                            bool by_weight, int symmetric, const double* refit, double* cx1, double* cy1, double* cx2, double* cy2)
{
    const auto k = by_weight ? k_sel_claim<true> : k_sel_claim<false>;
    hipLaunchKernelGGL(k, dim3((p.n + 255) / 256), dim3(256), 0, s, p.x1, p.y1, p.x2, p.y2, p.n, records, world, key_check, thr2,
                       mask, rec, sel_H, sel_counter, max_models, symmetric, refit, cx1, cy1, cx2, cy2);
    return hipGetLastError();
}

hipError_t launch_sel_refit(const Points& p, const Affines& a, const Epipolar& ep, const SelRecord* records, int world, double thr2,
                            const unsigned char* mask, int* labels, double* refit, int* sum, int* label_count, hipStream_t s,
                            bool by_weight, int symmetric, int* scratch3)
{
    const dim3 grid((p.n + 255) / 256);
    hipLaunchKernelGGL(k_sel_winner_labels, grid, dim3(256), 0, s, p.x1, p.y1, p.x2, p.y2, p.n, records, world, thr2, mask, labels,
                       refit, symmetric);
    hipError_t he = scratch3 ? launch_reestimate_3pt(p, labels, 1, ep, refit, label_count, scratch3, s)
                             : launch_reestimate(p, a, labels, 1, ep, refit, label_count, s);
    if (he != hipSuccess) return he;
    he = hipMemsetAsync(sum, 0, sizeof(int), s);
    if (he != hipSuccess) return he;
    const auto k = by_weight ? k_sel_measure<true> : k_sel_measure<false>;
    hipLaunchKernelGGL(k, grid, dim3(256), 0, s, p.x1, p.y1, p.x2, p.y2, p.n, thr2, mask, refit, sum, symmetric);
    hipLaunchKernelGGL(k_sel_measure_finish, dim3(1), dim3(64), 0, s, sum, refit);
    return hipGetLastError();
}

hipError_t launch_sel_publish(int* rec, unsigned long long* keys, SelRecord* my_record, int* h_rec_dev, hipStream_t s)
{
    hipLaunchKernelGGL(k_sel_publish, dim3(1), dim3(64), 0, s, rec, keys, my_record, h_rec_dev);
    return hipGetLastError();
}

hipError_t launch_best_fused(int* scores, int world, int longest, int base, int rem, int* h_best_dev, int* clear,
                             int clear_count, hipStream_t s)
{
    hipLaunchKernelGGL(k_best_fused, dim3(1), dim3(1024), 0, s, scores, world, longest, base, rem, h_best_dev, clear, clear_count);
    return hipGetLastError();
}

hipError_t launch_pad_scores(const int* counts, int m, int longest, int* scores, hipStream_t s)
{
    if (longest <= 0) return hipSuccess;
    hipLaunchKernelGGL(k_pad_scores, dim3((longest + 255) / 256), dim3(256), 0, s, counts, m, longest, scores);
    return hipGetLastError();
}

}
```

Baseline: 13.17 million.

## Chain selection-round kernels to cut launches and memsets per greedy round

```diff
diff --git a/multi-h_amd/csrc/capi.hip b/multi-h_amd/csrc/capi.hip
--- a/multi-h_amd/csrc/capi.hip
+++ b/multi-h_amd/csrc/capi.hip
@@ -714,6 +714,7 @@
     if (key == 38 && value >= 0 && value <= (1 << 20)) { e->tune_batch_min_labels = value; return MH_OK; }
     if (key == 39 && (value == 0 || value == 16 || value == 32 || value == 64)) { e->tune_batch_spw = value; return MH_OK; }
     if (key == 36 && (value == 0 || value == 1)) { e->tune_select_decrement = value; return MH_OK; }
+    if (key == 41 && (value == 0 || value == 1)) { e->tune_select_chain = value; return MH_OK; }
     if (key == 33 && value >= 0 && value <= (1 << 20)) { e->tune_ms_dense = value; return MH_OK; }
     if (key == 30 && (value == 0 || value == 1)) { e->tune_select_refine = value; return MH_OK; }
     if (key == 31 && (value == 0 || value == 1)) { e->tune_knn_grid = value; return MH_OK; }
diff --git a/multi-h_amd/csrc/capi_engine.hpp b/multi-h_amd/csrc/capi_engine.hpp
--- a/multi-h_amd/csrc/capi_engine.hpp
+++ b/multi-h_amd/csrc/capi_engine.hpp
@@ -289,6 +289,7 @@
     DevBuf<int> sel_pack_count;
     DevBuf<double> sel_gone[4];
     int tune_select_decrement = 1;
+    int tune_select_chain = 1;
     int tune_knn_grid = 1;
     DevBuf<int> knn_cell, knn_count, knn_start, knn_orig;
     DevBuf<float> knn_P;
@@ -400,9 +401,12 @@
 hipError_t reserve_counts(mh_engine* e, size_t n);
 int quiesce(mh_engine* e);
 int join_xchg(mh_engine* e);
-int score_models(mh_engine* e, const Points& p, const double* Hs, int m, double thr2, const unsigned char* dmask, int* counts_dev);
+struct ScorePrepared { bool table = false, sums_zeroed = false; };
+bool selection_uses_pretest(const mh_engine* e, double thr2, bool by_weight);
+int score_models(mh_engine* e, const Points& p, const double* Hs, int m, double thr2, const unsigned char* dmask, int* counts_dev,
+                 const ScorePrepared& prepared = ScorePrepared{});
 int msac_models(mh_engine* e, const Points& p, const double* Hs, int m, double thr2, const unsigned char* dmask, int* counts_dev,
-                int* weights_dev, bool plain_variant_only);
+                int* weights_dev, bool plain_variant_only, const ScorePrepared& prepared = ScorePrepared{});
 int launch_estimator(mh_engine* e, const int* labels_dev, int Nh, double* H_dev, int* counts_dev);
 int ensure_xchg_stream(mh_engine* e);
 int ensure_side_stream(mh_engine* e);
diff --git a/multi-h_amd/csrc/capi_score.hip b/multi-h_amd/csrc/capi_score.hip
--- a/multi-h_amd/csrc/capi_score.hip
+++ b/multi-h_amd/csrc/capi_score.hip
@@ -17,14 +17,20 @@
     return MH_OK;
 }
 
-int score_models(mh_engine* e, const Points& p, const double* Hs, int m, double thr2, const unsigned char* dmask, int* counts_dev)
+bool selection_uses_pretest(const mh_engine* e, double thr2, bool by_weight)
+{
+    return (by_weight || e->residual_mode != MH_RESIDUAL_SYMMETRIC) && pretest_usable(e, thr2, true);
+}
+
+int score_models(mh_engine* e, const Points& p, const double* Hs, int m, double thr2, const unsigned char* dmask, int* counts_dev,
+                 const ScorePrepared& prepared)
 {
     const bool fwd = e->residual_mode != MH_RESIDUAL_SYMMETRIC;
     if (fwd && m > 0 && pretest_usable(e, thr2, true)) {
-        HIPCHK(e->H32.reserve((size_t)m * 16));
+        if (!prepared.table) HIPCHK(e->H32.reserve((size_t)m * 16));
         HIPCHK(e->fb_pairs.reserve(1));
         if (e->score_pairs == 0) HIPCHK(hipMemsetAsync(e->fb_pairs.p, 0, sizeof(unsigned long long), e->stream));
-        HIPCHK(launch_model32(Hs, m, e->absmax_x, e->absmax_y, e->absmax_dst, e->H32.p, e->stream));
+        if (!prepared.table) HIPCHK(launch_model32(Hs, m, e->absmax_x, e->absmax_y, e->absmax_dst, e->H32.p, e->stream));
         int* ctl = nullptr;
         if (e->tune_score32_resident != 0) {
             int rc = ensure_sweep_ctl(e);
@@ -32,7 +38,7 @@
             ctl = e->sweep_ctl.p;
         }
         HIPCHK(launch_score32(p, Hs, e->H32.p, m, thr2, e->absmax_dst, dmask, counts_dev, e->fb_pairs.p, e->tune_score32_tiling, e->stream,
-                              ctl, e->cu_count, e->tune_score32_resident, &e->occ_score32));
+                              ctl, e->cu_count, e->tune_score32_resident, &e->occ_score32, prepared.sums_zeroed));
         e->score_pairs += (long long)m * p.n;
         return MH_OK;
     }
@@ -41,15 +47,17 @@
 }
 
 int msac_models(mh_engine* e, const Points& p, const double* Hs, int m, double thr2, const unsigned char* dmask, int* counts_dev,
-                int* weights_dev, bool plain_variant_only)
+                int* weights_dev, bool plain_variant_only, const ScorePrepared& prepared)
 {
     if (m <= 0 || p.n <= 0) return MH_OK;
     HIPCHK(e->fb_pairs.reserve(1));
     if (e->score_pairs == 0) HIPCHK(hipMemsetAsync(e->fb_pairs.p, 0, sizeof(unsigned long long), e->stream));
     if (pretest_usable(e, thr2, plain_variant_only)) {
-        HIPCHK(e->H32.reserve((size_t)m * 16));
-        HIPCHK(launch_model32(Hs, m, e->absmax_x, e->absmax_y, e->absmax_dst, e->H32.p, e->stream));
-        HIPCHK(launch_msac32(p, Hs, e->H32.p, m, thr2, e->absmax_dst, dmask, counts_dev, weights_dev, e->fb_pairs.p, e->stream));
+        if (!prepared.table) {
+            HIPCHK(e->H32.reserve((size_t)m * 16));
+            HIPCHK(launch_model32(Hs, m, e->absmax_x, e->absmax_y, e->absmax_dst, e->H32.p, e->stream));
+        }
+        HIPCHK(launch_msac32(p, Hs, e->H32.p, m, thr2, e->absmax_dst, dmask, counts_dev, weights_dev, e->fb_pairs.p, e->stream, prepared.sums_zeroed));
     } else {
         HIPCHK(launch_msac64(p, Hs, m, thr2, dmask, counts_dev, weights_dev, e->stream));
         e->score_pairs_plain_fp64 += (long long)m * p.n;
diff --git a/multi-h_amd/csrc/capi_select.hip b/multi-h_amd/csrc/capi_select.hip
--- a/multi-h_amd/csrc/capi_select.hip
+++ b/multi-h_amd/csrc/capi_select.hip
@@ -89,8 +89,9 @@
     for (int b = 0; b < 2; ++b) { HIPCHK(e->sel_orig[b].reserve(cap)); HIPCHK(e->sel_cand_H[b].reserve(cap * 9)); }
     HIPCHK(e->sel_counts.reserve(cap));
     if (by_weight) HIPCHK(e->sel_weights.reserve(cap));
-    HIPCHK(e->sel_rec.reserve(8));
-    HIPCHK(e->sel_keys.reserve(2));
+    const bool chain = e->tune_select_chain != 0;
+    HIPCHK(e->sel_rec.reserve(SEL_REC_WORDS));
+    HIPCHK(e->sel_keys.reserve(2 + (size_t)sel_offer_workgroups((int)cap)));
     HIPCHK(e->sel_out_H.reserve((size_t)max_models * 9));
     HIPCHK(e->sel_counter.reserve(max_models));
     HIPCHK(e->sel_records.reserve((size_t)world + 1));
@@ -104,7 +105,7 @@
     hipStream_t s = e->stream;
     if (point_mask) { HIPCHK(hipMemcpyAsync(e->mask.p, point_mask, n, hipMemcpyHostToDevice, s)); ++e->copies_h2d; }
     else HIPCHK(hipMemsetAsync(e->mask.p, 1, n, s));
-    HIPCHK(hipMemsetAsync(e->sel_rec.p, 0, sizeof(int) * 8, s));
+    HIPCHK(hipMemsetAsync(e->sel_rec.p, 0, sizeof(int) * SEL_REC_WORDS, s));
     HIPCHK(hipMemsetAsync(e->sel_keys.p, 0, sizeof(unsigned long long) * 2, s));
     HIPCHK(hipMemsetAsync(e->sel_records.p, 0, sizeof(SelRecord) * ((size_t)world + 1), s));
     if (sharded && longest > 0) HIPCHK(hipMemsetAsync(e->sel_scores.p, 0xff, sizeof(int) * (size_t)longest, s));
@@ -132,11 +133,14 @@
 
     int Mc = M, cur = 0, selected = 0, packed_as = -1;
     bool first = true;
+    const bool pretest = chain && selection_uses_pretest(e, thr2, by_weight);
+    bool table_made = false, left_cleared = false;
     for (int round = 0; round < max_models; ++round) {
         const double* Hs = first ? e->H.p : e->sel_cand_H[cur].p;
         const int* orig = first ? nullptr : e->sel_orig[cur].p;
-        auto score = [&](const Points& p, int* counts, int* wgts) -> int {
-            return by_weight ? msac_models(e, p, Hs, Mc, thr2, nullptr, counts, wgts, true) : score_models(e, p, Hs, Mc, thr2, nullptr, counts);
+        auto score = [&](const Points& p, int* counts, int* wgts, bool sums_zeroed) -> int {
+            const ScorePrepared prepared{ table_made, sums_zeroed };
+            return by_weight ? msac_models(e, p, Hs, Mc, thr2, nullptr, counts, wgts, true, prepared) : score_models(e, p, Hs, Mc, thr2, nullptr, counts, prepared);
         };
         auto score_round = [&]() -> int {
             if (e->inject_select_failure > 0 && --e->inject_select_failure == 0)
@@ -152,12 +156,12 @@
                 Points left = e->pts();
                 left.x1 = e->sel_gone[0].p; left.y1 = e->sel_gone[1].p; left.x2 = e->sel_gone[2].p; left.y2 = e->sel_gone[3].p;
                 left.n = gone;
-                const int rcs = score(left, e->sel_left.p, e->sel_left_w.p);
+                const int rcs = score(left, e->sel_left.p, e->sel_left_w.p, left_cleared);
                 if (rcs) return rcs;
                 HIPCHK(launch_sel_subtract(e->sel_carried[cur].p, e->sel_left.p, e->sel_carried_w[cur].p, e->sel_left_w.p, Mc, e->sel_counts.p, weights, s));
                 return MH_OK;
             }
-            if (active == n) return score(e->pts(), e->sel_counts.p, weights);
+            if (active == n) return score(e->pts(), e->sel_counts.p, weights, false);
             if (active > 0) {
                 HIPCHK(launch_sel_pack_points(e->pts(), e->mask.p, e->sel_pts[0].p, e->sel_pts[1].p, e->sel_pts[2].p, e->sel_pts[3].p,
                                               e->sel_pack_count.p, s));
@@ -165,7 +169,7 @@
                 Points packed = e->pts();
                 packed.x1 = e->sel_pts[0].p; packed.y1 = e->sel_pts[1].p; packed.x2 = e->sel_pts[2].p; packed.y2 = e->sel_pts[3].p;
                 packed.n = active;
-                return score(packed, e->sel_counts.p, weights);
+                return score(packed, e->sel_counts.p, weights, false);
             }
             HIPCHK(hipMemsetAsync(e->sel_counts.p, 0, sizeof(int) * (size_t)Mc, s));
             if (weights) HIPCHK(hipMemsetAsync(weights, 0, sizeof(int) * (size_t)Mc, s));
@@ -181,8 +185,13 @@
         }
         const int local_err = local_rc != MH_OK ? 1 : 0;
         const bool gather_scores = sharded && first && longest > 0;
-        HIPCHK(launch_sel_argmax(e->sel_counts.p, weights, orig, Mc, need, my_off, key_local, gather_scores ? e->sel_scores.p : nullptr, s));
-        HIPCHK(launch_sel_record(e->sel_counts.p, weights, orig, Hs, Mc, my_off, key_local, local_err, mode_word, my_record, s));
+        if (chain)
+            HIPCHK(launch_sel_offer(e->sel_counts.p, weights, orig, Hs, Mc, need, my_off, key_local, gather_scores ? e->sel_scores.p : nullptr,
+                                    e->sel_keys.p + 2, e->sel_rec.p + SEL_REC_OFFER_TICKET, local_err, mode_word, my_record, s));
+        else {
+            HIPCHK(launch_sel_argmax(e->sel_counts.p, weights, orig, Mc, need, my_off, key_local, gather_scores ? e->sel_scores.p : nullptr, s));
+            HIPCHK(launch_sel_record(e->sel_counts.p, weights, orig, Hs, Mc, my_off, key_local, local_err, mode_word, my_record, s));
+        }
         if (sharded) {
             if (gather_scores) {
                 rc = exchange(e, e->sel_scores.p, e->sel_gathered.p, sizeof(int) * (size_t)longest, s);
@@ -192,14 +201,22 @@
             rc = exchange(e, my_record, records, sizeof(SelRecord), s);
             if (rc) return rc;
         }
+        SelNextScore next;
+        if (pretest && e->H32.p && e->H32.cap >= (size_t)Mc * 16) {
+            next.H32 = e->H32.p; next.X = e->absmax_x; next.Y = e->absmax_y; next.Cmax = e->absmax_dst;
+        }
+        if (chain && decrement) { next.left = e->sel_left.p; next.left_w = e->sel_left_w.p; }
         HIPCHK(launch_sel_compact(e->sel_counts.p, weights, orig, Hs, Mc, need, records, world, my_off, e->sel_orig[cur ^ 1].p,
                                   e->sel_cand_H[cur ^ 1].p, e->sel_rec.p, decrement ? e->sel_carried[cur ^ 1].p : nullptr,
-                                  e->sel_carried_w[cur ^ 1].p, s));
+                                  e->sel_carried_w[cur ^ 1].p, s, next));
+        table_made = Mc > 0 && next.H32 != nullptr;
+        left_cleared = Mc > 0 && next.left != nullptr;
         const double* refit = nullptr;
         if (refine_usable) {
             Affines aff{ e->a11.p, e->a12.p, e->a21.p, e->a22.p };
             HIPCHK(launch_sel_refit(e->pts(), aff, e->epi, records, world, thr2, e->mask.p, e->labels_pts.p, e->sel_refit.p,
-                                    e->sel_refit_ctr.p, e->sel_refit_ctr.p + 1, s, by_weight, symmetric, refit3 ? e->r3_scratch.p : nullptr));
+                                    chain ? e->sel_rec.p + SEL_REC_MEASURE_SUM : e->sel_refit_ctr.p, e->sel_refit_ctr.p + 1, s, by_weight, symmetric,
+                                    refit3 ? e->r3_scratch.p : nullptr, chain ? e->sel_rec.p + SEL_REC_MEASURE_TICKET : nullptr));
             refit = e->sel_refit.p;
         }
         const unsigned long long* check = gather_scores && !local_err ? key_check : nullptr;
diff --git a/multi-h_amd/csrc/mh_kernels.hpp b/multi-h_amd/csrc/mh_kernels.hpp
--- a/multi-h_amd/csrc/mh_kernels.hpp
+++ b/multi-h_amd/csrc/mh_kernels.hpp
@@ -44,12 +44,12 @@
 hipError_t launch_model32(const double* H, int M, double X, double Y, double Cmax, float* H32 , hipStream_t s);
 hipError_t launch_score32(const Points& p, const double* H, const float* H32, int M, double thr2, double Cmax, const unsigned char* mask,
                           int* counts, unsigned long long* fallback_pairs, int tiling, hipStream_t s, int* resident_ctl = nullptr,
-                          int cu_count = 256, int resident_slices = 0, int* occ_cache = nullptr);
+                          int cu_count = 256, int resident_slices = 0, int* occ_cache = nullptr, bool counts_zeroed = false);
 hipError_t launch_cost32(const Points& p, const double* H, const float* H32, int M, double lambda, double thr2, double Cmax,
                          int* C, long long ldc, int* counts, hipStream_t s, int* resident_ctl = nullptr, int cu_count = 256,
                          int psplit_override = 0, int slice_major = 0, int batched = 0, int* occ_cache = nullptr, int rising = 0);
 hipError_t launch_msac32(const Points& p, const double* H, const float* H32, int M, double thr2, double Cmax, const unsigned char* mask,
-                         int* counts, int* weights, unsigned long long* fp64_pairs, hipStream_t s);
+                         int* counts, int* weights, unsigned long long* fp64_pairs, hipStream_t s, bool sums_zeroed = false);
 hipError_t launch_msac64(const Points& p, const double* H, int M, double thr2, const unsigned char* mask, int* counts, int* weights,
                          hipStream_t s);
 hipError_t launch_inliers_of_model(const Points& p, const double* H, int idx, double thr2,
@@ -263,15 +263,21 @@
 constexpr int SEL_MODE_HAF_MEMBERS_SHIFT = 17;
 constexpr int SEL_MODE_P3 = 1 << 23;
 static_assert(sizeof(SelRecord) == 88, "the exchanged record is 88 bytes");
+constexpr int SEL_REC_OFFER_TICKET = 8, SEL_REC_MEASURE_TICKET = 9, SEL_REC_MEASURE_SUM = 10, SEL_REC_WORDS = 12;
 hipError_t launch_sel_argmax(const int* counts, const int* weights, const int* orig, int Mc, int need, unsigned int my_off,
                              unsigned long long* key, int* scores_full, hipStream_t s);
 hipError_t launch_sel_argmax_gathered(const int* gathered, int world, int longest, int base, int rem, unsigned long long* key,
                                       hipStream_t s);
 hipError_t launch_sel_record(const int* counts, const int* weights, const int* orig, const double* Hs, int Mc, unsigned int my_off,
                              const unsigned long long* key_local, int err, int mode, SelRecord* record, hipStream_t s);
+inline int sel_offer_workgroups(int Mc) { return Mc > 0 ? (Mc + 255) / 256 : 1; }
+hipError_t launch_sel_offer(const int* counts, const int* weights, const int* orig, const double* Hs, int Mc, int need, unsigned int my_off,
+                            unsigned long long* key, int* scores_full, unsigned long long* wg_keys, int* ticket, int err, int mode,
+                            SelRecord* record, hipStream_t s);
+struct SelNextScore { float* H32 = nullptr; double X = 0.0, Y = 0.0, Cmax = 0.0; int* left = nullptr; int* left_w = nullptr; };
 hipError_t launch_sel_compact(const int* counts, const int* weights, const int* orig, const double* Hs, int Mc, int need,
                               const SelRecord* records, int world, unsigned int my_off, int* next_orig, double* next_H, int* rec,
-                              int* next_counts, int* next_weights, hipStream_t s);
+                              int* next_counts, int* next_weights, hipStream_t s, const SelNextScore& ns = SelNextScore{});
 hipError_t launch_sel_subtract(const int* carried_c, const int* left_c, const int* carried_w, const int* left_w, int Mc, int* counts,
                                int* weights, hipStream_t s);
 hipError_t launch_sel_claim(const Points& p, const SelRecord* records, int world, const unsigned long long* key_check, double thr2,
@@ -279,7 +285,7 @@
                             bool by_weight, int symmetric, const double* refit, double* cx1, double* cy1, double* cx2, double* cy2);
 hipError_t launch_sel_refit(const Points& p, const Affines& a, const Epipolar& ep, const SelRecord* records, int world, double thr2,
                             const unsigned char* mask, int* labels, double* refit, int* sum, int* label_count, hipStream_t s,
-                            bool by_weight, int symmetric, int* scratch3);
+                            bool by_weight, int symmetric, int* scratch3, int* ticket = nullptr);
 hipError_t launch_sel_publish(int* rec, unsigned long long* keys, SelRecord* my_record, int* h_rec_dev, hipStream_t s);
 hipError_t launch_best_fused(int* scores, int world, int longest, int base, int rem, int* h_best_dev, int* clear,
                              int clear_count, hipStream_t s);
diff --git a/multi-h_amd/csrc/msac32.hip b/multi-h_amd/csrc/msac32.hip
--- a/multi-h_amd/csrc/msac32.hip
+++ b/multi-h_amd/csrc/msac32.hip
@@ -105,13 +105,13 @@
 }
 
 hipError_t launch_msac32(const Points& p, const double* H, const float* H32, int M, double thr2, double Cmax, const unsigned char* mask,
-                         int* counts, int* weights, unsigned long long* fp64_pairs, hipStream_t s)
+                         int* counts, int* weights, unsigned long long* fp64_pairs, hipStream_t s, bool sums_zeroed)
 {
     if (M <= 0 || p.n <= 0) return hipSuccess;
     constexpr int PPL = 4, MC = 64;
     const int gx = (M + MC - 1) / MC, ntiles = (p.n + 256 * PPL - 1) / (256 * PPL);
     int psplit = 0;
-    hipError_t e = point_slices(gx, ntiles, 16, 4, 0, M, counts, weights, s, &psplit);
+    hipError_t e = point_slices(gx, ntiles, 16, 4, 0, M, counts, weights, s, &psplit, sums_zeroed);
     if (e != hipSuccess) return e;
     const Pretest32Launch c(thr2, Cmax, 1.0);
     if (mask) hipLaunchKernelGGL((k_msac32<PPL, MC, true>), dim3(gx, psplit), dim3(256), 0, s, p.x1, p.y1, p.x2, p.y2, p.n, H, H32, M, thr2, c.thr2_f, c.c_thr, c.k1, counts, weights, mask, psplit, fp64_pairs);
diff --git a/multi-h_amd/csrc/pretest32.hpp b/multi-h_amd/csrc/pretest32.hpp
--- a/multi-h_amd/csrc/pretest32.hpp
+++ b/multi-h_amd/csrc/pretest32.hpp
@@ -42,6 +42,26 @@
 struct Model32 {
     float h0, h1, h2, h3, h4, h5, h6, h7, h8, es, en, tau, a25;
 };
+
+__device__ __forceinline__ void model32_row(const double* __restrict__ h, double X, double Y, double Cmax, float* __restrict__ o)
+{
+    bool ok = true;
+    for (int q = 0; q < 9; ++q) {
+        ok = ok && fabs(h[q]) < 0x1p100;
+        o[q] = (float)h[q];
+    }
+    const double u = 0x1p-24;
+    const double as = fabs(h[6]) * X + fabs(h[7]) * Y + fabs(h[8]);
+    const double an = fmax(fabs(h[0]) * X + fabs(h[1]) * Y + fabs(h[2]), fabs(h[3]) * X + fabs(h[4]) * Y + fabs(h[5]));
+    const double es = 5.0 * u * as, en = 5.0 * u * an;
+    ok = ok && es >= 0x1p-80 && en >= 0x1p-80 && as < 0x1p100 && an < 0x1p100;
+    const double up = 1.0 + 0x1p-22;
+    o[9] = (float)(1.1 * es * up);
+    o[10] = (float)(1.1 * en * up);
+    o[11] = ok ? (float)(64.0 * es * up) : NAN;
+    o[12] = (float)(25.2 * 1.01 * (Cmax * es + en) * up);
+    o[13] = o[14] = o[15] = 0.f;
+}
 
 template <int MC, int THREADS>
 __device__ __forceinline__ void stage_model32(float4* s_m, const float* __restrict__ H32, int m0, int M)
@@ -198,11 +218,12 @@
     return ps < 1 ? 1 : ps;
 }
 
-inline hipError_t point_slices(int gx, int ntiles, int many_tiles, int few, int chosen, int M, int* sums, int* sums2, hipStream_t s, int* psplit)
+inline hipError_t point_slices(int gx, int ntiles, int many_tiles, int few, int chosen, int M, int* sums, int* sums2, hipStream_t s, int* psplit,
+                               bool sums_zeroed = false )
 {
     *psplit = clamp_slices(chosen > 0 ? chosen : gx < 1024 ? (2048 + gx - 1) / gx : (ntiles >= many_tiles ? few : 1), ntiles);
     for (int* a : { sums, sums2 })
-        if (a && *psplit > 1) {
+        if (a && *psplit > 1 && !sums_zeroed) {
             hipError_t e = hipMemsetAsync(a, 0, sizeof(int) * (size_t)M, s);
             if (e != hipSuccess) return e;
         }
diff --git a/multi-h_amd/csrc/score32.hip b/multi-h_amd/csrc/score32.hip
--- a/multi-h_amd/csrc/score32.hip
+++ b/multi-h_amd/csrc/score32.hip
@@ -7,24 +7,7 @@
 {
     const int m = blockIdx.x * 256 + threadIdx.x;
     if (m >= M) return;
-    const double* h = H + 9 * (size_t)m;
-    float* o = out + 16 * (size_t)m;
-    bool ok = true;
-    for (int q = 0; q < 9; ++q) {
-        ok = ok && fabs(h[q]) < 0x1p100;
-        o[q] = (float)h[q];
-    }
-    const double u = 0x1p-24;
-    const double as = fabs(h[6]) * X + fabs(h[7]) * Y + fabs(h[8]);
-    const double an = fmax(fabs(h[0]) * X + fabs(h[1]) * Y + fabs(h[2]), fabs(h[3]) * X + fabs(h[4]) * Y + fabs(h[5]));
-    const double es = 5.0 * u * as, en = 5.0 * u * an;
-    ok = ok && es >= 0x1p-80 && en >= 0x1p-80 && as < 0x1p100 && an < 0x1p100;
-    const double up = 1.0 + 0x1p-22;
-    o[9] = (float)(1.1 * es * up);
-    o[10] = (float)(1.1 * en * up);
-    o[11] = ok ? (float)(64.0 * es * up) : NAN;
-    o[12] = (float)(25.2 * 1.01 * (Cmax * es + en) * up);
-    o[13] = o[14] = o[15] = 0.f;
+    model32_row(H + 9 * (size_t)m, X, Y, Cmax, out + 16 * (size_t)m);
 }
 
 template <int PPL, int MC, bool MASK>
@@ -407,13 +390,13 @@
 template <int PPL, int MC, int MINW = 1>
 static hipError_t launch_score32_t(const Points& p, const double* H, const float* H32, int M, double thr2, double Cmax, const unsigned char* mask,
                                    int* counts, unsigned long long* fallback_pairs, hipStream_t s, int* resident_ctl = nullptr,
-                                   int cu_count = 256, int resident_slices = 0, int* occ_cache = nullptr)
+                                   int cu_count = 256, int resident_slices = 0, int* occ_cache = nullptr, bool counts_zeroed = false)
 {
     const int gx = (M + MC - 1) / MC, ntiles = (p.n + 256 * PPL - 1) / (256 * PPL);
     int psplit = 0, resident = 0;
     if (resident_ctl && resident_slices != 0 && !mask)
         resident = resident_grid((const void*)k_score32_resident<PPL, MC, false, MINW>, 256, occ_cache, cu_count, resident_slices, gx, ntiles, &psplit);
-    hipError_t e = point_slices(gx, ntiles, 16, 4, resident > 0 ? psplit : 0, M, counts, nullptr, s, &psplit);
+    hipError_t e = point_slices(gx, ntiles, 16, 4, resident > 0 ? psplit : 0, M, counts, nullptr, s, &psplit, counts_zeroed);
     if (e != hipSuccess) return e;
     const Pretest32Launch c(thr2, Cmax, 1.0);
     if (resident > 0) {
@@ -428,11 +411,11 @@
 
 hipError_t launch_score32(const Points& p, const double* H, const float* H32, int M, double thr2, double Cmax, const unsigned char* mask,
                           int* counts, unsigned long long* fallback_pairs, int tiling, hipStream_t s, int* resident_ctl, int cu_count,
-                          int resident_slices, int* occ_cache)
+                          int resident_slices, int* occ_cache, bool counts_zeroed)
 {
     if (M <= 0 || p.n <= 0) return hipSuccess;
     if (tiling == 0 && resident_ctl && resident_slices != 0)
-        return launch_score32_t<4, 64, 6>(p, H, H32, M, thr2, Cmax, mask, counts, fallback_pairs, s, resident_ctl, cu_count, resident_slices, occ_cache);
+        return launch_score32_t<4, 64, 6>(p, H, H32, M, thr2, Cmax, mask, counts, fallback_pairs, s, resident_ctl, cu_count, resident_slices, occ_cache, counts_zeroed);
 #ifdef MH_TUNING
     switch (tiling) {
     case 1: return launch_score32_t<4, 16>(p, H, H32, M, thr2, Cmax, mask, counts, fallback_pairs, s);
@@ -454,7 +437,7 @@
     default: break;
     }
 #endif
-    return launch_score32_t<4, 64, 6>(p, H, H32, M, thr2, Cmax, mask, counts, fallback_pairs, s);
-}
-
-}
+    return launch_score32_t<4, 64, 6>(p, H, H32, M, thr2, Cmax, mask, counts, fallback_pairs, s, nullptr, 256, 0, nullptr, counts_zeroed);
+}
+
+}
diff --git a/multi-h_amd/csrc/select.hip b/multi-h_amd/csrc/select.hip
--- a/multi-h_amd/csrc/select.hip
+++ b/multi-h_amd/csrc/select.hip
@@ -1,6 +1,7 @@
 #include "../../include/multih_hip.h"
 #include "mh_device.hpp"
 #include "mh_kernels.hpp"
+#include "pretest32.hpp"
 
 namespace mh {
 
@@ -91,6 +92,58 @@
     for (int q = 0; q < 9; ++q) record->H[q] = h[q];
 }
 
+__device__ __forceinline__ bool sel_last_workgroup(int* __restrict__ ticket)
+{
+    __shared__ int s_last;
+    asm volatile("s_waitcnt vmcnt(0)" ::: "memory");
+    __syncthreads();
+    if (threadIdx.x == 0) {
+        const int k = atomicAdd(ticket, 1);
+        s_last = k == (int)gridDim.x - 1 ? 1 : 0;
+        if (s_last) __hip_atomic_store(ticket, 0, __ATOMIC_RELAXED, __HIP_MEMORY_SCOPE_AGENT);
+    }
+    __syncthreads();
+    return s_last != 0;
+}
+
+template <bool BY_WEIGHT>
+__global__ void __launch_bounds__(256)
+k_sel_offer(const int* __restrict__ counts, const int* __restrict__ weights, const int* __restrict__ orig, const double* __restrict__ Hs,
+            int Mc, int need, unsigned int my_off, unsigned long long* __restrict__ key, int* __restrict__ scores_full,
+            unsigned long long* __restrict__ wg_keys, int* __restrict__ ticket, int err, int mode, SelRecord* __restrict__ record)
+{
+    const int c = blockIdx.x * 256 + threadIdx.x;
+    unsigned long long k = 0;
+    if (c < Mc) {
+        const int o = orig ? orig[c] : c;
+        const int cnt = counts[c];
+        const int rank = BY_WEIGHT ? weights[c] : cnt;
+        const bool eligible = cnt >= need;
+        if (eligible) k = sel_key(rank, my_off + (unsigned int)o);
+        if (scores_full) scores_full[o] = eligible ? rank : -1;
+    }
+    const unsigned long long b = wg_max_u64(k);
+    if (threadIdx.x == 0) {
+        if (b) atomicMax(key, b);
+        __hip_atomic_store(&wg_keys[blockIdx.x], b, __ATOMIC_RELAXED, __HIP_MEMORY_SCOPE_AGENT);
+    }
+    if (!sel_last_workgroup(ticket)) return;
+    const unsigned long long kl = __hip_atomic_load(key, __ATOMIC_RELAXED, __HIP_MEMORY_SCOPE_AGENT);
+    if (threadIdx.x == 0) { record->err = err; record->mode = mode; }
+    if (!kl) return;
+    __shared__ int s_wg;
+    for (int w = threadIdx.x; w < (int)gridDim.x; w += 256)
+        if (__hip_atomic_load(&wg_keys[w], __ATOMIC_RELAXED, __HIP_MEMORY_SCOPE_AGENT) == kl) s_wg = w;
+    __syncthreads();
+    const int cw = s_wg * 256 + threadIdx.x;
+    if (cw >= Mc) return;
+    const int o = orig ? orig[cw] : cw;
+    if (sel_key(BY_WEIGHT ? weights[cw] : counts[cw], my_off + (unsigned int)o) != kl) return;
+    record->key = kl;
+    const double* h = Hs + 9 * (size_t)cw;
+    for (int q = 0; q < 9; ++q) record->H[q] = h[q];
+}
+
 __device__ __forceinline__ unsigned long long sel_winner(const SelRecord* __restrict__ records, int world, int* rank_out)
 {
     unsigned long long kg = 0;
@@ -105,7 +158,7 @@
 k_sel_compact(const int* __restrict__ counts, const int* __restrict__ weights, const int* __restrict__ orig,
               const double* __restrict__ Hs, int Mc, int need, const SelRecord* __restrict__ records, int world, unsigned int my_off,
               int* __restrict__ next_orig, double* __restrict__ next_H, int* __restrict__ rec, int* __restrict__ next_counts,
-              int* __restrict__ next_weights)
+              int* __restrict__ next_weights, const SelNextScore ns)
 {
     const int c = blockIdx.x * 256 + threadIdx.x;
     const unsigned long long kg = sel_winner(records, world, nullptr);
@@ -135,6 +188,11 @@
         }
         const double* h = Hs + 9 * (size_t)c;
         for (int q = 0; q < 9; ++q) next_H[9 * (size_t)pos + q] = h[q];
+        if (ns.H32) model32_row(h, ns.X, ns.Y, ns.Cmax, ns.H32 + 16 * (size_t)pos);
+        if (ns.left) {
+            ns.left[pos] = 0;
+            if (BY_WEIGHT) ns.left_w[pos] = 0;
+        }
     }
 }
 
@@ -221,7 +279,7 @@
 __global__ void __launch_bounds__(256)
 k_sel_measure(const double* __restrict__ x1, const double* __restrict__ y1, const double* __restrict__ x2,
               const double* __restrict__ y2, int N, double thr2, const unsigned char* __restrict__ mask,
-              const double* __restrict__ refit, int* __restrict__ sum, int symmetric)
+              const double* __restrict__ refit, int* __restrict__ sum, int symmetric, int* __restrict__ ticket, double* __restrict__ value)
 {
     const int n = blockIdx.x * 256 + threadIdx.x;
     bool in = false;
@@ -232,14 +290,16 @@
         if (BY_WEIGHT) w = data_term<false>(d2, thr2, (double)MH_MSAC_SCALE, 0);
     }
     const unsigned long long m = __ballot(in);
-    if (!BY_WEIGHT) {
-        if ((threadIdx.x & 63) == 0 && m) atomicAdd(sum, (int)__popcll(m));
-        return;
-    }
-    if (m == 0ull) return;
+    if (m != 0ull) {
+        if (BY_WEIGHT) {
 #pragma unroll
-    for (int o = 32; o >= 1; o >>= 1) w += __shfl_xor(w, o, 64);
-    if ((threadIdx.x & 63) == 0) atomicAdd(sum, w);
+            for (int o = 32; o >= 1; o >>= 1) w += __shfl_xor(w, o, 64);
+        } else w = (int)__popcll(m);
+        if ((threadIdx.x & 63) == 0) atomicAdd(sum, w);
+    }
+    if (!ticket) return;
+    if (!sel_last_workgroup(ticket)) return;
+    if (threadIdx.x == 0) *value = (double)atomicExch(sum, 0);
 }
 
 __global__ void k_sel_measure_finish(const int* __restrict__ sum, double* __restrict__ refit)
@@ -345,14 +405,24 @@
     return hipGetLastError();
 }
 
+hipError_t launch_sel_offer(const int* counts, const int* weights, const int* orig, const double* Hs, int Mc, int need, unsigned int my_off,
+                            unsigned long long* key, int* scores_full, unsigned long long* wg_keys, int* ticket, int err, int mode,
+                            SelRecord* record, hipStream_t s)
+{
+    const auto k = weights ? k_sel_offer<true> : k_sel_offer<false>;
+    hipLaunchKernelGGL(k, dim3(sel_offer_workgroups(Mc)), dim3(256), 0, s, counts, weights, orig, Hs, Mc, need, my_off, key, scores_full,
+                       wg_keys, ticket, err, mode, record);
+    return hipGetLastError();
+}
+
 hipError_t launch_sel_compact(const int* counts, const int* weights, const int* orig, const double* Hs, int Mc, int need,
                               const SelRecord* records, int world, unsigned int my_off, int* next_orig, double* next_H, int* rec,
-                              int* next_counts, int* next_weights, hipStream_t s)
+                              int* next_counts, int* next_weights, hipStream_t s, const SelNextScore& ns)
 {
     if (Mc <= 0) return hipSuccess;
     const auto k = weights ? k_sel_compact<true> : k_sel_compact<false>;
     hipLaunchKernelGGL(k, dim3((Mc + 255) / 256), dim3(256), 0, s, counts, weights, orig, Hs, Mc, need, records, world, my_off,
-                       next_orig, next_H, rec, next_counts, next_weights);
+                       next_orig, next_H, rec, next_counts, next_weights, ns);
     return hipGetLastError();
 }
 
@@ -377,7 +447,7 @@
 
 hipError_t launch_sel_refit(const Points& p, const Affines& a, const Epipolar& ep, const SelRecord* records, int world, double thr2,
                             const unsigned char* mask, int* labels, double* refit, int* sum, int* label_count, hipStream_t s,
-                            bool by_weight, int symmetric, int* scratch3)
+                            bool by_weight, int symmetric, int* scratch3, int* ticket)
 {
     const dim3 grid((p.n + 255) / 256);
     hipLaunchKernelGGL(k_sel_winner_labels, grid, dim3(256), 0, s, p.x1, p.y1, p.x2, p.y2, p.n, records, world, thr2, mask, labels,
@@ -385,10 +455,14 @@
     hipError_t he = scratch3 ? launch_reestimate_3pt(p, labels, 1, ep, refit, label_count, scratch3, s)
                              : launch_reestimate(p, a, labels, 1, ep, refit, label_count, s);
     if (he != hipSuccess) return he;
+    const auto k = by_weight ? k_sel_measure<true> : k_sel_measure<false>;
+    if (ticket) {
+        hipLaunchKernelGGL(k, grid, dim3(256), 0, s, p.x1, p.y1, p.x2, p.y2, p.n, thr2, mask, refit, sum, symmetric, ticket, refit + 9);
+        return hipGetLastError();
+    }
     he = hipMemsetAsync(sum, 0, sizeof(int), s);
     if (he != hipSuccess) return he;
-    const auto k = by_weight ? k_sel_measure<true> : k_sel_measure<false>;
-    hipLaunchKernelGGL(k, grid, dim3(256), 0, s, p.x1, p.y1, p.x2, p.y2, p.n, thr2, mask, refit, sum, symmetric);
+    hipLaunchKernelGGL(k, grid, dim3(256), 0, s, p.x1, p.y1, p.x2, p.y2, p.n, thr2, mask, refit, sum, symmetric, (int*)nullptr, (double*)nullptr);
     hipLaunchKernelGGL(k_sel_measure_finish, dim3(1), dim3(64), 0, s, sum, refit);
     return hipGetLastError();
 }
```

After: 13.18 million, median of 2. No clear change (+0.0%).
